# shaohua-pan/RobustCap

Measured on AMD Instinct MI355X. Metric: body-frames/sec (sig_mp fwd + FK) at batch 256, higher is better.
Workload: dtype f32; 1 GPU; synthetic 60 fps, 6 IMU + 33 keypoints, batch 256 x 1448 frames per GPU (256 bodies in total, weak scaling), confidence schedule 'mixed', seeded random weights (63.4 M params); batch_per_gpu=256, bodies_total=256, frames=1448, conf=mixed, parallelism=dp1 (sequence sharding)

## Files before the change

### include/robustcap_hip.h

```cpp
#ifndef ROBUSTCAP_HIP_H
#define ROBUSTCAP_HIP_H

#include <stdint.h>

#ifdef __cplusplus
extern "C" {
#endif

typedef struct rc_ctx rc_ctx;

typedef enum {
    RC_OK = 0,
    RC_ERR_INVALID = -1,
    RC_ERR_HIP = -2,
    RC_ERR_STATE = -3,
    RC_ERR_UNKNOWN_KEY = -4
} rc_status;

typedef struct {
    double conf_lo, conf_hi;
    float contact_threshold;
    float distance_threshold;
    float height_threshold;
    double tran_filter_num;
    int32_t use_flat_floor;
    int32_t use_vision_updater;
    int32_t use_imu_updater;
    int32_t live;
    int32_t update_vision_freq;
    int32_t use_reproj_opt;
    float smooth;
    int32_t reserved;
} rc_params;

#define RC_FLAG_FIRST_FRAME 1u

int rc_create(int32_t batch, int32_t live_at_construction, rc_ctx** out);
int rc_destroy(rc_ctx* ctx);
const char* rc_last_error(const rc_ctx* ctx);
int rc_default_params(int32_t live_at_construction, rc_params* out);
int rc_get_params(const rc_ctx* ctx, rc_params* out);
int rc_set_params(rc_ctx* ctx, const rc_params* p);

int rc_load_weight(rc_ctx* ctx, const char* key, const float* host, int64_t numel);
int rc_finalize_weights(rc_ctx* ctx);

int rc_set_body(rc_ctx* ctx, const int32_t* parent, const float* J, const float* w33, const float* v33);

int rc_set_gravity(rc_ctx* ctx, const float* gravity_host);

int rc_reset(rc_ctx* ctx, const uint8_t* row_mask, void* stream);

int rc_step(rc_ctx* ctx, const float* j2dc, const float* accc, const float* oric, const float* first_tran,
            uint32_t flags, float* pose_out, float* tran_out, void* stream);

int rc_sequence(rc_ctx* ctx, int32_t T, const float* j2dc, int64_t rs_j2d, const float* accc, int64_t rs_acc,
                const float* oric, int64_t rs_ori, const float* first_tran, uint32_t flags, float* pose_out,
                int64_t rs_pose, float* tran_out, int64_t rs_tran, void* stream);

int rc_sequence_rows(rc_ctx* ctx, int32_t T, const int32_t* len_host, const float* j2dc, int64_t rs_j2d, const float* accc,
                     int64_t rs_acc, const float* oric, int64_t rs_ori, const float* first_tran, uint32_t flags, float* pose_out,
                     int64_t rs_pose, float* tran_out, int64_t rs_tran, void* stream);
int rc_get_sequence_row_frames(rc_ctx* ctx, int64_t* body_frames);

int rc_set_gemm_mode(rc_ctx* ctx, int32_t mode);
int rc_get_gemm_mode(const rc_ctx* ctx);
int rc_default_gemm_mode(int32_t total_rows);

int rc_set_sequence_mode(rc_ctx* ctx, int32_t mode, int32_t min_frames);
int rc_get_sequence_stats(rc_ctx* ctx, int64_t* wave_frames, int64_t* stepped_frames, int64_t* ticks);
int rc_get_launch_stats(rc_ctx* ctx, int64_t* lds_launches, int64_t* other_wide_launches);
int rc_get_launch_stats_w32(rc_ctx* ctx, int64_t* w32_launches);
int rc_set_resident(rc_ctx* ctx, int32_t enable, int32_t workgroups);
int rc_get_resident_stats(rc_ctx* ctx, int64_t* segments, int64_t* aborts);
int rc_plan_sequence(const int8_t* codes, int32_t B, int32_t T, const int32_t* pend, uint32_t flags, int32_t use_vision_updater,
                     uint8_t* mode_out);
int rc_plan_wave(const int8_t* codes, int32_t B, int32_t T, int32_t t0, const int32_t* first_reach, const int32_t* pend,
                 int32_t use_imu_updater, int32_t use_vision_updater, int32_t* frame_at, int64_t frame_at_cap,
                 int32_t* n_ticks, int32_t* n_prep, int32_t* counts, double* est_us);
int rc_plan_wave_rows(const int8_t* codes, int32_t B, int32_t T, int32_t t0, const int32_t* len, const int32_t* first_reach,
                      const int32_t* pend, int32_t use_imu_updater, int32_t use_vision_updater, int32_t* frame_at, int64_t frame_at_cap,
                      int32_t* n_ticks, int32_t* n_prep, int32_t* counts, double* est_us);

int rc_live_begin(rc_ctx* ctx);
int rc_live_step(rc_ctx* ctx, const float* j2dc_host, const float* accc_host, const float* oric_host,
                 const float* first_tran_host, uint32_t flags, float* pose_host, float* tran_host);
int rc_live_end(rc_ctx* ctx);
int rc_get_live_stats(rc_ctx* ctx, int64_t* lean_frames, int64_t* full_frames);
int rc_get_live_prestep(rc_ctx* ctx, int64_t* presteps, int32_t* available);
int rc_get_live_replayed(rc_ctx* ctx, int64_t* frames);
int rc_get_live_spin(rc_ctx* ctx, int64_t* taken, int64_t* lost);
int rc_get_live_profile(rc_ctx* ctx, double* avg_us4);
int rc_get_live_last_profile(rc_ctx* ctx, double* us6);
int rc_get_live_backend(rc_ctx* ctx, int32_t* lean_captured, int32_t* aql, char* note, int32_t note_len);

int rc_r6d_to_rotmat(const float* r6d, float* R, int64_t n, void* stream);
int rc_axis_angle_to_rotmat(const float* aa, float* R, int64_t n, void* stream);
int rc_rotmat_to_axis_angle(const float* R, float* aa, int64_t n, void* stream);
int rc_rotmat_to_r6d(const float* R, float* r6d, int64_t n, void* stream);
int rc_angle_between(const float* R1, const float* R2, float* out, int64_t n, void* stream);
int rc_lerp(const float* a, const float* b, double t, float* out, int64_t n, void* stream);
int rc_normalize_rows(const float* x, float* out, float* norm, int64_t rows, int32_t width, void* stream);
int rc_bbox_normalise(const float* kp, float* out, int64_t n, void* stream);
int rc_conf_mean(const float* j2dc, int64_t n, double lo, double hi, float* mean, int8_t* code, void* stream);
int rc_shape_body(rc_ctx* ctx, const float* v_template, const float* shapedirs, const float* J_regressor, const float* beta,
                  int32_t V, float* verts_out, float* joints_out);
int rc_fk_r(rc_ctx* ctx, const float* Rlocal, float* Rglobal, int64_t n, void* stream);
int rc_bone_to_joint(rc_ctx* ctx, const float* bone, float* joint, int64_t n, void* stream);
int rc_joint_to_bone(rc_ctx* ctx, const float* joint, float* bone, int64_t n, void* stream);
int rc_zero_pose(rc_ctx* ctx, float* joint, float* vert, void* stream);
int rc_ik_r(rc_ctx* ctx, const float* Rglobal, float* Rlocal, int64_t n, void* stream);
int rc_fk_bone(rc_ctx* ctx, const float* Rglobal, float* joints, int64_t n, void* stream);
int rc_body_fk(rc_ctx* ctx, const float* pose, const float* tran, float* grot, float* joint, float* j33,
               int64_t n, void* stream);
int rc_lstm_step(rc_ctx* ctx, const char* net, const float* x, const uint8_t* row_mask, float* y, void* stream);
#define RC_SUBNET_SCRATCH_BYTES (256ll << 20)
int rc_subnet_forward(rc_ctx* ctx, const char* net, int32_t n, const int32_t* lengths_host, const float* x, float* y,
                      const float* init_h, const float* init_c, float* final_h, float* final_c, void* stream);
int rc_init_net_forward(rc_ctx* ctx, int32_t n, const float* v, float* out, void* stream);
int rc_get_subnet_stats(rc_ctx* ctx, int64_t* calls, int64_t* frames, int64_t* chunks, int64_t* scratch_bytes);
int rc_set_mesh(rc_ctx* ctx, const float* v_template_host, const float* weights_host, int32_t V);
int rc_body_mesh(rc_ctx* ctx, const float* pose, const float* tran, float* vert, int64_t n, void* stream);
int rc_set_regressor(rc_ctx* ctx, const float* j_regressor_host, int32_t n_rows, int32_t n_used);
int rc_mesh_metrics(rc_ctx* ctx, const float* pose, const float* gt_pose, int64_t n, float* per_frame, double* mean_host,
                    void* stream);
int rc_synth_imu(rc_ctx* ctx, const float* pose, const float* tran, const int32_t* vertex_ids_host,
                 const int32_t* joint_ids_host, int64_t T, int32_t smooth_n, float* imu_ori, float* imu_acc, float* joint3d,
                 float* vert6, void* stream);
int rc_syn_acc(const float* v, int64_t T, int64_t width, int32_t smooth_n, float* acc, void* stream);
int rc_procrustes_error(const float* S1, const float* S2, int64_t n, int32_t n_points, float* err, void* stream);
int rc_position_error(const float* p, const float* t, int64_t n, float* dist, double* mean_host, void* stream);
int rc_set_ignored_landmarks(rc_ctx* ctx, const int32_t* ids_host, int32_t n);
int rc_reproj_residual(rc_ctx* ctx, const float* pose, const float* tran, const float* kp, const float* K,
                       float sigma, float* loss, int64_t T, void* stream);


int rc_smplify_set_prior(rc_ctx* ctx, const float* means_host, const float* precisions_host, const float* nll_weights_host);

int rc_smplify_loss_grad(rc_ctx* ctx, const float* x, const float* kp, const float* ref3d, const float* imu_aa,
                         const float* K_host, int64_t T, double* loss_host, float* grad, void* stream);

int rc_smplify_set_ref3d(rc_ctx* ctx, const float* ref3d);

typedef struct rc_smplify_info {
    int32_t status;
    int32_t n_iter, n_eval;
    int32_t reserved;
    double first_loss, final_loss;
    double host_ms, device_ms;
} rc_smplify_info;

int rc_smplify_run(rc_ctx* ctx, const float* pose, const float* tran, const float* kp, const float* imu_ori,
                   const float* K_host, int64_t T, float lr, int32_t max_iter, float loss_threshold, float* pose_out,
                   float* tran_out, uint8_t* update_host, rc_smplify_info* info, void* stream);

int rc_smplify_run_batch(rc_ctx* ctx, int32_t n_rows, const int64_t* T_rows, const float* const* pose, const float* const* tran,
                         const float* const* kp, const float* const* imu_ori, const float* K_host, float lr, int32_t max_iter,
                         float loss_threshold, float* const* pose_out, float* const* tran_out, uint8_t* const* update_host,
                         rc_smplify_info* infos, void* stream);

typedef double (*rc_objective_fn)(void* user, const double* x, double* grad, int64_t n);
int rc_lbfgs_minimize(rc_objective_fn objective, void* user, int64_t n, double* x, double lr, int32_t max_iter,
                      int32_t max_eval, int32_t history_size, double tolerance_grad, double tolerance_change,
                      int32_t* n_iter_out, int32_t* n_eval_out, double* losses_out, int64_t cap);

int rc_camera_inputs(const float* kp_pix, const float* imu_acc_w, const float* imu_ori_w, const float* K_host,
                     const float* Tcw_host, float* j2dc, float* accc, float* oric, float* gravity_out_host, int64_t n,
                     void* stream);

int rc_camera_inputs_rows(const float* kp_norm, const float* imu_acc_w, const float* imu_ori_w, const int32_t* seq_of_row,
                          const int32_t* len, const float* K_host, const float* Tcw_host, float image_w, float image_h,
                          int32_t n_rows, int32_t Tmax, float* j2dc, float* accc, float* oric, float* gravity_out_host,
                          void* cam_scratch, void* stream);

int rc_get_state(rc_ctx* ctx, const char* net, float* h_host, float* c_host, void* stream);
int rc_get_fusion_state(rc_ctx* ctx, int32_t* out_host, void* stream);

int rc_get_trace(rc_ctx* ctx, int32_t* trace_host, void* stream);

int rc_gemm_timing(rc_ctx* ctx, int32_t enable);
int rc_gemm_timing_read(rc_ctx* ctx, double* total_ms, int64_t* launches);
int rc_gemm_timing_busy(rc_ctx* ctx, double* busy_ms);

#ifdef __cplusplus
}
#endif
#endif
```

### robustcap_amd/_lib.py

```python
import ctypes as C
import os

_HERE = os.path.dirname(os.path.abspath(__file__))
LIB_PATH = os.environ.get("RC_LIB_PATH") or os.path.join(_HERE, "csrc", "librobustcap_hip.so")
HEADER_PATH = os.path.join(os.path.dirname(_HERE), "include", "robustcap_hip.h")

RC_FLAG_FIRST_FRAME = 1


class RcParams(C.Structure):
    _fields_ = [("conf_lo", C.c_double), ("conf_hi", C.c_double),
                ("contact_threshold", C.c_float), ("distance_threshold", C.c_float),
                ("height_threshold", C.c_float), ("tran_filter_num", C.c_double),
                ("use_flat_floor", C.c_int32), ("use_vision_updater", C.c_int32),
                ("use_imu_updater", C.c_int32), ("live", C.c_int32),
                ("update_vision_freq", C.c_int32), ("use_reproj_opt", C.c_int32), ("smooth", C.c_float),
                ("reserved", C.c_int32)]


class RcSmplifyInfo(C.Structure):
    _fields_ = [("status", C.c_int32), ("n_iter", C.c_int32), ("n_eval", C.c_int32), ("reserved", C.c_int32),
                ("first_loss", C.c_double), ("final_loss", C.c_double), ("host_ms", C.c_double), ("device_ms", C.c_double)]


OBJECTIVE_FN = C.CFUNCTYPE(C.c_double, C.c_void_p, C.POINTER(C.c_double), C.POINTER(C.c_double), C.c_int64)


class RobustcapLibraryError(RuntimeError):
    pass


_P, _I32, _I64, _U32, _F = C.c_void_p, C.c_int32, C.c_int64, C.c_uint32, C.c_float
SIGNATURES = {
    "rc_create": (_I32, [_I32, _I32, C.POINTER(_P)]),
    "rc_destroy": (_I32, [_P]),
    "rc_last_error": (C.c_char_p, [_P]),
    "rc_default_params": (_I32, [_I32, C.POINTER(RcParams)]),
    "rc_get_params": (_I32, [_P, C.POINTER(RcParams)]),
    "rc_set_params": (_I32, [_P, C.POINTER(RcParams)]),
    "rc_load_weight": (_I32, [_P, C.c_char_p, _P, _I64]),
    "rc_finalize_weights": (_I32, [_P]),
    "rc_set_body": (_I32, [_P, _P, _P, _P, _P]),
    "rc_set_gravity": (_I32, [_P, _P]),
    "rc_reset": (_I32, [_P, _P, _P]),
    "rc_step": (_I32, [_P, _P, _P, _P, _P, _U32, _P, _P, _P]),
    "rc_sequence": (_I32, [_P, _I32, _P, _I64, _P, _I64, _P, _I64, _P, _U32, _P, _I64, _P, _I64, _P]),
    "rc_sequence_rows": (_I32, [_P, _I32, _P, _P, _I64, _P, _I64, _P, _I64, _P, _U32, _P, _I64, _P, _I64, _P]),
    "rc_get_sequence_row_frames": (_I32, [_P, C.POINTER(_I64)]),
    "rc_set_gemm_mode": (_I32, [_P, _I32]),
    "rc_get_gemm_mode": (_I32, [_P]),
    "rc_default_gemm_mode": (_I32, [_I32]),
    "rc_set_sequence_mode": (_I32, [_P, _I32, _I32]),
    "rc_get_sequence_stats": (_I32, [_P, C.POINTER(_I64), C.POINTER(_I64), C.POINTER(_I64)]),
    "rc_get_launch_stats": (_I32, [_P, C.POINTER(_I64), C.POINTER(_I64)]),
    "rc_get_launch_stats_w32": (_I32, [_P, C.POINTER(_I64)]),
    "rc_set_resident": (_I32, [_P, _I32, _I32]),
    "rc_get_resident_stats": (_I32, [_P, C.POINTER(_I64), C.POINTER(_I64)]),
    "rc_plan_sequence": (_I32, [_P, _I32, _I32, _P, _U32, _I32, _P]),
    "rc_plan_wave": (_I32, [_P, _I32, _I32, _I32, _P, _P, _I32, _I32, _P, _I64, C.POINTER(_I32), C.POINTER(_I32), _P, _P]),
    "rc_plan_wave_rows": (_I32, [_P, _I32, _I32, _I32, _P, _P, _P, _I32, _I32, _P, _I64, C.POINTER(_I32), C.POINTER(_I32), _P, _P]),
    "rc_live_begin": (_I32, [_P]),
    "rc_live_step": (_I32, [_P, _P, _P, _P, _P, _U32, _P, _P]),
    "rc_live_end": (_I32, [_P]),
    "rc_get_live_stats": (_I32, [_P, _P, _P]),
    "rc_get_live_prestep": (_I32, [_P, _P, _P]),
    "rc_get_live_replayed": (_I32, [_P, _P]),
    "rc_get_live_spin": (_I32, [_P, _P, _P]),
    "rc_get_live_profile": (_I32, [_P, _P]),
    "rc_get_live_last_profile": (_I32, [_P, _P]),
    "rc_get_live_backend": (_I32, [_P, _P, _P, _P, _I32]),
    "rc_get_fusion_state": (_I32, [_P, _P, _P]),
    "rc_r6d_to_rotmat": (_I32, [_P, _P, _I64, _P]),
    "rc_axis_angle_to_rotmat": (_I32, [_P, _P, _I64, _P]),
    "rc_rotmat_to_axis_angle": (_I32, [_P, _P, _I64, _P]),
    "rc_rotmat_to_r6d": (_I32, [_P, _P, _I64, _P]),
    "rc_angle_between": (_I32, [_P, _P, _P, _I64, _P]),
    "rc_lerp": (_I32, [_P, _P, C.c_double, _P, _I64, _P]),
    "rc_normalize_rows": (_I32, [_P, _P, _P, _I64, _I32, _P]),
    "rc_bbox_normalise": (_I32, [_P, _P, _I64, _P]),
    "rc_conf_mean": (_I32, [_P, _I64, C.c_double, C.c_double, _P, _P, _P]),
    "rc_shape_body": (_I32, [_P, _P, _P, _P, _P, _I32, _P, _P]),
    "rc_fk_r": (_I32, [_P, _P, _P, _I64, _P]),
    "rc_bone_to_joint": (_I32, [_P, _P, _P, _I64, _P]),
    "rc_joint_to_bone": (_I32, [_P, _P, _P, _I64, _P]),
    "rc_zero_pose": (_I32, [_P, _P, _P, _P]),
    "rc_ik_r": (_I32, [_P, _P, _P, _I64, _P]),
    "rc_fk_bone": (_I32, [_P, _P, _P, _I64, _P]),
    "rc_body_fk": (_I32, [_P, _P, _P, _P, _P, _P, _I64, _P]),
    "rc_set_mesh": (_I32, [_P, _P, _P, _I32]),
    "rc_body_mesh": (_I32, [_P, _P, _P, _P, _I64, _P]),
    "rc_set_regressor": (_I32, [_P, _P, _I32, _I32]),
    "rc_mesh_metrics": (_I32, [_P, _P, _P, _I64, _P, C.POINTER(C.c_double), _P]),
    "rc_synth_imu": (_I32, [_P, _P, _P, _P, _P, _I64, _I32, _P, _P, _P, _P, _P]),
    "rc_syn_acc": (_I32, [_P, _I64, _I64, _I32, _P, _P]),
    "rc_procrustes_error": (_I32, [_P, _P, _I64, _I32, _P, _P]),
    "rc_position_error": (_I32, [_P, _P, _I64, _P, C.POINTER(C.c_double), _P]),
    "rc_lstm_step": (_I32, [_P, C.c_char_p, _P, _P, _P, _P]),
    "rc_subnet_forward": (_I32, [_P, C.c_char_p, _I32, _P, _P, _P, _P, _P, _P, _P, _P]),
    "rc_init_net_forward": (_I32, [_P, _I32, _P, _P, _P]),
    "rc_get_subnet_stats": (_I32, [_P, C.POINTER(_I64), C.POINTER(_I64), C.POINTER(_I64), C.POINTER(_I64)]),
    "rc_set_ignored_landmarks": (_I32, [_P, _P, _I32]),
    "rc_reproj_residual": (_I32, [_P, _P, _P, _P, _P, _F, _P, _I64, _P]),
    "rc_smplify_set_prior": (_I32, [_P, _P, _P, _P]),
    "rc_smplify_set_ref3d": (_I32, [_P, _P]),
    "rc_smplify_loss_grad": (_I32, [_P, _P, _P, _P, _P, _P, _I64, C.POINTER(C.c_double), _P, _P]),
    "rc_smplify_run": (_I32, [_P, _P, _P, _P, _P, _P, _I64, _F, _I32, _F, _P, _P, _P, C.POINTER(RcSmplifyInfo), _P]),
    "rc_smplify_run_batch": (_I32, [_P, _I32, _P, _P, _P, _P, _P, _P, _F, _I32, _F, _P, _P, _P, _P, _P]),
    "rc_lbfgs_minimize": (_I32, [OBJECTIVE_FN, _P, _I64, C.POINTER(C.c_double), C.c_double, _I32, _I32, _I32, C.c_double,
                                 C.c_double, C.POINTER(_I32), C.POINTER(_I32), C.POINTER(C.c_double), _I64]),
    "rc_camera_inputs": (_I32, [_P, _P, _P, _P, _P, _P, _P, _P, _P, _I64, _P]),
    "rc_camera_inputs_rows": (_I32, [_P, _P, _P, _P, _P, _P, _P, _F, _F, _I32, _I32, _P, _P, _P, _P, _P, _P]),
    "rc_get_state": (_I32, [_P, C.c_char_p, _P, _P, _P]),
    "rc_get_trace": (_I32, [_P, _P, _P]),
    "rc_gemm_timing": (_I32, [_P, _I32]),
    "rc_gemm_timing_read": (_I32, [_P, C.POINTER(C.c_double), C.POINTER(_I64)]),
    "rc_gemm_timing_busy": (_I32, [_P, C.POINTER(C.c_double)]),
}

_lib = None


OPTIONAL_IN_AB_BUILDS = frozenset({"rc_get_launch_stats_w32", "rc_set_resident", "rc_get_resident_stats", "rc_get_launch_stats", "rc_get_live_spin", "rc_get_live_replayed", "rc_get_live_profile", "rc_get_live_last_profile",
                                   "rc_get_live_prestep"})


def load():
    global _lib
    if _lib is not None:
        return _lib
    if not os.path.exists(LIB_PATH):
        raise RobustcapLibraryError(
            f"{LIB_PATH} not found: the HIP extension is not built. Run "
            "`python -c \"import __graft_entry__ as g; g.build()\"` at the repo root. There is no CPU fallback.")
    try:
        lib = C.CDLL(LIB_PATH)
    except OSError as e:
        raise RobustcapLibraryError(f"cannot load {LIB_PATH}: {e}") from e
    ab_build = bool(os.environ.get("RC_LIB_PATH"))
    skipped = []
    for name, (res, args) in SIGNATURES.items():
        if ab_build and name in OPTIONAL_IN_AB_BUILDS and not hasattr(lib, name):
            skipped.append(name)
            continue
        try:
            fn = getattr(lib, name)
        except AttributeError as e:
            raise RobustcapLibraryError(f"{LIB_PATH} does not export {name}: the library does not match include/robustcap_hip.h") from e
        fn.restype, fn.argtypes = res, args
    if skipped:
        import warnings
        warnings.warn(f"RC_LIB_PATH={LIB_PATH}: entry points missing in this build (calls to them will fail): {', '.join(skipped)}")
    _lib = lib
    return lib


def check(ctx, rc, what):
    if rc != 0:
        msg = load().rc_last_error(ctx)
        raise RobustcapLibraryError(f"{what} failed ({rc}): {msg.decode() if msg else ''}")


def ptr(t):
    return None if t is None else C.c_void_p(t.data_ptr())


def stream_ptr():
    import torch
    return C.c_void_p(torch.cuda.current_stream().cuda_stream)
```

### robustcap_amd/csrc/rc_api.cpp

```cpp
#include "../../include/robustcap_hip.h"
#include "rc_internal.h"

#include <algorithm>
#if defined(__x86_64__) || defined(_M_X64)
#include <immintrin.h>
#define RC_STORE_FENCE() _mm_sfence()
#else
#define RC_STORE_FENCE() __atomic_thread_fence(__ATOMIC_SEQ_CST)
#endif

#include <chrono>
#include <cmath>
#include <cstdio>
#include <cstdlib>
#include <cstring>
#include <map>
#include <string>
#include <thread>
#include <vector>

#define RC_SPLIT_MAIN_MIN_BATCH 48
#define RC_SPLIT_MIN_BATCH 48
#define RC_TILE64_MIN_BATCH 192

// ... 8 lines not shown
struct NetSpec { const char* name; int in, H, out; };
const NetSpec kNets[6] = {{"rnn2", 72, 512, 69},  {"rnn3", 141, 512, 3},   {"rnn4", 171, 1280, 69},
                          {"rnn6", 240, 1024, 3}, {"rnn7", 141, 512, 144}, {"rnn8", 141, 512, 2}};
enum { N2 = 0, N3 = 1, N4 = 2, N6 = 3, N7 = 4, N8 = 5 };
const int kInit[3][2] = {{69, 512}, {512, 1024}, {1024, 2048}};

inline int round_up(int x, int m) { return (x + m - 1) / m * m; }

struct Dense {
    float* W = nullptr; float* b = nullptr;
    void* Ws = nullptr;
    float* Wrm = nullptr;
    int K = 0, N = 0, Kp = 0, Np = 0;
    int mr = 2, nc = 4;
};
struct NetDev {
    Dense lin1, lin2;
    float* Wl[2] = {nullptr, nullptr};
    void* Wls[2] = {nullptr, nullptr};
    float* bl[2] = {nullptr, nullptr};
    float* h = nullptr;
    float* c = nullptr;
    int* steps = nullptr;
    float* x1 = nullptr;
    float* part = nullptr;
    int in = 0, H = 0, out = 0;
    int nc = 4;
    int mr = 2;
};

}

struct rc_ctx {
    int B = 0;
    int Bp = 0;
    int dev = 0;
    rc_params prm{};
    NetDev net[6];
    Dense init[3];
    float *hid1 = nullptr, *hid2 = nullptr, *xtmp = nullptr;
    FrameBuffers fb{};
    BodyConst* body = nullptr;
    float *mesh_vt = nullptr, *mesh_w = nullptr;
    int mesh_V = 0;
    float* mesh_kM = nullptr;
    int mesh_nk = 0;
    std::vector<float> mesh_vt_h, mesh_w_h, mesh_Jr_h;
    float jroot_h[3] = {0.f, 0.f, 0.f};
    bool fold_dirty = false;
    DevBuf<float> sweep_scratch;
    size_t sweep_scratch_cap = 0;
    unsigned long long ign_mask = RC_IGN_DEFAULT;
    bool have_body = false, have_weights = false;
    std::map<std::string, std::vector<float>> staged;
    std::vector<DevBuf<char>> allocs;
    std::vector<std::pair<void*, size_t>> alloc_bytes;
    std::vector<DevBuf<char>> weight_allocs;
    bool alloc_weights = false;
    HipEvent eager_ev;
    bool eager_dirty = false;
    std::string err;
    HipStream live_stream;
    HipGraph live_graph;
    HipGraphExec live_exec;
    PinBuf<float> live_in_h, live_out_h;
    DevBuf<float> live_in_d, live_out_d, live_ft_d;
    float *live_in_io = nullptr, *live_out_io = nullptr;
    bool live_zero_copy = false;
    bool live_eager = false;
    HipGraph live_graph_notr;
    HipGraphExec live_exec_notr;
    std::vector<unsigned char> live_maybe_pend;
    bool live_prev_known = false;
    int live_lean = 1;
    int live_lean_nc = 1;
    HipGraph live_graph_lean;
    HipGraphExec live_exec_lean;
    LiveFrame live_frame{};
    int live_aql_on = 1;
    AqlChain* live_aql = nullptr;
    std::string live_aql_note;
    int live_prestep = 1;
    bool live_spin = false, live_spin_always = false;
    volatile unsigned* spin_mb = nullptr;
    float* spin_in = nullptr;
    PinBuf<unsigned> spin_state_h;
    int aql_prog_spin[2] = {-1, -1}, aql_prog_spin_pre[2] = {-1, -1};
    int spin_pending = -1;
    int spin_pending_par = 0, spin_next_par = 0;
    unsigned long long spin_pending_seq = 0;
    bool live_spin_b2b = true;
    bool spin_valid = false;
    long long stat_live_spin = 0, stat_live_spin_lost = 0;
    bool live_arm = true;
    double live_prestep_idle_us = 500.0;
    DevBuf<float> live_pre_buf;
    int aql_prog_lean = -1, aql_prog_lean_pre = -1, aql_prog_pre = -1;
    bool live_pre_valid = false;
    bool live_have_return = false;
    std::chrono::steady_clock::time_point live_last_return{};
    long long stat_live_pre = 0;
    PinBuf<int> live_status_h;
    std::vector<unsigned char> live_may_reach;
    long long stat_live_lean = 0, stat_live_full = 0;
    long long stat_live_replayed = 0;
    DevBuf<int> live_abort_d;
    bool live_blind = false;
    double live_prof_us[4] = {0.0, 0.0, 0.0, 0.0};
    long long live_prof_n = 0;
    double live_prof_last[6] = {0, 0, 0, 0, 0, 0};
    bool timing = false;
    int timing_mode = 1;
    std::vector<std::pair<HipEvent, HipEvent>> ev_pool;
    size_t ev_used = 0;
    double timed_ms = 0.0;
    double timed_busy_ms = 0.0;
    long long timed_launches = 0;
    bool gemm_split = false;
    bool live_launch = false;
    unsigned live_nt_mask = 63u;
    int seq_mode = 1;
    int seq_min_frames = 8;
    float* x1_alt[6] = {nullptr, nullptr, nullptr, nullptr, nullptr, nullptr};
    int tile6[2] = {0, 0}, tile378[2] = {0, 0}, tile2[2] = {0, 0}, tile4[2] = {0, 0};
    bool ring2_failed = false;
    HipStream aux_stream;
    HipStream wide2_stream;
    HipEvent ev_main[8], ev_aux[8], ev_wide2[4];
    HipStream wide3_stream;
    HipEvent ev_head[4], ev_wide3[4];
    float* x1_alt2[6] = {nullptr, nullptr, nullptr, nullptr, nullptr, nullptr};
    DevBuf<signed char> scan_codes_d;
    PinBuf<signed char> scan_codes_h;
    PinBuf<int> scan_state_h;
    size_t scan_cap = 0;
    long long stat_wave_frames = 0, stat_stepped_frames = 0, stat_ticks = 0;
    long long stat_row_frames = 0;
    DevBuf<int> row_len_d;
    PinBuf<int> row_len_h;
    size_t row_len_cap = 0;
    HipEvent row_len_ev[2];
    unsigned row_len_turn = 0;
    bool ring2_ready = false;
    FrameBuffers ring2[16];
    std::vector<GemmProblem> wave2_prob;
    bool wave2_valid = false;
    DevBuf<int> frame_at_d;
    PinBuf<int> frame_at_h;
    size_t frame_at_cap = 0;
    double cost_tick_us = 1.0, cost_tick_small_us = 13.0, cost_frame_us = 285.0, cost_tr_us = 55.0;
    SmplifyOwner smplify;
    SubnetOwner subnet;
    int trace_next = 0;
    long long stat_wide_launches = 0;
    int lds_min_rows = 64;
    int lds_min_batch = 65;
    int lds_ksplit[3] = {1, 2, 2};
    DevBuf<float> lds_slab;
    DevBuf<int> lds_tickets;
    size_t lds_region_tiles = 0;
    unsigned lds_rot = 0;
    DevBuf<ResidentTick> res_ticks_d;
    PinBuf<ResidentTick> res_ticks_h;
    DevBuf<int> res_ints_d;
    PinBuf<int> res_base_h;
    PinBuf<int> res_abort_h;
    size_t res_cap = 0;
    long long stat_resident_segments = 0, stat_resident_aborts = 0;
    bool live_selfcheck_ran = false;
    bool resident_on = false;
    int resident_wgs = 224;
    long long stat_lds_launches = 0;
    long long stat_w32_launches = 0;
};

namespace {

int fail(rc_ctx* ctx, int code, const std::string& msg) {
    if (ctx) ctx->err = msg; else g_create_error = msg;
    return code;
}

template <typename T>
int dev_alloc(rc_ctx* ctx, T** p, size_t count, bool zero = true) {
    DevBuf<char> q;
    HIP_TRY(ctx, rc_alloc(q, count * sizeof(T)));
    if (zero) HIP_TRY(ctx, hipMemset(q.get(), 0, count * sizeof(T)));
    *p = reinterpret_cast<T*>(q.get());
    if (!ctx->alloc_weights) ctx->alloc_bytes.emplace_back(q.get(), count * sizeof(T));
    (ctx->alloc_weights ? ctx->weight_allocs : ctx->allocs).push_back(std::move(q));
    return RC_OK;
}

int dismiss_queued_frame(rc_ctx* ctx) {
    if (ctx->spin_pending < 0 || !ctx->live_aql || !ctx->spin_mb) return RC_OK;
    const int par = ctx->spin_pending_par;
    ctx->spin_mb[32 * par] = 2u;
    RC_STORE_FENCE();
    const int arc = rc_aql_wait_frame(ctx->live_aql);
    ctx->spin_state_h[4 * par] = 0;
    ctx->stat_live_spin_lost += 1;
    ctx->spin_pending = -1;
    return arc == 0 ? RC_OK : fail(ctx, RC_ERR_HIP, "the live frame queued ahead did not leave");
}

int mark_eager(rc_ctx* ctx, hipStream_t st) {
    ctx->live_pre_valid = false;
    ctx->spin_valid = false;
    if (int rc = dismiss_queued_frame(ctx)) return rc;
    if (!ctx->eager_ev) return RC_OK;
    HIP_TRY(ctx, hipEventRecord(ctx->eager_ev.get(), st));
    ctx->eager_dirty = true;
    return RC_OK;
}

template <typename Body>
void for_column_blocks(int n_cb, Body body) {
    const int nt = std::max(1, std::min({8, n_cb / 8, (int)std::thread::hardware_concurrency()}));
    if (nt <= 1) { for (int cb = 0; cb < n_cb; ++cb) body(cb); return; }
    std::vector<std::thread> th;
    for (int t = 0; t < nt; ++t)
        th.emplace_back([=] { for (int cb = t; cb < n_cb; cb += nt) body(cb); });
    for (std::thread& x : th) x.join();
}

template <typename F>
std::vector<float> pack_weights(int Np, int Kp, F getW) {
    std::vector<float> out((size_t)Np * Kp);
    const int Q = Kp / RC_KC;
    for_column_blocks(Np / 16, [&](int cb) {
        for (int q = 0; q < Q; ++q)
            for (int l = 0; l < 64; ++l) {
                const int kq = l >> 4, j = l & 15;
                float* d = &out[(((size_t)cb * Q + q) * 64 + l) * 4];
                for (int s = 0; s < 4; ++s) d[s] = getW(cb * 16 + j, RC_KC * q + 4 * kq + s);
            }
    });
    return out;
}

template <typename F>
std::vector<uint16_t> pack_weights_split(int Np, int Kp, F getW) {
    std::vector<uint16_t> out((size_t)Np * Kp * 3);
    const int Qs = Kp / 32;
    for_column_blocks(Np / 16, [&](int cb) {
        for (int kb = 0; kb < Qs; ++kb)
            for (int l = 0; l < 64; ++l) {
                const int kq = l >> 4, j = l & 15;
                for (int e = 0; e < 8; ++e) {
                    const int k = 32 * kb + (e < 4 ? 4 * kq + e : 16 + 4 * kq + (e - 4));
                    const float w = getW(cb * 16 + j, k);
                    uint32_t u;
                    std::memcpy(&u, &w, 4);
                    const uint32_t uh = u & 0xffff0000u;
                    float fh;
                    std::memcpy(&fh, &uh, 4);
                    const float r1 = w - fh;
                    uint32_t u1;
                    std::memcpy(&u1, &r1, 4);
                    const uint32_t um = u1 & 0xffff0000u;
                    float fm;
                    std::memcpy(&fm, &um, 4);
                    const float r2 = r1 - fm;
                    uint32_t u2;
                    std::memcpy(&u2, &r2, 4);
                    const size_t base = (((size_t)cb * Qs + kb) * 3) * 512 + (size_t)l * 8 + e;
                    out[base] = (uint16_t)(uh >> 16);
                    out[base + 512] = (uint16_t)(um >> 16);
                    out[base + 1024] = (uint16_t)(u2 >> 16);
                }
            }
    });
    return out;
}

int upload16(rc_ctx* ctx, void** dst, const std::vector<uint16_t>& v) {
    uint16_t* q = nullptr;
    if (int rc = dev_alloc(ctx, &q, v.size(), false)) return rc;
    HIP_TRY(ctx, hipMemcpy(q, v.data(), v.size() * sizeof(uint16_t), hipMemcpyHostToDevice));
    *dst = q;
    return RC_OK;
}

int upload(rc_ctx* ctx, float** dst, const std::vector<float>& v) {
    if (int rc = dev_alloc(ctx, dst, v.size(), false)) return rc;
    HIP_TRY(ctx, hipMemcpy(*dst, v.data(), v.size() * sizeof(float), hipMemcpyHostToDevice));
    return RC_OK;
}

int make_dense(rc_ctx* ctx, Dense& d, const std::vector<float>& W, const std::vector<float>& b, int N, int K) {
    d.mr = N <= 160 ? 1 : 2; d.nc = N <= 160 ? 2 : 4;
    d.N = N; d.K = K; d.Kp = round_up(K, RC_KALIGN); d.Np = round_up(N, 16 * d.nc);
    auto get = [&](int n, int k) -> float { return (n < N && k < K) ? W[(size_t)n * K + k] : 0.0f; };
    std::vector<float> bp(d.Np, 0.0f);
    for (int n = 0; n < N; ++n) bp[n] = b[n];
    if (int rc = upload(ctx, &d.W, pack_weights(d.Np, d.Kp, get))) return rc;
    if (int rc = upload16(ctx, &d.Ws, pack_weights_split(d.Np, d.Kp, get))) return rc;
    if (N <= 160) if (int rc = upload(ctx, &d.Wrm, W)) return rc;
    return upload(ctx, &d.b, bp);
}

const std::vector<float>* staged(rc_ctx* ctx, const std::string& key, size_t numel) {
    auto it = ctx->staged.find(key);
    if (it == ctx->staged.end() || it->second.size() != numel) return nullptr;
    return &it->second;
}
// ... 604 lines not shown
        if (i < 4) HIP_TRY(ctx, hipEventCreateWithFlags(rc_out(ctx->ev_wide3[i]), evf));
    }
    ctx->ring2_ready = true;
    ctx->wave2_valid = false;
    return RC_OK;
}

int ensure_wave2_buffers(rc_ctx* ctx) {
    if (ctx->ring2_ready) return RC_OK;
    if (ctx->ring2_failed) return fail(ctx, RC_ERR_STATE, "wavefront engine: its buffers could not be allocated earlier (out of memory?)");
    const int rc = ensure_wave2_buffers_once(ctx);
    if (rc != RC_OK) ctx->ring2_failed = true;
    return rc;
}

int build_wave2_problems(rc_ctx* ctx) {
    ctx->wave2_prob.assign((size_t)kRing * W2_PROB, GemmProblem{});
    const int B = ctx->B;
    for (int sl = 0; sl < kRing; ++sl) {
        const FrameBuffers& fb = ctx->ring2[sl];
        for (int q = 0; q < RC_TICK_PROB; ++q) {
            const TickStage& ts = kTick[q];
            const NetDev& n = ctx->net[ts.net];
            float* x1 = (sl & 1) ? ctx->x1_alt[ts.net] : n.x1;
            Stage st{ts.net, (int)RC_ROW2_VALID, nullptr, 256, Out{nullptr, 0, 0, false}, fb.flags2};
            switch (ts.net) {
                case N4: st.x = fb.x4; st.y = Out{fb.x6, 256, 171, true}; st.flag_bit = (int)RC_ROW2_M4; st.x_alt = fb.x4l;
                         st.sel_bit = (int)RC_ROW_VIS; st.out_bit = (int)RC_ROW_VIS; break;
                case N2: st.x = fb.x2; st.ldx = 128; st.y = Out{fb.x3, 256, 72, true}; break;
                case N6: st.x = fb.x6; st.y = Out{fb.pc, 4, 0, false}; st.flag_bit = (int)RC_ROW2_M6; st.x_alt = fb.x6l;
                         st.sel_bit = (int)RC_ROW_PC; st.out_bit = (int)RC_ROW_PC; break;
                case N3: st.x = fb.x3; st.y = Out{fb.vr, 4, 0, false}; break;
                case N7: st.x = fb.x78; st.y = Out{fb.r6d, 144, 0, false}; break;
                default: st.x = fb.x78; st.y = Out{fb.contact, 2, 0, false}; break;
            }
            GemmProblem p = ts.kind == 0 ? lin1_problem(ctx, st) : (ts.kind == 3 ? lin2_problem(ctx, st) : lstm_problem(ctx, st, ts.kind - 1));
            if (ts.kind == 0) { p.out = x1; p.sel_flags = fb.flags; }
            if (ts.kind == 1) p.seg[0].base = x1;
            if (ts.kind == 3) p.out_flags = fb.flags;
            p.steps = fb.wsteps + (size_t)ts.net * B;
            p.open_step = 0; p.step_off = 0;
            ctx->wave2_prob[(size_t)sl * W2_PROB + q] = p;
        }
        ctx->wave2_prob[(size_t)sl * W2_PROB + W2_INIT0] = dense_problem(ctx, ctx->init[0], seg(fb.xi, 128, 0), Out{ctx->hid1, 512, 0, true}, true, RC_ROW_REACH, fb.flags, nullptr, false);
        ctx->wave2_prob[(size_t)sl * W2_PROB + W2_INIT1] = dense_problem(ctx, ctx->init[1], seg(ctx->hid1, 512, 0), Out{ctx->hid2, 1024, 0, true}, true, RC_ROW_REACH, fb.flags, nullptr, false);
        ctx->wave2_prob[(size_t)sl * W2_PROB + W2_INIT2] = dense_problem(ctx, ctx->init[2], seg(ctx->hid2, 1024, 0), Out{ctx->fb.init_out, 2048, 0, false}, false, RC_ROW_REACH, fb.flags, nullptr, false);
    }
    ctx->wave2_valid = true;
    return RC_OK;
}

inline int w2_stage(int q) { return q < RC_TICK_PROB ? kTick[q].stage : kInitStage + (q - W2_INIT0); }

enum WaveEngine { ENG_PLAIN, ENG_SPLIT, ENG_TRI };
WaveEngine pick_wave_engine(const rc_ctx* c) {
    if (c->B < RC_SPLIT_MAIN_MIN_BATCH) return ENG_PLAIN;
    return lds_context(c) ? ENG_TRI : ENG_SPLIT;
}
bool resident_segment(const rc_ctx* c, WaveEngine eng, const WavePlan& P) {
    return eng == ENG_TRI && c->resident_on && c->B <= 256 && P.n_ticks > 0 && !(c->timing && c->timing_mode != 3);
}
inline int w2_group(int q, bool tri) {
    if (q >= RC_TICK_PROB) return tri ? G_REST : G_BIG;
    return (tri && kTick[q].net == N6 && kTick[q].group == G_BIG) ? G_REST : kTick[q].group;
}

struct WaveTiles { int t4[2], t6[2], t5[2]; };
WaveTiles wave_tiles(WaveEngine eng) {
    WaveTiles t{{4, eng == ENG_PLAIN ? 5 : 8}, {4, 8}, {4, 8}};
    tile_env("RC_SEQ_RNN4", &t.t4[0], &t.t4[1]);
    tile_env("RC_SEQ_RNN6", &t.t6[0], &t.t6[1]);
    tile_env("RC_SEQ_H512", &t.t5[0], &t.t5[1]);
    return t;
}

int reserve_frame_at(rc_ctx* ctx, size_t need, size_t want) {
    HIP_TRY(ctx, rc_grow(ctx->frame_at_cap, need, want, ctx->frame_at_d, want, ctx->frame_at_h, want));
    return RC_OK;
}

std::vector<GemmProblem> collect(const rc_ctx* ctx, const WavePlan& P, WaveEngine eng, const WaveTiles& tiles, int k, int g) {
    static const int tile64_rows = tune_env("RC_SEQ_TILE64_ROWS", 33);
    static const bool rows_as_padded = tune_env("RC_SEQ_ROWS_AS_PADDED", 1) != 0;
    const int B = ctx->B;
    std::vector<GemmProblem> ps;
    for (int qi = 0; qi < W2_PROB; ++qi) {
        const int q = qi < 4 ? (qi ^ 2) : qi;
        if (w2_group(q, eng == ENG_TRI) != g) continue;
        const int e = k - w2_stage(q);
        if (e < 0 || e >= P.n_prep) continue;
        const int net = q < RC_TICK_PROB ? kTick[q].net : -1;
        const int kind = q < RC_TICK_PROB ? kTick[q].kind : 4;
        const int riders = P.n_rider[e];
        const int rows = kind == 4 ? P.n_reach[e] : ((net == N4 || net == N6) ? P.n_vis[e] + riders : P.n_valid[e]);
        if (rows <= 0) continue;
        const int rows_k = kind == 4 ? rows : rows + (rows_as_padded ? P.done(e) : 0);
        GemmProblem p = ctx->wave2_prob[(size_t)(e % kRing) * W2_PROB + q];
        if (kind == 0 || kind == 1) {
            float* x1 = e % 3 == 0 ? ctx->net[net].x1 : (e % 3 == 1 ? ctx->x1_alt[net] : ctx->x1_alt2[net]);
            if (kind == 0) p.out = x1; else p.seg[0].base = x1;
        }
        if (kind == 1 || kind == 2) {
            const NetDev& n = ctx->net[net];
            int mr, nc;
            if (lds_problem(ctx, rows_k)) {
                mr = 16; nc = 8;
            } else if (ctx->gemm_split && rows_k >= tile64_rows) {
                const int* t = n.H == 512 ? tiles.t5 : (n.H == 1024 ? tiles.t6 : tiles.t4);
                mr = t[0]; nc = t[1];
            } else {
                pick_tile(n.H, rows_k, &mr, &nc);
            }
            p.mr = mr; p.nc = nc; p.n_tiles = n.H / (4 * nc);
        } else if (kind == 0 || kind == 4) {
            if (rows_k <= 16) { p.mr = 1; p.nc = 1; p.n_tiles = (p.N + 15) / 16; }
            else if (kind == 0 && ctx->gemm_split && rows_k >= tile64_rows) {
                const int np = round_up(p.N, 64);
                if (np % 128 == 0) { p.mr = 4; p.nc = 8; p.n_tiles = np / 128; }
            }
        }
        p.m_tiles = (rows + 16 * p.mr - 1) / (16 * p.mr);
        if (rows == B && kind != 4) {
            p.flags = nullptr; p.flag_bit = 0;
            if (riders == 0 && (net == N4 || net == N6) && P.n_vis[e] == B) {
                p.alt_base = nullptr; p.sel_flags = nullptr; p.sel_bit = 0; p.out_flags = nullptr; p.out_bit = 0;
            }
        }
        ps.push_back(p);
    }
    if (g != G_LIN2) {
        int total = 0;
        for (const GemmProblem& p : ps) total += p.n_tiles * p.m_tiles;
        if (total > 0 && total <= 128)
            for (GemmProblem& p : ps)
                if (p.epi == RC_EPI_LSTM && p.mr == 4 && p.nc == 8) { p.nc = 4; p.n_tiles *= 2; }
    }
    return ps;
}

struct WaveSeg {
    rc_ctx* ctx; const WavePlan& P; const FrameIO& io0; hipStream_t st, aux;
    WaveEngine eng; WaveTiles tiles; rc_params_dev prm; WavePrep wp; WaveTail wt;
    int rows(const std::vector<int>& v, int tick) const { return tick >= 0 && tick < P.n_prep ? v[tick] : 0; }
    std::vector<GemmProblem> group(int k, int g) const { return collect(ctx, P, eng, tiles, k, g); }
};

void wave_prep(WaveSeg& S, int k) {
    if (k >= S.P.n_prep) return;
    S.wp.frame_at = S.ctx->frame_at_d.get() + (size_t)k * S.ctx->B;
    S.wp.first_tick = k == 0 ? 1 : 0;
    rc_launch_prep_wave(S.ctx->ring2[k % kRing], S.io0, S.prm, S.ctx->B, S.wp, S.aux);
}

int wave_lin2_fuse_tail(WaveSeg& S, int k, bool merge, hipEvent_t signal) {
    rc_ctx* ctx = S.ctx;
    const int B = ctx->B;
    if (int rc = launch_problems(ctx, S.group(k, G_LIN2), nullptr, S.aux, true)) return rc;
    const bool fuse = S.rows(S.P.n_valid, k - kFuseStage) > 0, tail = S.rows(S.P.n_valid, k - kTailStage) > 0;
    bool merged = false, carried = false;
    if (tail) {
        const FrameBuffers& tgt = ctx->ring2[k % kRing];
        S.wt.x4l = tgt.x4l; S.wt.x6l = tgt.x6l; S.wt.flags2 = tgt.flags2; S.wt.wsteps = tgt.wsteps;
    }
    if (merge && fuse && tail)
        merged = carried = rc_launch_fuse_tail(ctx->ring2[(k - kTailStage) % kRing], ctx->ring2[(k - kFuseStage) % kRing], S.io0, S.prm, ctx->body, B, S.wt, S.aux, signal);
    if (!merged && fuse) rc_launch_fuse(ctx->ring2[(k - kFuseStage) % kRing], S.io0, S.prm, B, S.aux);
    if (!merged && tail) {
        rc_launch_tail(ctx->ring2[(k - kTailStage) % kRing], S.io0, S.prm, ctx->body, B, 0, S.aux, nullptr, &S.wt, signal);
        carried = true;
    }
    if (signal && !carried) HIP_TRY(ctx, hipEventRecord(signal, S.aux));
    return RC_OK;
}

inline int wave_wait(rc_ctx* ctx, int k, hipStream_t s, std::initializer_list<hipEvent_t> waits) {
    if (k > 0) for (hipEvent_t w : waits) if (w) HIP_TRY(ctx, hipStreamWaitEvent(s, w, 0));
    return RC_OK;
}

int wave_issue(rc_ctx* ctx, int k, hipStream_t s, std::initializer_list<hipEvent_t> waits, const std::vector<GemmProblem>& ps, hipEvent_t signal) {
    if (int rc = wave_wait(ctx, k, s, waits)) return rc;
    bool carried = false;
    if (int rc = launch_problems(ctx, ps, nullptr, s, false, signal, &carried)) return rc;
    if (signal && !carried) HIP_TRY(ctx, hipEventRecord(signal, s));
    return RC_OK;
}

int stream_tick(WaveSeg& S, int k) {
    rc_ctx* ctx = S.ctx;
    const int e = k & 3, ep = (k + 3) & 3;
    hipStream_t st = S.st, aux = S.aux, w2 = ctx->wide2_stream.get(), w3 = ctx->wide3_stream.get();
    hipEvent_t main_p = ctx->ev_main[ep].get(), aux_p = ctx->ev_aux[ep].get(), w2_p = ctx->ev_wide2[ep].get(), w3_p = ctx->ev_wide3[ep].get(),
               head_p = ctx->ev_head[ep].get();
    hipEvent_t main_e = ctx->ev_main[e].get(), aux_e = ctx->ev_aux[e].get(), w2_e = ctx->ev_wide2[e].get(), w3_e = ctx->ev_wide3[e].get(),
               head_e = ctx->ev_head[e].get();
    bool init_now = false;
    for (int q = W2_INIT0; q < W2_PROB; ++q) init_now = init_now || S.rows(S.P.n_reach, k - w2_stage(q)) > 0;
    if (S.eng == ENG_TRI) {
        std::vector<GemmProblem> l1, rnn6, h512;
        for (const GemmProblem& p : S.group(k, G_REST)) (p.epi != RC_EPI_LSTM ? l1 : (p.H == 1024 ? rnn6 : h512)).push_back(p);
        if (int rc = wave_issue(ctx, k, aux, {}, l1, head_e)) return rc;
        wave_prep(S, k);
        if (int rc = wave_wait(ctx, k, aux, {w3_p, main_p, w2_p})) return rc;
        if (int rc = wave_lin2_fuse_tail(S, k, true, aux_e)) return rc;
        if (int rc = wave_issue(ctx, k, w2, {head_p}, rnn6, w2_e)) return rc;
        static const int h5_early = tune_env("RC_SEQ_H5_EARLY", 0);
        const bool early = h5_early && S.rows(S.P.n_reach, k - 1 - kTailStage) == 0;
        if (int rc = wave_issue(ctx, k, w3, {early ? head_p : aux_p}, h512, w3_e)) return rc;
        if (int rc = wave_issue(ctx, k, st, {head_p}, S.group(k, G_BIG), main_e)) return rc;
    } else if (S.eng == ENG_SPLIT) {
        if (int rc = wave_wait(ctx, k, aux, {main_p, w2_p})) return rc;
        wave_prep(S, k);
        if (int rc = wave_lin2_fuse_tail(S, k, false, aux_e)) return rc;
        if (int rc = wave_issue(ctx, k, w2, {aux_p}, S.group(k, G_REST), w2_e)) return rc;
        if (int rc = wave_issue(ctx, k, st, {w2_p, init_now ? aux_p : nullptr}, S.group(k, G_BIG), main_e)) return rc;
    } else {
        if (int rc = wave_wait(ctx, k, aux, {main_p})) return rc;
        wave_prep(S, k);
        if (int rc = wave_lin2_fuse_tail(S, k, false, aux_e)) return rc;
        if (int rc = wave_issue(ctx, k, st, {init_now ? aux_p : nullptr}, S.group(k, G_BIG), nullptr)) return rc;
        if (int rc = wave_issue(ctx, k, st, {init_now ? nullptr : aux_p}, S.group(k, G_REST), main_e)) return rc;
    }
    ctx->stat_ticks += 1;
    return RC_OK;
}

struct ResidentWords { int *item_base, *done, *tick_done, *words; };

int build_resident_ticks(WaveSeg& S, std::vector<std::vector<GemmProblem>>& init_l) {
    rc_ctx* ctx = S.ctx;
    int run = 0;
    for (int k = 0; k < S.P.n_ticks; ++k) {
        std::vector<GemmProblem> ls;
        for (int g : {G_BIG, G_REST})
            for (GemmProblem& p : S.group(k, g)) {
                if (p.epi == RC_EPI_LSTM) { p.mr = 16; p.nc = 8; }
                else if (p.epi == RC_EPI_RELU && p.out_packed && p.N % 128 == 0 && p.Kp % 128 == 0 && p.out_bit == 0 && p.out_col0 == 0 && p.seg[0].par_mode == 0 &&
                         p.out != ctx->hid1 && p.out != ctx->hid2) { }
                else { init_l[k].push_back(p); continue; }
                p.m_tiles = 1;
                ls.push_back(p);
            }
        ResidentTick& T = ctx->res_ticks_h[k];
        const size_t region = (size_t)(k & 3);
        size_t tiles = 0;
        T.B = ctx->B;
        T.n = build_lds_problems(ctx, ls, nullptr, ctx->lds_slab.get() + region * ctx->lds_region_tiles * RC_LDS_SLAB_FLOATS,
                                 ctx->lds_tickets.get() + region * ctx->lds_region_tiles, T.p, RC_RES_MAXP, &T.n_items, &tiles, true);
        if (T.n != (int)ls.size()) return fail(ctx, RC_ERR_INVALID, "resident engine: more problems in a tick than its table holds");
        if (tiles > ctx->lds_region_tiles) return fail(ctx, RC_ERR_INVALID, "resident engine: more tiles in a tick than a slab region holds");
        const bool tail_wrote = S.rows(S.P.n_reach, k - 1 - kTailStage) > 0;
        for (int i = 0; i < RC_RES_MAXP; ++i) {
            T.dep[i][0] = T.dep[i][1] = -1; T.dep_items[i][0] = T.dep_items[i][1] = 0;
            T.need_tail[i] = 0;
            if (i >= T.n) continue;
            const bool lstm = T.p[i].epi == RC_EPI_LSTM;
            T.need_tail[i] = lstm ? ((tail_wrote && T.p[i].H == 512) ? 1 : 0) : 1;
            if (k == 0 || !lstm) continue;
            const ResidentTick& Tp = ctx->res_ticks_h[k - 1];
            for (int j = 0; j < Tp.n; ++j) {
                const int items_j = (j + 1 < Tp.n ? Tp.p[j + 1].wg_base : Tp.n_items) - Tp.p[j].wg_base;
                const bool lstm_j = Tp.p[j].epi == RC_EPI_LSTM;
                if (lstm_j && Tp.p[j].hstate == T.p[i].hstate) { T.dep[i][0] = j; T.dep_items[i][0] = items_j; }
                if ((const float*)(lstm_j ? Tp.p[j].hstate : Tp.p[j].out) == T.p[i].seg[0].base) { T.dep[i][1] = j; T.dep_items[i][1] = items_j; }
            }
        }
        ctx->res_base_h[k] = run;
        run += T.n_items;
    }
    ctx->res_base_h[S.P.n_ticks] = run;
    return RC_OK;
}

int run_resident_segment(WaveSeg& S) {
    rc_ctx* ctx = S.ctx;
    hipStream_t st = S.st, aux = S.aux;
    const int res_wgs = std::min(240, std::max(8, ctx->resident_wgs));
    if (int rc = ensure_lds_pool(ctx)) return rc;
    if (!ctx->res_abort_h) {
        HIP_TRY(ctx, rc_alloc(ctx->res_abort_h, 1));
        ctx->res_abort_h[0] = 0;
    }
    const size_t nt = (size_t)S.P.n_ticks;
    if (nt > ctx->res_cap) {
        HIP_TRY(ctx, hipDeviceSynchronize());
        const size_t cap = nt + nt / 4 + 64;
        HIP_TRY(ctx, rc_grow(ctx->res_cap, nt, cap, ctx->res_ticks_d, cap, ctx->res_ticks_h, cap,
                             ctx->res_ints_d, cap * (RC_RES_MAXP + 2) + 1 + 4 + 16, ctx->res_base_h, cap + 1));
    }
    const size_t cap = ctx->res_cap;
    ResidentWords W{};
    W.item_base = ctx->res_ints_d.get(); W.done = W.item_base + cap + 1; W.tick_done = W.done + cap * RC_RES_MAXP; W.words = W.tick_done + cap;
    std::vector<std::vector<GemmProblem>> init_l(nt);
    if (int rc = build_resident_ticks(S, init_l)) return rc;
    HIP_TRY(ctx, hipMemcpyAsync(ctx->res_ticks_d.get(), ctx->res_ticks_h.get(), nt * sizeof(ResidentTick), hipMemcpyHostToDevice, st));
    HIP_TRY(ctx, hipMemcpyAsync(W.item_base, ctx->res_base_h.get(), (nt + 1) * sizeof(int), hipMemcpyHostToDevice, st));
    HIP_TRY(ctx, hipMemsetAsync(W.done, 0, (cap * (RC_RES_MAXP + 1) + 4 + 16) * sizeof(int), st));
    HIP_TRY(ctx, hipEventRecord(ctx->ev_main[6].get(), st));
    HIP_TRY(ctx, hipStreamWaitEvent(aux, ctx->ev_main[6].get(), 0));
    ResidentArgs R{};
    R.ticks = ctx->res_ticks_d.get(); R.item_base = W.item_base; R.n_ticks = S.P.n_ticks;
    R.head = W.words; R.done = W.done; R.tick_done = W.tick_done;
    R.flag_tail = W.words + 2; R.abort = W.words + 3;
    R.spin_bound = (unsigned long long)std::max(1, tune_env("RC_SEQ_RESIDENT_BOUND_MS", 2000)) * 100000ull;
    {
        hipEvent_t ta = nullptr, tb = nullptr;
        if (ctx->timing && !timing_pair(ctx, &ta, &tb)) return fail(ctx, RC_ERR_HIP, "hipEventCreate");
        if (ta) HIP_TRY(ctx, hipEventRecord(ta, st));
        rc_launch_gemm_resident(R, res_wgs, st);
        if (tb) HIP_TRY(ctx, hipEventRecord(tb, st));
    }
    ctx->stat_lds_launches += 1;
    for (int k = 0; k < S.P.n_ticks; ++k) {
        if (int rc = launch_problems(ctx, init_l[k], nullptr, aux, false)) return rc;
        wave_prep(S, k);
        if (k > 0) rc_launch_flag_wait(W.tick_done + (k - 1), ctx->res_ticks_h[k - 1].n_items, W.words + 3, R.spin_bound, aux);
// ... 556 lines not shown
        {
            std::vector<int> fr(ctx->scan_state_h.get(), ctx->scan_state_h.get() + B), pd(ctx->scan_state_h.get() + B, ctx->scan_state_h.get() + 2 * B);
            if (w0) {
                for (int b = 0; b < B; ++b) {
                    if (L && L[b] < 1) continue;
                    const int c = ctx->scan_codes_h[b];
                    if (fr[b] && c == 2 && imu) fr[b] = 0;
                    pd[b] = (c == 0 && vup) ? 1 : 0;
                }
            }
            const double cost[4] = {ctx->cost_tick_us, ctx->cost_tick_small_us, ctx->cost_frame_us, ctx->cost_tr_us};
            plan_wave(ctx->scan_codes_h.get(), B, T, w0, fr.data(), pd.data(), imu, vup, cost, wplan, L);
            if (ctx->seq_mode == 2 || wplan.est_wave_us < wplan.est_stepped_us) wave2_from = w0;
            static const bool dbg = tune_env("RC_SEQ_DEBUG", 0) != 0;
            if (dbg) std::fprintf(stderr, "rc_sequence plan: T=%d ticks=%d lag_max=%d est_wave=%.0f us est_stepped=%.0f us -> %s\n", T, wplan.n_ticks,
                                  wplan.lag_max, wplan.est_wave_us, wplan.est_stepped_us, wave2_from >= 0 ? "wavefront" : "frame-stepped");
        }
        plan_sequence(ctx->scan_codes_h.get(), B, T, ctx->scan_state_h.get() + B, ff, vup, mode.data(), L);
    }
    bool prep_done = false;
    for (int t = 0; t < T;) {
        if (t == wave2_from) {
            FrameIO io0 = io_at(0);
            io0.first_tran = nullptr;
            if (int rc = run_wave2_segment(ctx, wplan, io0, t, T - 1, st)) return rc;
            t = T;
        } else {
            const bool chain = t + 1 < T && t + 1 != wave2_from;
            const FrameIO next = chain ? io_at(t + 1) : FrameIO{};
            if (int rc = step_impl(ctx, io_at(t), t == 0 ? flags : 0u, st, mode[t] == SEQ_STEPPED_TR, prep_done, chain ? &next : nullptr,
                                   L ? n_live[t] : -1)) return rc;
            prep_done = chain;
            ctx->stat_stepped_frames += 1;
            ++t;
        }
    }
    return mark_eager(ctx, st);
}

int rc_sequence(rc_ctx* ctx, int32_t T, const float* j2dc, int64_t rs_j2d, const float* accc, int64_t rs_acc, const float* oric,
                int64_t rs_ori, const float* first_tran, uint32_t flags, float* pose_out, int64_t rs_pose, float* tran_out,
                int64_t rs_tran, void* stream) {
    if (int rc = check_ready(ctx)) return rc;
    if (T == 0) return RC_OK;
    ctx->live_prev_known = false;
    if (T < 0 || !j2dc || !accc || !oric || !pose_out || !tran_out) return fail(ctx, RC_ERR_INVALID, "rc_sequence: bad argument");
    return sequence_impl(ctx, T, nullptr, 0, j2dc, rs_j2d, accc, rs_acc, oric, rs_ori, first_tran, flags, pose_out, rs_pose, tran_out, rs_tran, stream);
}

int rc_sequence_rows(rc_ctx* ctx, int32_t T, const int32_t* len_host, const float* j2dc, int64_t rs_j2d, const float* accc, int64_t rs_acc,
                     const float* oric, int64_t rs_ori, const float* first_tran, uint32_t flags, float* pose_out, int64_t rs_pose,
                     float* tran_out, int64_t rs_tran, void* stream) {
    if (int rc = check_ready(ctx)) return rc;
    if (T < 0 || !len_host || !j2dc || !accc || !oric || !pose_out || !tran_out) return fail(ctx, RC_ERR_INVALID, "rc_sequence_rows: bad argument");
    const size_t B = (size_t)ctx->B;
    for (size_t b = 0; b < B; ++b)
        if (len_host[b] < 0 || len_host[b] > T) return fail(ctx, RC_ERR_INVALID, "rc_sequence_rows: a row's length is outside 0 .. T");
    if (T == 0) return RC_OK;
    ctx->live_prev_known = false;
    hipStream_t st = (hipStream_t)stream;
    for (HipEvent& ev : ctx->row_len_ev)
        if (!ev) HIP_TRY(ctx, hipEventCreateWithFlags(rc_out(ev), hipEventDisableTiming));
    const unsigned turn = ctx->row_len_turn++ & 1u;
    if (B > ctx->row_len_cap) HIP_TRY(ctx, rc_grow(ctx->row_len_cap, B, B, ctx->row_len_d, B, ctx->row_len_h, 2 * B));
    else HIP_TRY(ctx, hipEventSynchronize(ctx->row_len_ev[turn].get()));
    int* len_h = ctx->row_len_h.get() + turn * B;
    std::memcpy(len_h, len_host, B * sizeof(int));
    HIP_TRY(ctx, hipMemcpyAsync(ctx->row_len_d.get(), len_h, B * sizeof(int), hipMemcpyHostToDevice, st));
    HIP_TRY(ctx, hipEventRecord(ctx->row_len_ev[turn].get(), st));
    return sequence_impl(ctx, T, len_h, 0, j2dc, rs_j2d, accc, rs_acc, oric, rs_ori, first_tran, flags, pose_out, rs_pose, tran_out, rs_tran, stream);
}

int rc_get_sequence_row_frames(rc_ctx* ctx, int64_t* body_frames) {
    if (!ctx || !body_frames) return RC_ERR_INVALID;
    *body_frames = ctx->stat_row_frames;
    return RC_OK;
}

int rc_set_gemm_mode(rc_ctx* ctx, int32_t mode) {
    if (!ctx || mode < 0 || mode > 1) return ctx ? fail(ctx, RC_ERR_INVALID, "rc_set_gemm_mode: 0 (fp32 MFMA) or 1 (split-bf16 products)") : RC_ERR_INVALID;
    if ((mode != 0) != ctx->gemm_split) rc_live_end(ctx);
    ctx->gemm_split = mode != 0;
    return RC_OK;
}
int rc_get_gemm_mode(const rc_ctx* ctx) { return ctx ? (ctx->gemm_split ? 1 : 0) : RC_ERR_INVALID; }
int rc_default_gemm_mode(int32_t total_rows) { return tune_env("RC_GEMM_SPLIT", total_rows >= RC_SPLIT_MIN_BATCH ? 1 : 0) != 0 ? 1 : 0; }

int rc_set_sequence_mode(rc_ctx* ctx, int32_t mode, int32_t min_frames) {
    if (!ctx || mode < 0 || mode > 2 || min_frames < 1) return ctx ? fail(ctx, RC_ERR_INVALID, "rc_set_sequence_mode: mode 0|1|2, min_frames >= 1") : RC_ERR_INVALID;
    ctx->seq_mode = mode;
    ctx->seq_min_frames = min_frames;
    return RC_OK;
}

int rc_get_sequence_stats(rc_ctx* ctx, int64_t* wave_frames, int64_t* stepped_frames, int64_t* ticks) {
    if (!ctx) return RC_ERR_INVALID;
    if (wave_frames) *wave_frames = ctx->stat_wave_frames;
    if (stepped_frames) *stepped_frames = ctx->stat_stepped_frames;
    if (ticks) *ticks = ctx->stat_ticks;
    return RC_OK;
}

int rc_set_resident(rc_ctx* ctx, int32_t enable, int32_t workgroups) {
    if (!ctx) return RC_ERR_INVALID;
    ctx->resident_on = enable != 0;
    if (workgroups > 0) ctx->resident_wgs = workgroups;
    return RC_OK;
}

int rc_get_resident_stats(rc_ctx* ctx, int64_t* segments, int64_t* aborts) {
    if (!ctx) return RC_ERR_INVALID;
    if (segments) *segments = ctx->stat_resident_segments;
    if (aborts) *aborts = ctx->stat_resident_aborts;
    return RC_OK;
}

int rc_get_launch_stats_w32(rc_ctx* ctx, int64_t* w32_launches) {
    if (!ctx || !w32_launches) return RC_ERR_INVALID;
    *w32_launches = ctx->stat_w32_launches;
    return RC_OK;
}

int rc_get_launch_stats(rc_ctx* ctx, int64_t* tick_launches, int64_t* other_wide_launches) {
    if (!ctx) return RC_ERR_INVALID;
    if (tick_launches) *tick_launches = ctx->stat_lds_launches;
    if (other_wide_launches) *other_wide_launches = ctx->stat_wide_launches;
    return RC_OK;
}

int rc_plan_sequence(const int8_t* codes, int32_t B, int32_t T, const int32_t* pend, uint32_t flags, int32_t use_vision_updater,
                     uint8_t* mode_out) {
    if (!codes || !pend || !mode_out || B < 1 || T < 0) return RC_ERR_INVALID;
    plan_sequence(reinterpret_cast<const signed char*>(codes), B, T, pend, (flags & RC_FLAG_FIRST_FRAME) != 0, use_vision_updater != 0, mode_out);
    return RC_OK;
}

static int plan_wave_abi(const int8_t* codes, int32_t B, int32_t T, int32_t t0, const int32_t* len, const int32_t* first_reach,
                         const int32_t* pend, int32_t use_imu_updater, int32_t use_vision_updater, int32_t* frame_at, int64_t frame_at_cap,
                         int32_t* n_ticks, int32_t* n_prep, int32_t* counts, double* est_us) {
    if (!codes || !first_reach || !pend || !n_ticks || !n_prep || B < 1 || T < 1 || t0 < 0 || t0 >= T) return RC_ERR_INVALID;
    WavePlan P;
    const double cost[4] = {1.0, 13.0, 285.0, 55.0};
    plan_wave(reinterpret_cast<const signed char*>(codes), B, T, t0, first_reach, pend, use_imu_updater != 0, use_vision_updater != 0, cost, P, len);
    *n_ticks = P.n_ticks;
    *n_prep = P.n_prep;
    if (est_us) { est_us[0] = P.est_wave_us; est_us[1] = P.est_stepped_us; }
    if (!frame_at || (int64_t)P.frame_at.size() > frame_at_cap) return RC_ERR_INVALID;
    std::memcpy(frame_at, P.frame_at.data(), P.frame_at.size() * sizeof(int));
    if (counts)
        for (int k = 0; k < P.n_prep; ++k) {
            counts[k] = P.n_valid[k]; counts[P.n_prep + k] = P.n_vis[k];
            counts[2 * P.n_prep + k] = P.n_rider[k]; counts[3 * P.n_prep + k] = P.n_reach[k];
        }
    return RC_OK;
}

int rc_plan_wave(const int8_t* codes, int32_t B, int32_t T, int32_t t0, const int32_t* first_reach, const int32_t* pend,
                 int32_t use_imu_updater, int32_t use_vision_updater, int32_t* frame_at, int64_t frame_at_cap, int32_t* n_ticks,
                 int32_t* n_prep, int32_t* counts, double* est_us) {
    return plan_wave_abi(codes, B, T, t0, nullptr, first_reach, pend, use_imu_updater, use_vision_updater, frame_at, frame_at_cap, n_ticks, n_prep,
                         counts, est_us);
}

int rc_plan_wave_rows(const int8_t* codes, int32_t B, int32_t T, int32_t t0, const int32_t* len, const int32_t* first_reach,
                      const int32_t* pend, int32_t use_imu_updater, int32_t use_vision_updater, int32_t* frame_at, int64_t frame_at_cap,
                      int32_t* n_ticks, int32_t* n_prep, int32_t* counts, double* est_us) {
    if (!len || B < 1) return RC_ERR_INVALID;
    for (int b = 0; b < B; ++b) if (len[b] < 0 || len[b] > T) return RC_ERR_INVALID;
    return plan_wave_abi(codes, B, T, t0, len, first_reach, pend, use_imu_updater, use_vision_updater, frame_at, frame_at_cap, n_ticks, n_prep,
                         counts, est_us);
}

int rc_live_end(rc_ctx* ctx) {
    if (!ctx) return RC_ERR_INVALID;
    ctx->live_exec.reset(); ctx->live_graph.reset(); ctx->live_exec_notr.reset();
    if (ctx->live_aql) { rc_aql_destroy(ctx->live_aql); ctx->live_aql = nullptr; }
    ctx->spin_mb = nullptr; ctx->spin_in = nullptr; ctx->spin_pending = -1; ctx->spin_valid = false;
    for (int q = 0; q < 2; ++q) ctx->aql_prog_spin[q] = ctx->aql_prog_spin_pre[q] = -1;
    ctx->spin_state_h.reset(); ctx->live_pre_buf.reset();
    ctx->aql_prog_lean = ctx->aql_prog_lean_pre = ctx->aql_prog_pre = -1;
    ctx->live_pre_valid = false; ctx->live_have_return = false;
    ctx->live_exec_lean.reset(); ctx->live_graph_lean.reset(); ctx->live_status_h.reset(); ctx->live_abort_d.reset();
    ctx->live_graph_notr.reset(); ctx->live_stream.reset();
    ctx->live_in_h.reset(); ctx->live_out_h.reset(); ctx->live_in_d.reset(); ctx->live_out_d.reset(); ctx->live_ft_d.reset();
    return RC_OK;
}

int rc_live_begin(rc_ctx* ctx) {
    if (int rc = check_ready(ctx)) return rc;
    rc_live_end(ctx);
    const size_t B = ctx->B;
    HIP_TRY(ctx, hipStreamCreateWithFlags(rc_out(ctx->live_stream), hipStreamNonBlocking));
    HIP_TRY(ctx, rc_alloc(ctx->live_in_h, B * 171, hipHostMallocMapped));
    HIP_TRY(ctx, rc_alloc(ctx->live_out_h, B * 219, hipHostMallocMapped));
    HIP_TRY(ctx, rc_alloc_all(ctx->live_in_d, B * 171, ctx->live_out_d, B * 219, ctx->live_ft_d, B * 3));
    ctx->live_zero_copy = B <= 16;
    ctx->live_in_io = ctx->live_in_d.get();
    ctx->live_out_io = ctx->live_out_d.get();
    if (ctx->live_zero_copy) {
        HIP_TRY(ctx, hipHostGetDevicePointer((void**)&ctx->live_in_io, ctx->live_in_h.get(), 0));
        HIP_TRY(ctx, hipHostGetDevicePointer((void**)&ctx->live_out_io, ctx->live_out_h.get(), 0));
    }
    hipStream_t st = ctx->live_stream.get();
    const bool timing = ctx->timing;
    struct TimingGuard { rc_ctx* c; bool v; ~TimingGuard() { c->timing = v; } } timing_guard{ctx, timing};
    ctx->timing = false;
    FrameIO io{ctx->live_in_io, ctx->live_in_io + B * 99, ctx->live_in_io + B * 117, nullptr,
               ctx->live_out_io, ctx->live_out_io + B * 216, 99, 18, 54, 216, 3};
    int rc = RC_OK;
    for (int v = 0; v < 2 && !rc; ++v) {
        HIP_TRY(ctx, hipStreamBeginCapture(st, hipStreamCaptureModeThreadLocal));
        if (!ctx->live_zero_copy) (void)hipMemcpyAsync(ctx->live_in_d.get(), ctx->live_in_h.get(), B * 171 * sizeof(float), hipMemcpyHostToDevice, st);
        ctx->live_launch = true;
        rc = step_impl(ctx, io, 0u, st, v == 0);
        ctx->live_launch = false;
        if (!ctx->live_zero_copy) (void)hipMemcpyAsync(ctx->live_out_h.get(), ctx->live_out_d.get(), B * 219 * sizeof(float), hipMemcpyDeviceToHost, st);
        HipGraph& g = v == 0 ? ctx->live_graph : ctx->live_graph_notr;
        const hipError_t e = hipStreamEndCapture(st, rc_out(g));
        if (!rc && e != hipSuccess) rc = fail(ctx, RC_ERR_HIP, std::string("hipStreamEndCapture: ") + hipGetErrorString(e));
        if (!rc && hipGraphInstantiate(rc_out(v == 0 ? ctx->live_exec : ctx->live_exec_notr), g.get(), nullptr, nullptr, 0) != hipSuccess)
            rc = fail(ctx, RC_ERR_HIP, "hipGraphInstantiate");
    }
    if (!rc && ctx->live_lean && B <= RC_LIVE_MAXB && !ctx->gemm_split) {
        ctx->live_aql_note.clear();
        auto lean_setup = [&]() -> std::string {
            if (rc_alloc(ctx->live_status_h, 1, hipHostMallocMapped) != hipSuccess) return "lean frame: status word allocation failed";
            ctx->live_status_h[0] = 0;
            if (rc_alloc(ctx->live_abort_d, 16) != hipSuccess || hipMemset(ctx->live_abort_d.get(), 0, 64) != hipSuccess) return "lean frame: abort word allocation failed";
            LiveFrame& F = ctx->live_frame;
            F = LiveFrame{};
            for (int i = 0; i < 6; ++i) {
                const NetDev& n = ctx->net[i];
                LiveNet& l = F.net[i];
                l.W1 = n.lin1.W; l.b1 = n.lin1.b;
                for (int q = 0; q < 2; ++q) { l.Wl[q] = n.Wl[q]; l.bl[q] = n.bl[q]; }
                l.W2 = n.lin2.Wrm; l.b2 = n.lin2.b;
                l.x1 = n.x1; l.h = n.h; l.c = n.c; l.part = n.part; l.steps = n.steps;
                l.H = n.H; l.out = n.out; l.outp = round_up(n.out, 4); l.Kp1 = n.lin1.Kp;
                l.BpH = (long long)ctx->Bp * n.H;
            }
            F.fb = ctx->fb; F.io = io; F.prm = dev_params(ctx->prm); F.body = ctx->body; F.B = (int)B; F.nc = ctx->live_lean_nc;
            if (hipHostGetDevicePointer((void**)&F.status, ctx->live_status_h.get(), 0) != hipSuccess) return "lean frame: status word not mapped";
            F.abort = ctx->live_abort_d.get();
            std::vector<LiveKernel> plan(RC_LIVE_KERNELS);
            const int nk = rc_live_plan(F, plan.data());
            if (nk != RC_LIVE_KERNELS) return "lean frame: sub-net sizes these kernels are not compiled for";
            if (hipStreamBeginCapture(st, hipStreamCaptureModeThreadLocal) != hipSuccess) return "lean frame: hipStreamBeginCapture failed";
            if (!ctx->live_zero_copy) (void)hipMemcpyAsync(ctx->live_in_d.get(), ctx->live_in_h.get(), B * 171 * sizeof(float), hipMemcpyHostToDevice, st);
            rc_launch_live_frame(F, st);
            if (!ctx->live_zero_copy) (void)hipMemcpyAsync(ctx->live_out_h.get(), ctx->live_out_d.get(), B * 219 * sizeof(float), hipMemcpyDeviceToHost, st);
            const hipError_t e = hipStreamEndCapture(st, rc_out(ctx->live_graph_lean));
            if (e != hipSuccess) return std::string("lean frame: hipStreamEndCapture: ") + hipGetErrorString(e);
            if (hipGraphInstantiate(rc_out(ctx->live_exec_lean), ctx->live_graph_lean.get(), nullptr, nullptr, 0) != hipSuccess) return "lean frame: hipGraphInstantiate failed";
            const char* preload = std::getenv("LD_PRELOAD");
            bool tool = std::getenv("ROCP_TOOL_LIBRARIES") || std::getenv("HSA_TOOLS_LIB") || std::getenv("ROCPROFILER_REGISTER_FORCE_LOAD") ||
                        std::getenv("ROCR_DEBUG_AGENT") || std::getenv("HSA_ENABLE_DEBUG");
            for (const char* sub : {"rocprof", "roctracer", "rocm-debug", "rocgdb", "omnitrace", "rocprofiler"}) tool = tool || (preload && std::strstr(preload, sub));
            if (tool && ctx->live_aql_on == 1) ctx->live_aql_note = "a profiling / debugging tool intercepts the HSA queues";
            else if (ctx->live_aql_on && ctx->live_zero_copy && !ctx->live_eager) {
                char msg[256] = {0};
                if (rc_aql_create(ctx->dev, &ctx->live_aql, msg, (int)sizeof(msg)) != 0) { ctx->live_aql = nullptr; ctx->live_aql_note = msg; }
                else if ((ctx->aql_prog_lean = rc_aql_add(ctx->live_aql, plan.data(), nk, 1, msg, (int)sizeof(msg))) < 0) {
                    rc_aql_destroy(ctx->live_aql); ctx->live_aql = nullptr; ctx->live_aql_note = msg;
                } else if (ctx->live_prestep && F.nc == 1) {
                    const size_t nf = (size_t)rc_live_pre_floats(F);
                    if (rc_alloc(ctx->live_pre_buf, nf) == hipSuccess && hipMemset(ctx->live_pre_buf.get(), 0, nf * sizeof(float)) == hipSuccess) {
                        std::vector<LiveKernel> plan2(RC_LIVE_KERNELS), plan3(2);
                        const int n3 = rc_live_pre_plan(F, ctx->live_pre_buf.get(), plan3.data());
                        if (rc_live_plan(F, plan2.data(), ctx->live_pre_buf.get()) == RC_LIVE_KERNELS && n3 >= 1) {
                            ctx->aql_prog_lean_pre = rc_aql_add(ctx->live_aql, plan2.data(), RC_LIVE_KERNELS, 1, msg, (int)sizeof(msg));
                            if (ctx->aql_prog_lean_pre >= 0) ctx->aql_prog_pre = rc_aql_add(ctx->live_aql, plan3.data(), n3, 0, msg, (int)sizeof(msg));
                        }
                    } else { ctx->live_pre_buf.reset(); (void)hipGetLastError(); }
                    if (ctx->aql_prog_pre < 0) ctx->aql_prog_lean_pre = -1;
                }
                if (ctx->live_aql && (ctx->live_spin || ctx->live_spin_b2b) && ctx->aql_prog_lean >= 0 && RC_LIVE_KERNELS * 6 + 8 <= 64) {
                    void* shared = nullptr;
                    unsigned* state_d = nullptr;
                    if (rc_aql_alloc_shared(ctx->live_aql, 4096 + B * 171 * sizeof(float), &shared) == 0 &&
                        rc_alloc(ctx->spin_state_h, 16, hipHostMallocMapped) == hipSuccess &&
                        hipHostGetDevicePointer((void**)&state_d, ctx->spin_state_h.get(), 0) == hipSuccess) {
                        for (int q = 0; q < 16; ++q) ctx->spin_state_h[q] = 0;
                        ctx->spin_mb = (volatile unsigned*)shared;
                        ctx->spin_in = (float*)((char*)shared + 4096);
                        for (int q = 0; q < 64; ++q) ctx->spin_mb[q] = 0u;
                        LiveFrame Fs = F;
                        Fs.io.j2d = ctx->spin_in; Fs.io.acc = ctx->spin_in + B * 99; Fs.io.ori = ctx->spin_in + B * 117;
                        std::vector<LiveKernel> ps(RC_LIVE_KERNELS);
                        bool ok = true;
                        for (int par = 0; par < 2 && ok; ++par) {
                            Fs.spin_mb = (unsigned*)shared + 32 * par; Fs.spin_state = state_d + 4 * par;
                            if (rc_live_plan(Fs, ps.data()) == RC_LIVE_KERNELS) ctx->aql_prog_spin[par] = rc_aql_add(ctx->live_aql, ps.data(), RC_LIVE_KERNELS, 1, msg, (int)sizeof(msg));
                            ok = ctx->aql_prog_spin[par] >= 0;
                            if (ok && ctx->aql_prog_lean_pre >= 0 && rc_live_plan(Fs, ps.data(), ctx->live_pre_buf.get()) == RC_LIVE_KERNELS)
                                ctx->aql_prog_spin_pre[par] = rc_aql_add(ctx->live_aql, ps.data(), RC_LIVE_KERNELS, 1, msg, (int)sizeof(msg));
                        }
                        if (!ok) ctx->aql_prog_spin[0] = ctx->aql_prog_spin[1] = -1;
                        if (ctx->aql_prog_spin_pre[0] < 0 || ctx->aql_prog_spin_pre[1] < 0) ctx->aql_prog_spin_pre[0] = ctx->aql_prog_spin_pre[1] = -1;
                        if (ok) rc_aql_set_mailbox(ctx->live_aql, ctx->spin_mb);
                    }
                    if (ctx->aql_prog_spin[0] < 0) { ctx->spin_mb = nullptr; ctx->spin_in = nullptr; (void)hipGetLastError(); }
                }
            } else ctx->live_aql_note = "switched off";
            return std::string();
        };
        const std::string why = lean_setup();
// ... 640 lines not shown
```

### robustcap_amd/csrc/rc_frame.hip

```cpp
#include "rc_internal.h"
#include <hip/hip_ext.h>
#include <cstdlib>

#include "rc_device.h"
#include "rc_frame_dev.h"

__global__ __launch_bounds__(64) void rc_prep_kernel(FrameBuffers fb, FrameIO io, rc_params_dev prm, int B, int first_frame) {
    const int row = blockIdx.x;
    if (!rc_row_live(io, row, io.t)) {
        if (threadIdx.x == 0) { fb.flags[row] = 0; fb.flags2[row] = 0; }
        return;
    }
    prep_body(fb, io, prm, row, threadIdx.x, first_frame, fb.pend[row], fb.uv_count[row], io.len ? RC_ROW2_VALID : 0u);
}

template <int RPB>
__global__ __launch_bounds__(64 * RPB) void rc_prep_wave_kernel(FrameBuffers fb, FrameIO io, rc_params_dev prm, int B, WavePrep w) {
    const int row = blockIdx.x * RPB + (threadIdx.x >> 6), lane = threadIdx.x & 63;
    if (row >= B) return;
    const int f = w.frame_at[row];
    const bool rider = w.first_tick && prm.use_vision_updater && fb.pend[row] != 0 && rc_row_live(io, row, io.t + w.t0);
    unsigned fl = 0;
    if (f >= 0) {
        FrameIO iof = io;
        iof.j2d += (long long)f * 99; iof.acc += (long long)f * 18; iof.ori += (long long)f * 54;
        fl = prep_body(fb, iof, prm, row, lane, 0, 0, 0, RC_ROW2_VALID);
    }
    if (lane == 0) {
        fb.frame[row] = f;
        unsigned f2 = f >= 0 ? (RC_ROW2_VALID | ((fl & RC_ROW_VIS) ? RC_ROW2_M4 : 0u) | ((fl & RC_ROW_PC) ? RC_ROW2_M6 : 0u)) : 0u;
        if (f < 0) fb.flags[row] = 0;
        else {
            const int always[4] = {0, 1, 4, 5};
#pragma unroll
            for (int q = 0; q < 4; ++q) { const int n = always[q]; fb.wsteps[n * B + row] = ++w.steps[n][row]; }
            if (fl & RC_ROW_VIS) fb.wsteps[2 * B + row] = ++w.steps[2][row];
            if (fl & RC_ROW_PC) fb.wsteps[3 * B + row] = ++w.steps[3][row];
        }
        if (rider) {
            fb.wsteps[2 * B + row] = ++w.steps[2][row];
            fb.wsteps[3 * B + row] = ++w.steps[3][row];
            f2 |= RC_ROW2_M4 | RC_ROW2_M6;
            fb.pend[row] = 0;
        }
        fb.flags2[row] = (unsigned char)f2;
    }
    if (rider) {
        for (int k = lane; k < 256; k += 64) {
            fb.x4l[rc_pk(row, k, LD_X4)] = w.cx4l[rc_pk(row, k, LD_X4)];
            fb.x6l[rc_pk(row, k, LD_X6)] = w.cx6l[rc_pk(row, k, LD_X6)];
        }
    }
}

__device__ __forceinline__ void fuse_body(const FrameBuffers& fb, const FrameIO& io, const rc_params_dev& prm, const int B, const int idx) {
    const int row = idx / 24, j = idx % 24;
    if (row >= B) return;
    int frame = 0;
    if (fb.frame) { frame = fb.frame[row]; if (frame < 0) return; }
    else if (!rc_row_live(io, row, io.t)) return;
    const int regime = fb.regime[row];
    if (j == 23) {
        if (regime == 2 && prm.use_imu_updater && fb.first_reach[row]) {
            fb.first_reach[row] = 0;
            fb.flags[row] |= RC_ROW_REACH;
            fb.trace[row * 8 + 4] = 1;
        }
        return;
    }
    const float* R = io.ori + row * io.s_ori + (long long)frame * 54 + 45;
    float vc[3], vi[3];
#pragma unroll
    for (int c = 0; c < 3; ++c) {
        vc[c] = fb.x6[rc_pk(row, 171 + 3 * j + c, LD_X6)];
        vi[c] = fb.x3[rc_pk(row, 72 + 3 * j + c, LD_X3)];
    }
    float out[3];
    if (regime == 0) {
        out[0] = vi[0]; out[1] = vi[1]; out[2] = vi[2];
    } else {
        float v[3];
#pragma unroll
        for (int c = 0; c < 3; ++c) v[c] = (vc[0] * R[c] + vc[1] * R[3 + c]) + vc[2] * R[6 + c];
        if (regime == 2) {
            out[0] = v[0]; out[1] = v[1]; out[2] = v[2];
        } else {
            const double k = fb.kconf[row];
            const float w1 = (float)(1.0 - k), w2 = (float)k;
#pragma unroll
            for (int c = 0; c < 3; ++c) out[c] = vi[c] * w1 + v[c] * w2;
        }
    }
#pragma unroll
    for (int c = 0; c < 3; ++c) {
        fb.x78[rc_pk(row, 72 + 3 * j + c, LD_X78)] = out[c];
        fb.xi[rc_pk(row, 3 * j + c, LD_XI)] = out[c];
    }
}

__global__ __launch_bounds__(256) void rc_fuse_kernel(FrameBuffers fb, FrameIO io, rc_params_dev prm, int B) {
    fuse_body(fb, io, prm, B, blockIdx.x * 256 + threadIdx.x);
}

__global__ __launch_bounds__(256) void rc_fuse_tail_kernel(FrameBuffers fb_tail, FrameBuffers fb_fuse, FrameIO io, rc_params_dev prm,
                                                           const BodyConst* __restrict__ body_g, int B, WaveTail wt, int n_tail_blocks) {
    __shared__ WaveScratch s_all[4];
    __shared__ __attribute__((aligned(16))) BodyConst s_body;
    if ((int)blockIdx.x >= n_tail_blocks) {
        fuse_body(fb_fuse, io, prm, B, ((int)blockIdx.x - n_tail_blocks) * 256 + (int)threadIdx.x);
        return;
    }
    tail_impl<4, false>(fb_tail, io, prm, body_g, B, 0, io, 0, wt, s_all, s_body, nullptr);
}

struct ResetArgs {
    float* h[6];
    float* c[6];
    long long h_elems[6];
    long long c_elems[6];
    int H[6];
};
__global__ __launch_bounds__(256) void rc_reset_kernel(FrameBuffers fb, ResetArgs a, const unsigned char* mask, int B) {
    const int row = blockIdx.x;
    if (mask && !mask[row]) return;
    for (int n = 0; n < 6; ++n) {
        const int H = a.H[n];
        for (int e = threadIdx.x; e < H; e += 256) {
#pragma unroll
            for (int q = 0; q < 2 * RC_HBUF; ++q) a.h[n][q * a.h_elems[n] + rc_pk(row, e, H)] = 0.0f;
            a.c[n][(long long)row * H + e] = 0.0f;
            a.c[n][a.c_elems[n] + (long long)row * H + e] = 0.0f;
        }
    }
    if (threadIdx.x == 0) {
        fb.has_last[row] = 0;
        fb.n_floor[row] = 0;
        fb.first_reach[row] = 1;
        fb.pend[row] = 0;
    }
}

__global__ void rc_r6d_kernel(const float* r6d, float* R, long long n) {
    const long long i = (long long)blockIdx.x * blockDim.x + threadIdx.x;
    if (i >= n) return;
    float v[6], M[9];
#pragma unroll
    for (int k = 0; k < 6; ++k) v[k] = r6d[6 * i + k];
    r6d_to_R(v, M);
#pragma unroll
    for (int k = 0; k < 9; ++k) R[9 * i + k] = M[k];
}

__global__ void rc_ik_kernel(const BodyConst* __restrict__ body, const float* Rg, float* Rl, long long n) {
    const long long idx = (long long)blockIdx.x * blockDim.x + threadIdx.x;
    const long long b = idx / 24;
    const int j = (int)(idx % 24);
    if (b >= n) return;
    const float* g = Rg + (b * 24 + j) * 9;
    float M[9];
    if (j == 0) {
#pragma unroll
        for (int k = 0; k < 9; ++k) M[k] = g[k];
    } else {
        mat3T_mul(Rg + (b * 24 + body->parent[j]) * 9, g, M);
    }
#pragma unroll
    for (int k = 0; k < 9; ++k) Rl[(b * 24 + j) * 9 + k] = M[k];
}

__global__ __launch_bounds__(64) void rc_fk_bone_kernel(const BodyConst* __restrict__ body, const float* Rg, float* joints, long long n) {
    __shared__ float sR[24][9];
    const long long b = blockIdx.x;
    const int lane = threadIdx.x;
    for (int e = lane; e < 216; e += 64) sR[e / 9][e % 9] = Rg[b * 216 + e];
    __syncthreads();
    if (lane < 24) {
        float o[3];
        bone_chain(body, sR, lane, o);
#pragma unroll
        for (int c = 0; c < 3; ++c) joints[(b * 24 + lane) * 3 + c] = o[c];
    }
}

__global__ __launch_bounds__(64) void rc_body_fk_kernel(const BodyConst* __restrict__ body, const float* pose, const float* tran,
                                                        float* grot, float* joint, float* j33) {
    __shared__ WaveScratch s;
    const long long b = blockIdx.x;
    const int lane = threadIdx.x;
    for (int e = lane; e < 216; e += 64) s.Rl[e / 9][e % 9] = pose[b * 216 + e];
    const float t[3] = {tran[b * 3], tran[b * 3 + 1], tran[b * 3 + 2]};
    __syncthreads();
    wave_body_fk(body, s, t, lane);
    if (grot) for (int e = lane; e < 216; e += 64) grot[b * 216 + e] = s.G[e / 9][e % 9];
    if (lane < 24) {
#pragma unroll
        for (int c = 0; c < 3; ++c) joint[(b * 24 + lane) * 3 + c] = s.P[lane][c] + t[c];
    }
    if (lane < 33) {
#pragma unroll
        for (int c = 0; c < 3; ++c) j33[(b * 33 + lane) * 3 + c] = s.J33[lane][c];
    }
}

__global__ void rc_aa2R_kernel(const float* aa, float* R, long long n) {
    const long long i = (long long)blockIdx.x * blockDim.x + threadIdx.x;
    if (i >= n) return;
    const float a[3] = {aa[3 * i], aa[3 * i + 1], aa[3 * i + 2]};
    const float th = norm3(a);
    float k[3] = {a[0] / th, a[1] / th, a[2] / th};
#pragma unroll
    for (int q = 0; q < 3; ++q) if (!(fabsf(k[q]) <= 3.0e38f)) k[q] = 0.0f;
    const float c = cosf(th), sn = sinf(th), t = 1.0f - c;
    const float K[9] = {0.f, -k[2], k[1], k[2], 0.f, -k[0], -k[1], k[0], 0.f};
#pragma unroll
    for (int r = 0; r < 3; ++r)
#pragma unroll
        for (int q = 0; q < 3; ++q)
            R[9 * i + 3 * r + q] = ((r == q ? c : 0.0f) + t * (k[r] * k[q])) + sn * K[3 * r + q];
}

__global__ void rc_R2aa_kernel(const float* Rm, float* aa, long long n) {
    const long long i = (long long)blockIdx.x * blockDim.x + threadIdx.x;
    if (i >= n) return;
    rotmat_to_aa(Rm + 9 * i, aa + 3 * i);
}

__global__ void rc_camera_inputs_kernel(const float* kp, const float* acc, const float* ori, CamConst cam, float* j2dc,
                                        float* accc, float* oric, long long n) {
    const long long f = blockIdx.x;
    const int t = threadIdx.x;
    if (t < 33) {
        const float u = kp[(f * 33 + t) * 3], v = kp[(f * 33 + t) * 3 + 1], cf = kp[(f * 33 + t) * 3 + 2];
        float* o = j2dc + (f * 33 + t) * 3;
        o[0] = (cam.Kinv[0] * u + cam.Kinv[1] * v) + cam.Kinv[2];
        o[1] = (cam.Kinv[3] * u + cam.Kinv[4] * v) + cam.Kinv[5];
        o[2] = cf;
    } else if (t < 33 + 18) {
        const int e = t - 33, i = e / 3, r = e % 3;
        const float* a = acc + (f * 6 + i) * 3;
        accc[f * 18 + e] = (cam.R[3 * r] * a[0] + cam.R[3 * r + 1] * a[1]) + cam.R[3 * r + 2] * a[2];
    } else if (t < 33 + 18 + 54) {
        const int e = t - 51, i = e / 9, r = (e % 9) / 3, c = e % 3;
        const float* o = ori + (f * 6 + i) * 9;
        oric[f * 54 + e] = (cam.R[3 * r] * o[c] + cam.R[3 * r + 1] * o[3 + c]) + cam.R[3 * r + 2] * o[6 + c];
    }
}

__global__ __launch_bounds__(128) void rc_camera_inputs_rows_kernel(const float* kp, const float* acc, const float* ori,
                                                                    const int* seq_of_row, const int* len, const CamConst* cams,
                                                                    float sx, float sy, int Tmax, float* j2dc, float* accc, float* oric) {
    const long long r = blockIdx.y, f = blockIdx.x;
    const int t = threadIdx.x;
    const long long o = r * Tmax + f, in = (long long)seq_of_row[r] * Tmax + f;
    const bool pad = f >= len[r];
    const CamConst& cam = cams[r];
    if (t < 33) {
        const float* k = kp + (o * 33 + t) * 3;
        float* d = j2dc + (o * 33 + t) * 3;
        const float u = pad ? 0.f : k[0] * sx, v = pad ? 0.f : k[1] * sy;
        d[0] = pad ? 0.f : (cam.Kinv[0] * u + cam.Kinv[1] * v) + cam.Kinv[2];
        d[1] = pad ? 0.f : (cam.Kinv[3] * u + cam.Kinv[4] * v) + cam.Kinv[5];
        d[2] = pad ? 0.f : k[2];
    } else if (t < 33 + 18) {
        const int e = t - 33, i = e / 3, q = e % 3;
        const float* a = acc + (in * 6 + i) * 3;
        accc[o * 18 + e] = pad ? 0.f : (cam.R[3 * q] * a[0] + cam.R[3 * q + 1] * a[1]) + cam.R[3 * q + 2] * a[2];
    } else if (t < 33 + 18 + 54) {
        const int e = t - 51, i = e / 9, q = (e % 9) / 3, c = e % 3;
        const float* m = ori + (in * 6 + i) * 9;
        oric[o * 54 + e] = pad ? (q == c ? 1.f : 0.f) : (cam.R[3 * q] * m[c] + cam.R[3 * q + 1] * m[3 + c]) + cam.R[3 * q + 2] * m[6 + c];
    }
}

__global__ __launch_bounds__(64) void rc_residual_kernel(const BodyConst* __restrict__ body, const float* pose, const float* tran,
                                                         const float* kp, const float* K, float sigma, unsigned long long ign_mask,
                                                         float* loss) {
    __shared__ WaveScratch s;
    const long long b = blockIdx.x;
    const int lane = threadIdx.x;
    for (int e = lane; e < 216; e += 64) s.Rl[e / 9][e % 9] = pose[b * 216 + e];
    const float t[3] = {tran[b * 3], tran[b * 3 + 1], tran[b * 3 + 2]};
    __syncthreads();
    wave_body_fk(body, s, t, lane);
    if (lane < 33) {
        const float z = s.J33[lane][2];
        const float q[3] = {s.J33[lane][0] / z, s.J33[lane][1] / z, z / z};
        const float u = (K[0] * q[0] + K[1] * q[1]) + K[2] * q[2];
        const float v = (K[3] * q[0] + K[4] * q[1]) + K[5] * q[2];
        const float* k3 = kp + (b * 33 + lane) * 3;
        const bool ign = (ign_mask >> lane) & 1ull;
        const float cf = ign ? 0.0f : k3[2];
        const float s2 = sigma * sigma;
        const float dx = u - k3[0], dy = v - k3[1];
        const float ex = (s2 * (dx * dx)) / (s2 + dx * dx), ey = (s2 * (dy * dy)) / (s2 + dy * dy);
        loss[b * 33 + lane] = (cf * cf) * (ex + ey);
    }
}

__global__ void rc_pack_rows_kernel(const float* src, int src_ld, int cols, float* dst, int ld, int B) {
    const long long idx = (long long)blockIdx.x * blockDim.x + threadIdx.x;
    const long long row = idx / cols;
    const int k = (int)(idx % cols);
    if (row >= B) return;
    dst[rc_pk(row, k, ld)] = src[row * src_ld + k];
}

__global__ void rc_flush_flags_kernel(FrameBuffers fb, int B) {
    const int row = blockIdx.x * blockDim.x + threadIdx.x;
    if (row >= B) return;
    fb.flags2[row] = fb.pend[row] ? RC_ROW2_FLUSH : 0;
    fb.pend[row] = 0;
}

__global__ __launch_bounds__(256) void rc_scan_conf_kernel(const float* j2d, long long row_stride, int B, int T, double conf_lo,
                                                          double conf_hi, signed char* codes, float* means, const int* len, int len_t0) {
    const long long item = (long long)blockIdx.x * 4 + (threadIdx.x >> 6);
    const int lane = threadIdx.x & 63;
    if (item >= (long long)B * T) return;
    const int t = (int)(item / B), row = (int)(item % B);
    if (len && len_t0 + t >= len[row]) {
        if (lane == 0 && codes) codes[item] = -1;
        return;
    }
    const float* kp = j2d + row * row_stride + (long long)t * 99;
    const float cf = lane < 33 ? kp[3 * lane + 2] : 0.f;
    const float c = rc_conf_mean33(cf);
    const double c64 = (double)c;
    if (lane == 0 && codes) codes[item] = c64 >= conf_hi ? 2 : (c64 > conf_lo ? 1 : 0);
    if (lane == 0 && means) means[item] = c;
}

struct StepPtrs { int* p[6]; };
__global__ void rc_advance_steps_kernel(StepPtrs sp, int n_frames, int B) {
    const int i = blockIdx.x * blockDim.x + threadIdx.x;
    if (i >= 6 * B) return;
    sp.p[i / B][i % B] += n_frames;
}

static int rc_wave_rows_per_wg() {
    static const int v = [] { const char* e = std::getenv("RC_SEQ_ROWS_PER_WG"); return (e && std::atoi(e) == 1) ? 1 : 4; }();
    return v;
}

void rc_launch_scan_conf(const float* j2d, long long row_stride, int B, int T, double conf_lo, double conf_hi, signed char* codes,
                         hipStream_t st, float* means, const int* len, int len_t0) {
    const long long items = (long long)B * T;
    if (items <= 0) return;
    hipLaunchKernelGGL(rc_scan_conf_kernel, dim3((unsigned)((items + 3) / 4)), dim3(256), 0, st, j2d, row_stride, B, T, conf_lo, conf_hi, codes,
                       means, len, len_t0);
}
void rc_launch_advance_steps(int* const* steps6, int n_frames, int B, hipStream_t st) {
    StepPtrs sp;
    for (int i = 0; i < 6; ++i) sp.p[i] = steps6[i];
    hipLaunchKernelGGL(rc_advance_steps_kernel, dim3((6 * B + 255) / 256), dim3(256), 0, st, sp, n_frames, B);
}
void rc_launch_flush_flags(const FrameBuffers& fb, int B, hipStream_t st) {
    hipLaunchKernelGGL(rc_flush_flags_kernel, dim3((B + 255) / 256), dim3(256), 0, st, fb, B);
}
void rc_launch_pack_rows(const float* src, int src_ld, int cols, float* dst, int ld, int B, hipStream_t st) {
    const long long n = (long long)B * cols;
    hipLaunchKernelGGL(rc_pack_rows_kernel, dim3((unsigned)((n + 255) / 256)), dim3(256), 0, st, src, src_ld, cols, dst, ld, B);
}
void rc_launch_prep(const FrameBuffers& fb, const FrameIO& io, const rc_params_dev& prm, int B, int first_frame, hipStream_t st) {
    hipLaunchKernelGGL(rc_prep_kernel, dim3(B), dim3(64), 0, st, fb, io, prm, B, first_frame);
}
void rc_launch_fuse(const FrameBuffers& fb, const FrameIO& io, const rc_params_dev& prm, int B, hipStream_t st) {
    hipLaunchKernelGGL(rc_fuse_kernel, dim3((B * 24 + 255) / 256), dim3(256), 0, st, fb, io, prm, B);
}
void rc_launch_tail(const FrameBuffers& fb, const FrameIO& io, const rc_params_dev& prm, const BodyConst* body, int B,
                    int first_frame, hipStream_t st, const FrameIO* io_next, const WaveTail* wt, hipEvent_t stop) {
    const WaveTail w = wt ? *wt : WaveTail{};
    const FrameIO nx = io_next ? *io_next : io;
    const int has_next = io_next ? 1 : 0;
    if (w.on && rc_wave_rows_per_wg() == 4) {
        const dim3 g((B + 3) / 4), b(256);
        if (stop) hipExtLaunchKernelGGL(rc_tail_kernel<4>, g, b, 0, st, nullptr, stop, 0, fb, io, prm, body, B, first_frame, nx, has_next, w);
        else hipLaunchKernelGGL(rc_tail_kernel<4>, g, b, 0, st, fb, io, prm, body, B, first_frame, nx, has_next, w);
    } else {
        if (stop) hipExtLaunchKernelGGL(rc_tail_kernel<1>, dim3(B), dim3(64), 0, st, nullptr, stop, 0, fb, io, prm, body, B, first_frame, nx, has_next, w);
        else hipLaunchKernelGGL(rc_tail_kernel<1>, dim3(B), dim3(64), 0, st, fb, io, prm, body, B, first_frame, nx, has_next, w);
    }
}
bool rc_launch_fuse_tail(const FrameBuffers& fb_tail, const FrameBuffers& fb_fuse, const FrameIO& io, const rc_params_dev& prm, const BodyConst* body, int B,
                         const WaveTail& wt, hipStream_t st, hipEvent_t stop) {
    if (rc_wave_rows_per_wg() != 4) return false;
    const int n_tail = (B + 3) / 4, n_fuse = (B * 24 + 255) / 256;
    const dim3 g(n_tail + n_fuse), b(256);
    if (stop) hipExtLaunchKernelGGL(rc_fuse_tail_kernel, g, b, 0, st, nullptr, stop, 0, fb_tail, fb_fuse, io, prm, body, B, wt, n_tail);
    else hipLaunchKernelGGL(rc_fuse_tail_kernel, g, b, 0, st, fb_tail, fb_fuse, io, prm, body, B, wt, n_tail);
    return true;
}
void rc_launch_prep_wave(const FrameBuffers& slot, const FrameIO& io0, const rc_params_dev& prm, int B, const WavePrep& w, hipStream_t st) {
    if (rc_wave_rows_per_wg() == 4) hipLaunchKernelGGL(rc_prep_wave_kernel<4>, dim3((B + 3) / 4), dim3(256), 0, st, slot, io0, prm, B, w);
    else hipLaunchKernelGGL(rc_prep_wave_kernel<1>, dim3(B), dim3(64), 0, st, slot, io0, prm, B, w);
}
void rc_launch_reset(const FrameBuffers& fb, float* const* h, float* const* c, const int* hidden, const unsigned char* mask,
                     int B, hipStream_t st) {
    ResetArgs a;
    const long long Bp = (B + 31) / 32 * 32;
    for (int n = 0; n < 6; ++n) {
        a.h[n] = h[n]; a.c[n] = c[n]; a.H[n] = hidden[n];
        a.h_elems[n] = Bp * hidden[n]; a.c_elems[n] = (long long)B * hidden[n];
    }
    hipLaunchKernelGGL(rc_reset_kernel, dim3(B), dim3(256), 0, st, fb, a, mask, B);
}
void rc_launch_r6d(const float* r6d, float* R, long long n, hipStream_t st) {
    if (n <= 0) return;
    hipLaunchKernelGGL(rc_r6d_kernel, dim3((unsigned)((n + 255) / 256)), dim3(256), 0, st, r6d, R, n);
}
void rc_launch_camera_inputs(const float* kp, const float* acc, const float* ori, const CamConst& cam, float* j2dc, float* accc,
                             float* oric, long long n, hipStream_t st) {
    hipLaunchKernelGGL(rc_camera_inputs_kernel, dim3((unsigned)n), dim3(128), 0, st, kp, acc, ori, cam, j2dc, accc, oric, n);
}
void rc_launch_camera_inputs_rows(const float* kp, const float* acc, const float* ori, const int* seq_of_row, const int* len,
                                  const CamConst* cams, float sx, float sy, int n_rows, int Tmax, float* j2dc, float* accc,
                                  float* oric, hipStream_t st) {
    if (n_rows <= 0 || Tmax <= 0) return;
    hipLaunchKernelGGL(rc_camera_inputs_rows_kernel, dim3((unsigned)Tmax, (unsigned)n_rows), dim3(128), 0, st, kp, acc, ori, seq_of_row,
                       len, cams, sx, sy, Tmax, j2dc, accc, oric);
}
void rc_launch_aa2R(const float* aa, float* R, long long n, hipStream_t st) {
    hipLaunchKernelGGL(rc_aa2R_kernel, dim3((unsigned)((n + 255) / 256)), dim3(256), 0, st, aa, R, n);
}
void rc_launch_R2aa(const float* R, float* aa, long long n, hipStream_t st) {
    hipLaunchKernelGGL(rc_R2aa_kernel, dim3((unsigned)((n + 255) / 256)), dim3(256), 0, st, R, aa, n);
}
void rc_launch_ik(const BodyConst* body, const float* Rg, float* Rl, long long n, hipStream_t st) {
    if (n <= 0) return;
    hipLaunchKernelGGL(rc_ik_kernel, dim3((unsigned)((n * 24 + 255) / 256)), dim3(256), 0, st, body, Rg, Rl, n);
}
void rc_launch_fk_bone(const BodyConst* body, const float* Rg, float* joints, long long n, hipStream_t st) {
    if (n <= 0) return;
    hipLaunchKernelGGL(rc_fk_bone_kernel, dim3((unsigned)n), dim3(64), 0, st, body, Rg, joints, n);
}
void rc_launch_body_fk(const BodyConst* body, const float* pose, const float* tran, float* grot, float* joint, float* j33,
                       long long n, hipStream_t st) {
    if (n <= 0) return;
    hipLaunchKernelGGL(rc_body_fk_kernel, dim3((unsigned)n), dim3(64), 0, st, body, pose, tran, grot, joint, j33);
}
void rc_launch_residual(const BodyConst* body, const float* pose, const float* tran, const float* kp, const float* K, float sigma,
                        unsigned long long ign_mask, float* loss, long long T, hipStream_t st) {
    if (T <= 0) return;
    hipLaunchKernelGGL(rc_residual_kernel, dim3((unsigned)T), dim3(64), 0, st, body, pose, tran, kp, K, sigma, ign_mask, loss);
}
```

### robustcap_amd/csrc/rc_gemm.hip

```cpp
#include "rc_internal.h"
#include <hip/hip_ext.h>
#include <cstdlib>


#ifdef RC_TRACE_TILES
__device__ unsigned long long* g_trace_buf = nullptr;
__device__ unsigned long long g_trace_cap = 0;
extern "C" int rc_trace_tiles_set(unsigned long long* buf, unsigned long long cap_records) {
    if (hipMemcpyToSymbol(HIP_SYMBOL(g_trace_buf), &buf, sizeof(buf)) != hipSuccess) return -1;
    return hipMemcpyToSymbol(HIP_SYMBOL(g_trace_cap), &cap_records, sizeof(cap_records)) == hipSuccess ? 0 : -1;
}
#define TRACE_T(i) do { if (threadIdx.x == 0) trace_t[i] = wall_clock64(); } while (0)
#else
#define TRACE_T(i) do { } while (0)
#endif

#ifndef LDS_PAD
#define LDS_PAD 16
#endif
#define RC_LDS_HEAD 192

#include "rc_gates.h"
#include "rc_mma.h"
__device__ __forceinline__ float sigmoidf_(float x) { return rc_gate_sigmoid(x); }
__device__ __forceinline__ float tanhf_(float x) { return rc_gate_tanh(x); }


template <int MR, int NC, int D, bool PIPE, bool SPLIT = false, bool DEEPOK = true, bool NTW = false, bool W32 = (RC_SPLIT_W32 != 0)>
__device__ __forceinline__ void gemm_tile(const GemmProblem& P, const int B, const int m_tile0, const int n_tile, float* s_mem) {
    constexpr int MT = 16 * MR, NT = 16 * NC, UT = 4 * NC, LD = NT + (MR >= 8 ? 4 : LDS_PAD);
#ifdef RC_TRACE_TILES
    unsigned long long trace_t[4] = {0, 0, 0, 0};
    bool traced = false;
#endif
  for (int m_tile = m_tile0;; m_tile += P.m_tiles) {
    int* s_rows = reinterpret_cast<int*>(s_mem);
    int* s_cnt = s_rows + 128;
    float* s_part = s_mem + RC_LDS_HEAD;
    const int tid = threadIdx.x, lane = tid & 63, wave = tid >> 6;

    TRACE_T(0);
    const int lo = m_tile * MT;
    int nrows;
    if (P.flag_bit == 0) {
        nrows = min(MT, B - lo);
        if (nrows <= 0) return;
        __syncthreads();
        if (tid < MT) s_rows[tid] = lo + min(tid, nrows - 1);
        __syncthreads();
    } else {
        int total = 0;
        __syncthreads();
        for (int base = 0; base < B && total < lo + MT; base += RC_NW * 64) {
            const int r = base + tid;
            const bool f = r < B && (P.flags[r] & P.flag_bit);
            const unsigned long long bal = __ballot(f);
            if (lane == 0) s_cnt[wave] = __popcll(bal);
            __syncthreads();
            int woff = 0, sum = 0;
#pragma unroll
            for (int w = 0; w < RC_NW; ++w) {
                const int cw = s_cnt[w];
                woff += (w < wave) ? cw : 0;
                sum += cw;
            }
            const int idx = total + woff + __popcll(bal & ((1ull << lane) - 1ull));
            if (f && idx >= lo && idx < lo + MT) s_rows[idx - lo] = r;
            total += sum;
            __syncthreads();
        }
        nrows = min(MT, total - lo);
        if (nrows <= 0) return;
        if (tid < MT && tid >= nrows) s_rows[tid] = s_rows[0];
        __syncthreads();
    }
    if (P.open_step && n_tile == 0 && tid < nrows) P.steps[s_rows[tid]] += 1;

    const int i = lane & 15, kq = lane >> 4;
    const float* pa0[MR];
    const float* pa1[MR];
    int row_r[MR], st_r[MR];
#pragma unroll
    for (int r = 0; r < MR; ++r) {
        row_r[r] = s_rows[16 * r + i];
        st_r[r] = (P.seg[0].par_mode | P.seg[1].par_mode) ? P.steps[row_r[r]] : 0;
    }
    FragS<MR, NC, W32> fa = {}, fb = {};
    const int Qs = P.Kp / 32, Qws = Qs / RC_NW;
    constexpr int WPL = W32 ? 2 : 3;
    constexpr int KBU = WPL * 64;
    const long long bs = (long long)Qs * KBU;
    const u32x4* pbs = reinterpret_cast<const u32x4*>(W32 ? (const void*)P.W : P.Ws) + ((long long)(n_tile * NC) * Qs + (long long)wave * Qws) * KBU + lane;
    constexpr bool DEEP = SPLIT && DEEPOK && MR >= 2 && (MR * 8 + NC * 4 * WPL) * 3 + (W32 ? NC * 12 : 0) + MR * NC * 4 <= 380;
    if constexpr (SPLIT) {
        load_kblock_b(fa, pbs, bs);
        if constexpr (DEEP) load_kblock_b(fb, pbs + (long long)min(1, Qws - 1) * KBU, bs);
    }
#pragma unroll
    for (int r = 0; r < MR; ++r) {
        const int row = row_r[r];
        const int st = st_r[r] + ((P.seg[0].par_mode | P.seg[1].par_mode) ? P.step_off : 0);
        const float* pp[2];
#pragma unroll
        for (int sgi = 0; sgi < 2; ++sgi) {
            const GemmSeg& sg = P.seg[sgi];
            const int par = sg.par_mode == RC_PAR_SRC ? ((st - 1) % RC_HBUF) : (sg.par_mode == RC_PAR_DST ? (st % RC_HBUF) : 0);
            const float* base = sg.base;
            if (sgi == 0 && P.sel_bit && !(P.sel_flags[row] & P.sel_bit)) base = P.alt_base;
            pp[sgi] = base + (long long)par * sg.par_stride + rc_pk(row, 4 * kq, sg.ld);
        }
        pa0[r] = pp[0];
        pa1[r] = pp[1];
    }
    const int Q = P.Kp / RC_KC, Qw = Q / RC_NW;
    const int K0 = P.seg[0].K;
    const long long bstride = (long long)Q * 256;
    const float* pb = P.W + ((long long)(n_tile * NC) * Q + (long long)wave * Qw) * 256 + lane * 4;
    const int kbase = wave * Qw * RC_KC;

    TRACE_T(1);
    f32x4 acc[MR][NC];
#pragma unroll
    for (int r = 0; r < MR; ++r)
#pragma unroll
        for (int j = 0; j < NC; ++j) acc[r][j] = f32x4{0.f, 0.f, 0.f, 0.f};
#define LOADC(F, QI)                                                                                      \
    do {                                                                                                  \
        const int k_ = kbase + (QI) * RC_KC;                                                              \
        if (k_ < K0) load_chunk<MR, NC, NTW>(F, pa0, (long long)k_ * 16, pb + (long long)(QI) * 256, bstride);  \
        else load_chunk<MR, NC, NTW>(F, pa1, (long long)(k_ - K0) * 16, pb + (long long)(QI) * 256, bstride);   \
    } while (0)
#define SB() do { if (PIPE) __builtin_amdgcn_sched_barrier(0); } while (0)
    if constexpr (SPLIT) {
        const int kb0 = wave * Qws * 32;
#define LOADS_A(F, QI)                                                                                              \
    do {                                                                                                            \
        const int k_ = kb0 + (QI) * 32;                                                                             \
        if (k_ < K0) load_kblock_a(F, pa0, (long long)k_ * 16);                                        \
        else load_kblock_a(F, pa1, (long long)(k_ - K0) * 16);                                              \
    } while (0)
#define LOADS(F, QI)                                                                                                \
    do {                                                                                                            \
        const int k_ = kb0 + (QI) * 32;                                                                             \
        if (k_ < K0) load_kblock(F, pa0, (long long)k_ * 16, pbs + (long long)(QI) * KBU, bs);              \
        else load_kblock(F, pa1, (long long)(k_ - K0) * 16, pbs + (long long)(QI) * KBU, bs);               \
    } while (0)
        int q = 0;
#define STEP(FL, QL, FM) do { LOADS(FL, QL); SB(); mma_kblock(FM, acc); SB(); } while (0)
        if constexpr (DEEP) {
            FragS<MR, NC, W32> fc = {};
            LOADS_A(fa, 0);
            LOADS_A(fb, min(1, Qws - 1));
            for (; q + 3 <= Qws; q += 3) {
                STEP(fc, min(q + 2, Qws - 1), fa);
                STEP(fa, min(q + 3, Qws - 1), fb);
                STEP(fb, min(q + 4, Qws - 1), fc);
            }
            if (q < Qws) mma_kblock(fa, acc);
            if (q + 1 < Qws) mma_kblock(fb, acc);
        } else {
            LOADS_A(fa, 0);
            for (; q + 2 <= Qws; q += 2) {
                STEP(fb, min(q + 1, Qws - 1), fa);
                STEP(fa, min(q + 2, Qws - 1), fb);
            }
            if (q < Qws) mma_kblock(fa, acc);
        }
#undef STEP
#undef LOADS_A
#undef LOADS
    } else if constexpr (D == 2) {
        Frag<MR, NC> fa = {}, fb = {};
        int q = 0;
        LOADC(fa, 0);
        for (; q + 2 < Qw; q += 2) {
            LOADC(fb, q + 1);
            SB();
            mma_chunk<MR, NC>(fa, acc);
            SB();
            LOADC(fa, q + 2);
            SB();
            mma_chunk<MR, NC>(fb, acc);
            SB();
        }
        LOADC(fb, q + 1);
        SB();
        mma_chunk<MR, NC>(fa, acc);
        SB();
        mma_chunk<MR, NC>(fb, acc);
    } else {
        Frag<MR, NC> f[D];
    #pragma unroll
        for (int d = 0; d < D; ++d) f[d] = Frag<MR, NC>{};
    #pragma unroll
        for (int d = 0; d < D - 1; ++d) LOADC(f[d], min(d, Qw - 1));
        int q = 0;
        for (; q + D <= Qw; q += D) {
    #pragma unroll
            for (int d = 0; d < D; ++d) {
                LOADC(f[(d + D - 1) % D], min(q + d + D - 1, Qw - 1));
                SB();
                mma_chunk<MR, NC>(f[d], acc);
                SB();
            }
        }
        const int rem = Qw - q;
    #pragma unroll
        for (int d = 0; d < D - 1; ++d)
            if (d < rem) mma_chunk<MR, NC>(f[d], acc);
    }
#undef LOADC
#undef SB

    TRACE_T(2);
    constexpr int EPI_ITEMS = (MT * UT + RC_NW * 64 - 1) / (RC_NW * 64);
    float c_prev[EPI_ITEMS];
    int st_row[EPI_ITEMS];
    constexpr bool BIAS_ONE = (RC_NW * 64) % UT == 0;
    f32x4 bias4 = f32x4{0.f, 0.f, 0.f, 0.f};
    if (P.epi == RC_EPI_LSTM) {
#pragma unroll
        for (int k = 0; k < EPI_ITEMS; ++k) {
            const int item = tid + k * RC_NW * 64;
            const int rr = item / UT, u = item - rr * UT;
            const bool ok = item < MT * UT && rr < nrows;
            const int r2 = s_rows[ok ? rr : 0];
            c_prev[k] = ok ? P.cstate[(long long)r2 * P.H + n_tile * UT + u] : 0.f;
            st_row[k] = ok ? P.steps[r2] : 0;
        }
    }
#pragma unroll
    for (int r = 0; r < MR; ++r)
#pragma unroll
        for (int j = 0; j < NC; ++j)
#pragma unroll
            for (int e = 0; e < 4; ++e)
                s_part[(wave * MT + 16 * r + 4 * kq + e) * LD + 16 * j + i] = acc[r][j][e];
    if (P.epi == RC_EPI_LSTM) {
        if constexpr (BIAS_ONE) bias4 = *reinterpret_cast<const f32x4*>(&P.bias[n_tile * NT + 4 * (tid % UT)]);
    }
    __syncthreads();

    if (P.epi == RC_EPI_LSTM) {
#pragma unroll
        for (int k = 0; k < EPI_ITEMS; ++k) {
            const int item = tid + k * RC_NW * 64;
            const int rr = item / UT, u = item - rr * UT;
            if (item >= MT * UT || rr >= nrows) continue;
            const int unit = n_tile * UT + u;
            static_assert(RC_NW == 4, "the reduction order below names the four K quarters");
            f32x4 g4 = (*reinterpret_cast<const f32x4*>(&s_part[rr * LD + 4 * u]) + *reinterpret_cast<const f32x4*>(&s_part[(MT + rr) * LD + 4 * u])) +
                       (*reinterpret_cast<const f32x4*>(&s_part[(2 * MT + rr) * LD + 4 * u]) + *reinterpret_cast<const f32x4*>(&s_part[(3 * MT + rr) * LD + 4 * u]));
            if constexpr (BIAS_ONE) g4 += bias4; else g4 += *reinterpret_cast<const f32x4*>(&P.bias[n_tile * NT + 4 * u]);
            const int r2 = s_rows[rr];
            const int dst = (st_row[k] + P.step_off) % RC_HBUF;
            const long long ci = (long long)r2 * P.H + unit;
            float cn, hn;
            rc_lstm_cell(g4[0], g4[1], g4[2], g4[3], c_prev[k], cn, hn);
            P.cstate[ci] = cn;
            P.hstate[(long long)dst * P.h_par_stride + rc_pk(r2, unit, P.H)] = hn;
        }
    } else {
        const bool vec4 = P.out_packed && P.out_bit == 0 && ((P.out_col0 | P.N) & 3) == 0;
        if (vec4) {
            constexpr int V4_ITEMS = (MT * (NT / 4) + RC_NW * 64 - 1) / (RC_NW * 64);
            constexpr bool B4_ONE = (RC_NW * 64) % (NT / 4) == 0;
            f32x4 b4 = f32x4{0.f, 0.f, 0.f, 0.f};
            if constexpr (B4_ONE) b4 = *reinterpret_cast<const f32x4*>(&P.bias[n_tile * NT + (tid % (NT / 4)) * 4]);
#pragma unroll
            for (int k = 0; k < V4_ITEMS; ++k) {
                const int item = tid + k * RC_NW * 64;
                const int rr = item / (NT / 4), c4 = (item - rr * (NT / 4)) * 4;
                const int n = n_tile * NT + c4;
                if (item >= MT * (NT / 4) || rr >= nrows || n >= P.N) continue;
                f32x4 v = *reinterpret_cast<const f32x4*>(&s_part[rr * LD + c4]);
#pragma unroll
                for (int w = 1; w < RC_NW; ++w) v += *reinterpret_cast<const f32x4*>(&s_part[(w * MT + rr) * LD + c4]);
                if constexpr (B4_ONE) v += b4; else v += *reinterpret_cast<const f32x4*>(&P.bias[n]);
                if (P.epi == RC_EPI_RELU) { v[0] = fmaxf(v[0], 0.0f); v[1] = fmaxf(v[1], 0.0f); v[2] = fmaxf(v[2], 0.0f); v[3] = fmaxf(v[3], 0.0f); }
                *reinterpret_cast<f32x4*>(&P.out[rc_pk(s_rows[rr], P.out_col0 + n, P.ldo)]) = v;
            }
        } else
        for (int item = tid; item < MT * NT; item += RC_NW * 64) {
            const int rr = item / NT, col = item - rr * NT;
            if (rr >= nrows) continue;
            const int n = n_tile * NT + col;
            float v = s_part[rr * LD + col];
#pragma unroll
            for (int w = 1; w < RC_NW; ++w) v += s_part[(w * MT + rr) * LD + col];
            v += P.bias[n];
            if (P.epi == RC_EPI_RELU) v = fmaxf(v, 0.0f);
            const int r2 = s_rows[rr];
            if (n < P.N && (P.out_bit == 0 || (P.out_flags[r2] & P.out_bit))) {
                P.out[P.out_packed ? rc_pk(r2, P.out_col0 + n, P.ldo) : (long long)r2 * P.ldo + P.out_col0 + n] = v;
            }
        }
    }
#ifdef RC_TRACE_TILES
    if (threadIdx.x == 0 && !traced && g_trace_buf) {
        traced = true;
        const unsigned long long idx = (unsigned long long)P.trace_base + blockIdx.x;
        if (idx < g_trace_cap) {
            unsigned long long* r = g_trace_buf + idx * 8;
            r[0] = (unsigned long long)blockIdx.x + 1; r[1] = (unsigned long long)(MR * 16 + NC) | ((unsigned long long)nrows << 16);
            r[2] = __smid(); r[3] = (unsigned long long)n_tile | ((unsigned long long)m_tile << 32);
            r[4] = trace_t[0]; r[5] = trace_t[1]; r[6] = trace_t[2]; r[7] = wall_clock64();
        }
    }
#endif
  }
}

#ifndef RC_LDS_FLOATS
#define RC_LDS_FLOATS (RC_LDS_HEAD + RC_NW * 64 * (16 * 8 + LDS_PAD))
#endif

#ifndef RC_WPS
#define RC_WPS 1
#endif
__device__ __forceinline__ bool locate_tile(const GemmLaunch& L, int& pi, int& m_tile, int& n_tile) {
    pi = 0;
#pragma unroll
    for (int q = 1; q < RC_MAX_PROB; ++q)
        if (q < L.n && (int)blockIdx.x >= L.p[q].wg_base) pi = q;
    const GemmProblem& P = L.p[pi];
    const int local = blockIdx.x - P.wg_base;
    if ((P.n_tiles & 7) == 0) {
        const int xcd = local & 7, s = local >> 3;
        m_tile = s % P.m_tiles;
        n_tile = (s / P.m_tiles) * 8 + xcd;
    } else {
        m_tile = local % P.m_tiles;
        n_tile = local / P.m_tiles;
    }
    return n_tile < P.n_tiles;
}

template <bool SPLIT>
__device__ __forceinline__ void wide_tiles(const GemmLaunch& L, float* s_mem) {
    int pi, m_tile, n_tile;
    if (!locate_tile(L, pi, m_tile, n_tile)) return;
    const GemmProblem& P = L.p[pi];
    switch (P.mr * 16 + P.nc) {
        case 8 * 16 + 4: gemm_tile<8, 4, 2, true, SPLIT>(P, L.B, m_tile, n_tile, s_mem); break;
        case 4 * 16 + 8: gemm_tile<4, 8, 2, true, SPLIT>(P, L.B, m_tile, n_tile, s_mem); break;
        case 4 * 16 + 5: gemm_tile<4, 5, 2, true, SPLIT>(P, L.B, m_tile, n_tile, s_mem); break;
        case 4 * 16 + 4: gemm_tile<4, 4, 2, true, SPLIT>(P, L.B, m_tile, n_tile, s_mem); break;
        case 2 * 16 + 10: gemm_tile<2, 10, 2, true, SPLIT>(P, L.B, m_tile, n_tile, s_mem); break;
        case 2 * 16 + 8: gemm_tile<2, 8, 2, true, SPLIT>(P, L.B, m_tile, n_tile, s_mem); break;
        case 1 * 16 + 2: gemm_tile<1, 2, 8, true, SPLIT>(P, L.B, m_tile, n_tile, s_mem); break;
        case 1 * 16 + 1: gemm_tile<1, 1, 8, true, SPLIT>(P, L.B, m_tile, n_tile, s_mem); break;
        default: gemm_tile<2, 4, 2, true, SPLIT>(P, L.B, m_tile, n_tile, s_mem); break;
    }
}

__global__ __launch_bounds__(RC_NW * 64, RC_WPS) void rc_gemm_kernel(const GemmLaunch L) {
    __shared__ __attribute__((aligned(16))) float s_mem[RC_LDS_FLOATS];
    wide_tiles<false>(L, s_mem);
}
__global__ __launch_bounds__(RC_NW * 64, RC_WPS) void rc_gemm_split_kernel(const GemmLaunch L) {
    __shared__ __attribute__((aligned(16))) float s_mem[RC_LDS_FLOATS];
    wide_tiles<true>(L, s_mem);
}

__global__ __launch_bounds__(RC_NW * 64, RC_WPS) void rc_gemm_split48_w32_kernel(const GemmLaunch L) {
    __shared__ __attribute__((aligned(16))) float s_mem[RC_LDS_FLOATS];
    int pi, m_tile, n_tile;
    if (!locate_tile(L, pi, m_tile, n_tile)) return;
    gemm_tile<4, 8, 2, true, true, true, false, true>(L.p[pi], L.B, m_tile, n_tile, s_mem);
}

#define RC_MID_LDS_FLOATS (RC_LDS_HEAD + RC_NW * 32 * (16 * 4 + LDS_PAD))
template <bool SPLIT>
__device__ __forceinline__ void mid_tiles(const GemmLaunch& L, float* s_mem) {
    int pi, m_tile, n_tile;
    if (!locate_tile(L, pi, m_tile, n_tile)) return;
    const GemmProblem& P = L.p[pi];
    switch (P.mr * 16 + P.nc) {
        case 1 * 16 + 2: gemm_tile<1, 2, 8, true, SPLIT>(P, L.B, m_tile, n_tile, s_mem); break;
        case 1 * 16 + 1: gemm_tile<1, 1, 8, true, SPLIT>(P, L.B, m_tile, n_tile, s_mem); break;
        default: gemm_tile<2, 4, 2, true, SPLIT, false>(P, L.B, m_tile, n_tile, s_mem); break;
    }
}
__global__ __launch_bounds__(RC_NW * 64, 2) void rc_gemm_mid_kernel(const GemmLaunch L) {
    __shared__ __attribute__((aligned(16))) float s_mem[RC_MID_LDS_FLOATS];
    mid_tiles<false>(L, s_mem);
}
__global__ __launch_bounds__(RC_NW * 64, 2) void rc_gemm_mid_split_kernel(const GemmLaunch L) {
    __shared__ __attribute__((aligned(16))) float s_mem[RC_MID_LDS_FLOATS];
    mid_tiles<true>(L, s_mem);
}

#define RC_SMALL_LDS_FLOATS (RC_LDS_HEAD + RC_NW * 16 * (16 * 2 + LDS_PAD))
template <bool SPLIT, bool NTW = false>
__device__ __forceinline__ void small_tiles(const GemmLaunch& L, float* s_mem) {
    int pi, m_tile, n_tile;
    if (!locate_tile(L, pi, m_tile, n_tile)) return;
    const GemmProblem& P = L.p[pi];
    if constexpr (NTW) {
        if (P.nc == 2) gemm_tile<1, 2, 4, true, SPLIT, true, true>(P, L.B, m_tile, n_tile, s_mem);
        else if (P.nt) gemm_tile<1, 1, 8, true, SPLIT, true, true>(P, L.B, m_tile, n_tile, s_mem);
        else gemm_tile<1, 1, 8, true, SPLIT, true, false>(P, L.B, m_tile, n_tile, s_mem);
    } else {
        if (P.nc == 2) gemm_tile<1, 2, 4, true, SPLIT, true, false>(P, L.B, m_tile, n_tile, s_mem);
        else gemm_tile<1, 1, 8, true, SPLIT, true, false>(P, L.B, m_tile, n_tile, s_mem);
    }
}
__global__ __launch_bounds__(RC_NW * 64, 4) void rc_gemm_small_kernel(const GemmLaunch L) {
    __shared__ __attribute__((aligned(16))) float s_mem[RC_SMALL_LDS_FLOATS];
    small_tiles<false>(L, s_mem);
}
__global__ __launch_bounds__(RC_NW * 64, 4) void rc_gemm_small_nt_kernel(const GemmLaunch L) {
    __shared__ __attribute__((aligned(16))) float s_mem[RC_SMALL_LDS_FLOATS];
    small_tiles<false, true>(L, s_mem);
}
__global__ __launch_bounds__(RC_NW * 64, 4) void rc_gemm_small_split_kernel(const GemmLaunch L) {
    __shared__ __attribute__((aligned(16))) float s_mem[RC_SMALL_LDS_FLOATS];
    small_tiles<true>(L, s_mem);
}

bool rc_gemm_is_small(const GemmLaunch& L) {
    bool small = true;
    for (int q = 0; q < L.n; ++q) small = small && L.p[q].mr == 1 && L.p[q].nc <= 2;
    return small;
}

bool rc_gemm_is_mid(const GemmLaunch& L) {
    bool mid = true;
    for (int q = 0; q < L.n; ++q) mid = mid && L.p[q].mr <= 2 && L.p[q].nc <= 4 && !(L.p[q].mr == 2 && L.p[q].nc < 4);
    return mid;
}

bool rc_gemm_is_w32(const GemmLaunch& L) {
    if (rc_gemm_is_small(L) || rc_gemm_is_mid(L)) return false;
    bool one_reader = L.split != 0;
    for (int q = 0; q < L.n; ++q) one_reader = one_reader && L.p[q].mr == 4 && L.p[q].nc == 8 && L.p[q].m_tiles == 1;
    static const bool w32 = !std::getenv("RC_GEMM_W32") || std::atoi(std::getenv("RC_GEMM_W32")) != 0;
    return one_reader && w32;
}

void rc_launch_gemm(const GemmLaunch& L, int total_wg, hipStream_t s, hipEvent_t stop) {
    const dim3 g(total_wg), b(RC_NW * 64);
#define RC_GO(K) do { if (stop) hipExtLaunchKernelGGL(K, g, b, 0, s, nullptr, stop, 0, L); else hipLaunchKernelGGL(K, g, b, 0, s, L); } while (0)
    if (rc_gemm_is_small(L)) {
        bool single_reader = L.live != 0;
        for (int q = 0; q < L.n; ++q) single_reader = single_reader && L.p[q].m_tiles == 1;
        if (L.split) RC_GO(rc_gemm_small_split_kernel);
        else if (single_reader) RC_GO(rc_gemm_small_nt_kernel);
        else RC_GO(rc_gemm_small_kernel);
    } else if (rc_gemm_is_mid(L)) {
        if (L.split) RC_GO(rc_gemm_mid_split_kernel);
        else RC_GO(rc_gemm_mid_kernel);
    } else {
        if (rc_gemm_is_w32(L)) RC_GO(rc_gemm_split48_w32_kernel);
        else if (L.split) RC_GO(rc_gemm_split_kernel);
        else RC_GO(rc_gemm_kernel);
    }
#undef RC_GO
}
```

### robustcap_amd/csrc/rc_internal.h

```cpp
#pragma once
#include <hip/hip_runtime.h>
#include <stdint.h>
#include <memory>
#include <string>
#include <type_traits>

#define RC_MT 32
#define RC_NT 64
#ifndef RC_NW
#define RC_NW 4
#endif
#define RC_KC 16
#define RC_KALIGN 128
#define RC_HBUF 3
#define RC_MAX_PROB 14

__host__ __device__ inline long long rc_pk(long long row, int k, int ld) {
    return (row >> 4) * (16ll * ld) + (long long)(k >> 4) * 256 + ((k >> 2) & 3) * 64 + (row & 15) * 4 + (k & 3);
}

enum { RC_EPI_DENSE = 0, RC_EPI_RELU = 1, RC_EPI_LSTM = 2 };
enum { RC_PAR_NONE = 0, RC_PAR_SRC = 1, RC_PAR_DST = 2 };

#define RC_ROW_VIS 1u
// ... 91 lines not shown
struct ResidentArgs {
    const ResidentTick* ticks;
    const int* item_base;
    int n_ticks;
    int* head;
    int* done;
    int* tick_done;
    const int* flag_tail;
    int* abort;
    unsigned long long spin_bound;
};
void rc_launch_gemm_resident(const ResidentArgs& R, int workgroups, hipStream_t s);
void rc_launch_flag_set(int* flag, int value, hipStream_t s);
void rc_launch_flag_wait(const int* counter, int target, int* abort, unsigned long long spin_bound, hipStream_t s);

struct BodyConst {
    int parent[24];
    int level[24];
    float bone[24][3];
    float jrest[24][3];
    float jroot[3];
    float w33[33][24];
    float v33[33][3];
    int override_joint[33];
    int nchild[24];
    int child[24][4];
};

struct FrameBuffers {
    float *x2, *x3, *x4, *x6, *x78, *x4l, *x6l, *xi;
    float *vr, *pc, *r6d, *contact;
    float *init_out;
    unsigned char* flags;
    unsigned char* flags2;
    unsigned char* pend;
    unsigned char* regime;
    double* kconf;
    float* gravity;
    float *last_pfoot, *last_tran, *floor, *j_temp;
    int *has_last, *n_floor, *first_reach, *uv_count;
    int* trace;
    float *h2, *c2;
    int* steps2;
    long long h2_par_stride, h2_layer_stride, c2_layer_stride;
    int* frame;
    int* wsteps;
};

struct WavePrep {
    const int* frame_at;
    int* steps[6];
    const float *cx4l, *cx6l;
    int first_tick;
    int t0;
};
struct WaveTail {
    int on;
    int t_last;
    float *x4l, *x6l;
    unsigned char* flags2;
    int* wsteps;
    int *steps4, *steps6;
    float *cx4l, *cx6l;
};

struct FrameIO {
    const float *j2d, *acc, *ori, *first_tran;
    float *pose_out, *tran_out;
    long long s_j2d, s_acc, s_ori, s_pose, s_tran;
    const int* len;
    int t;
};
__host__ __device__ inline bool rc_row_live(const FrameIO& io, int row, int t) { return !io.len || t < io.len[row]; }

struct rc_params_dev {
    double conf_lo, conf_hi, tran_filter_num;
    float contact_threshold, distance_threshold, height_threshold;
    int use_flat_floor, use_vision_updater, use_imu_updater, live, update_vision_freq, use_reproj_opt;
    float smooth;
};

#define RC_LIVE_MAXB 4
struct LiveGrid { int hot; int st[4][RC_LIVE_MAXB]; int act[4][RC_LIVE_MAXB]; int pre; int pre_base; const float* prebuf; };
struct LiveNet {
    const float *W1, *b1;
    const float *Wl[2], *bl[2];
    const float *W2, *b2;
    float *x1, *h, *c, *part;
    int* steps;
    int H, out, outp, Kp1;
    long long BpH;
};
struct LiveFrame {
    LiveNet net[6];
    FrameBuffers fb;
    FrameIO io;
    rc_params_dev prm;
    const BodyConst* body;
    int* status;
    int* abort;
    unsigned* spin_mb;
    unsigned* spin_state;
    LiveGrid* hot[4];
    unsigned* done_flag;
    unsigned* done_seq;
    int B;
    int nc;
};
#define RC_LIVE_KERNELS 7
struct LiveKernel {
    const void* fn;
    const char* name;
    unsigned grid;
    int has_grid;
    unsigned wg;
    LiveFrame F;
    LiveGrid G;
};
int rc_live_plan(const LiveFrame& F, LiveKernel* out, const float* prebuf = nullptr);
int rc_live_pre_plan(const LiveFrame& F, float* prebuf, LiveKernel* out);
long long rc_live_pre_floats(const LiveFrame& F);
void rc_launch_live_frame(const LiveFrame& F, hipStream_t s, const float* prebuf = nullptr);
void rc_launch_live_pre(const LiveFrame& F, float* prebuf, hipStream_t s);

struct AqlChain;
int rc_aql_create(int hip_device, AqlChain** out, char* err, int err_len);
int rc_aql_add(AqlChain* c, const LiveKernel* k, int n, int frame, char* err, int err_len);
int rc_aql_run(AqlChain* c, int prog);
int rc_aql_submit(AqlChain* c, int prog);
int rc_aql_alloc_shared(AqlChain* c, size_t bytes, void** ptr);
int rc_aql_submit_ahead(AqlChain* c, int prog, int beside);
unsigned long long rc_aql_seq(const AqlChain* c);
int rc_aql_wait_seq(AqlChain* c, unsigned long long seq);
int rc_aql_wait_frame(AqlChain* c);
int rc_aql_fence_background(AqlChain* c);
void rc_aql_set_mailbox(AqlChain* c, volatile unsigned* mb);
int rc_aql_arm(AqlChain* c);
int rc_aql_wait_background(AqlChain* c);
void rc_aql_destroy(AqlChain* c);

void rc_launch_gemm(const GemmLaunch& L, int total_wg, hipStream_t s, hipEvent_t stop = nullptr);
void rc_launch_scan_conf(const float* j2d, long long row_stride, int B, int T, double conf_lo, double conf_hi, signed char* codes, hipStream_t s,
                         float* means = nullptr, const int* len = nullptr, int len_t0 = 0);
void rc_launch_advance_steps(int* const* steps6, int n_frames, int B, hipStream_t s);
bool rc_gemm_is_w32(const GemmLaunch& L);
bool rc_gemm_is_small(const GemmLaunch& L);
void rc_launch_prep(const FrameBuffers& fb, const FrameIO& io, const rc_params_dev& prm, int B, int first_frame, hipStream_t s);
void rc_launch_fuse(const FrameBuffers& fb, const FrameIO& io, const rc_params_dev& prm, int B, hipStream_t s);
void rc_launch_tail(const FrameBuffers& fb, const FrameIO& io, const rc_params_dev& prm, const BodyConst* body, int B,
                    int first_frame, hipStream_t s, const FrameIO* io_next = nullptr,
                    const WaveTail* wt = nullptr, hipEvent_t stop = nullptr);
bool rc_launch_fuse_tail(const FrameBuffers& fb_tail, const FrameBuffers& fb_fuse, const FrameIO& io, const rc_params_dev& prm, const BodyConst* body, int B,
                         const WaveTail& wt, hipStream_t s, hipEvent_t stop);
void rc_launch_prep_wave(const FrameBuffers& slot, const FrameIO& io0, const rc_params_dev& prm, int B, const WavePrep& w, hipStream_t s);
void rc_launch_reset(const FrameBuffers& fb, float* const* h, float* const* c, const int* hidden, const unsigned char* mask,
                     int B, hipStream_t s);

void rc_launch_flush_flags(const FrameBuffers& fb, int B, hipStream_t s);
void rc_launch_pack_rows(const float* src, int src_ld, int cols, float* dst, int ld, int B, hipStream_t s);

void rc_launch_r6d(const float* r6d, float* R, long long n, hipStream_t s);
struct CamConst { float Kinv[9]; float R[9]; };
void rc_launch_camera_inputs(const float* kp, const float* acc, const float* ori, const CamConst& cam, float* j2dc, float* accc,
                             float* oric, long long n, hipStream_t s);
void rc_launch_shape_body(const float* vt, const float* sd, const float* beta, const float* Jr, int V, float* v, float* j, hipStream_t s);
void rc_launch_fk_r(const BodyConst* body, const float* Rl, float* Rg, long long n, hipStream_t s);
void rc_launch_bone_to_joint(const BodyConst* body, const float* bone, float* joint, long long n, hipStream_t s);
void rc_launch_joint_to_bone(const BodyConst* body, const float* joint, float* bone, long long n, hipStream_t s);
void rc_launch_zero_pose(const BodyConst* body, const float* vt, int V, float* joint, float* vert, hipStream_t s);
void rc_launch_rotmat_to_r6d(const float* R, float* r6d, long long n, hipStream_t s);
void rc_launch_lerp(const float* a, const float* b, float w1, float w2, float* out, long long n, hipStream_t s);
void rc_launch_normalize_rows(const float* x, float* out, float* norm, long long rows, int width, hipStream_t s);
void rc_launch_angle_between(const float* R1, const float* R2, float* out, long long n, hipStream_t s);
void rc_launch_bbox_normalise(const float* kp, float* out, long long n, hipStream_t s);
void rc_launch_camera_inputs_rows(const float* kp, const float* acc, const float* ori, const int* seq_of_row, const int* len,
                                  const CamConst* cams, float sx, float sy, int n_rows, int Tmax, float* j2dc, float* accc,
                                  float* oric, hipStream_t s);
void rc_launch_aa2R(const float* aa, float* R, long long n, hipStream_t s);
void rc_launch_R2aa(const float* R, float* aa, long long n, hipStream_t s);
void rc_launch_ik(const BodyConst* body, const float* Rg, float* Rl, long long n, hipStream_t s);
void rc_launch_fk_bone(const BodyConst* body, const float* Rg, float* joints, long long n, hipStream_t s);
void rc_launch_body_fk(const BodyConst* body, const float* pose, const float* tran, float* grot, float* joint,
                       float* j33, long long n, hipStream_t s);
void rc_launch_body_mesh(const BodyConst* body, const float* vt, const float* w, int V, const float* pose, const float* tran,
                         float* vert, long long n, float* scratch, hipStream_t s);
long long rc_body_mesh_scratch_floats(long long n);
void rc_launch_residual(const BodyConst* body, const float* pose, const float* tran, const float* kp, const float* K,
                        float sigma, unsigned long long ign_mask, float* loss, long long T, hipStream_t s);
#define RC_IGN_DEFAULT 0x1800003FEull
void rc_launch_mesh_metrics(const BodyConst* body, const float* vt, const float* w, int V, const float* kM, int nk, const float* pose_p,
                            const float* pose_t, float* out, long long n, float* scratch, hipStream_t s);
long long rc_mesh_metrics_scratch_floats(int V, long long n);
void rc_launch_imu_frames(const BodyConst* body, const float* vt, const float* w, const int* vid, const int* jid, const float* pose,
                          const float* tran, float* ori, float* joint, float* vert6, long long T, hipStream_t s);
void rc_launch_syn_acc(const float* v, float* acc, long long T, long long width, int n, hipStream_t s);
void rc_launch_procrustes(const float* S1, const float* S2, int nk, float* err, long long n, hipStream_t s);
void rc_launch_point_distance(const float* a, const float* b, float* d, long long n, hipStream_t s);

struct SmplifyArgs {
    const float* aa;
    const float* tran;
    const float* kp;
    const float* ref3d;
    const float* imu_aa;
    const float* means;
    const float* prec;
    const float* prec_sym;
    const float* lognll;
    float* mj;
    float* proj;
    float* frame_loss;
    float* imu_loss;
    float* smooth_loss;
    int* argmin;
    float* prior_ll;
    float* prior_g;
    float* fk;
    float* grad_aa;
    float* grad_tran;
    float K[9];
    unsigned long long ign_mask;
    int T;
};
void rc_launch_smplify(const SmplifyArgs& A, const BodyConst* body, hipStream_t s);
#define RC_LBFGS_MAX_PAIRS 100
struct VecComb { const float* v[2 * RC_LBFGS_MAX_PAIRS + 1]; float c[2 * RC_LBFGS_MAX_PAIRS + 1]; int n_vec; };
struct VecJob { const float* a; const float* b; int op; int pad_; };
struct VecOp { const float* a; const float* b; const float* c; float* out; float* out2; float t; int kind; long long n; };
struct VecCombRow { VecComb c; float* out; long long n; };
struct VecJobN { const float* a; const float* b; int op; int pad_; long long n; };
void rc_launch_smplify_rows(const SmplifyArgs* rows_dev, int n_rows, int T_max, const BodyConst* body, hipStream_t s);
void rc_launch_smplify_totals(const SmplifyArgs* rows_dev, int n_rows, double* out_dev, hipStream_t s);
struct SmplifyRowIO {
    const float* pose;
    const float* tran;
    const float* kp;
    const float* imu_ori;
    float* x;
    float* imu_aa;
    float* joint;
    float* ref3d;
    float* res0;
    float* res1;
    float* pose_out;
    float* tran_out;
    float K[9];
    int T;
    int live;
};
void rc_launch_smplify_begin_rows(const SmplifyRowIO* rows_dev, int n_rows, int T_max, const BodyConst* body, float sigma,
                                  unsigned long long ign_mask, hipStream_t s);
void rc_launch_smplify_end_rows(const SmplifyRowIO* rows_dev, int n_rows, int T_max, const BodyConst* body, float sigma,
                                unsigned long long ign_mask, hipStream_t s);
void rc_launch_vec_ops(const VecOp* ops_dev, int n_ops, long long n_max, hipStream_t s);
void rc_launch_vec_comb_rows(const VecCombRow* rows_dev, int n_rows, long long n_max, hipStream_t s);
void rc_launch_vec_dots_rows(const VecJobN* jobs_dev, int n_jobs, int nb_max, double* partial, hipStream_t s);
void rc_launch_vec_axpy(const float* x, const float* d, float t, float* out, long long n, hipStream_t s);
void rc_launch_vec_pair(const float* g_new, const float* g_old, const float* d, float t, float* y, float* sv, long long n, hipStream_t s);
void rc_launch_vec_comb(const VecComb& c, float* out, long long n, hipStream_t s);
void rc_launch_vec_dots(const VecJob* jobs_dev, int n_jobs, long long n, double* partial, hipStream_t s);

template <auto Release> struct RcRelease { template <class P> void operator()(P p) const { (void)Release(p); } };
template <class T> using DevBuf = std::unique_ptr<T[], RcRelease<hipFree>>;
template <class T> using PinBuf = std::unique_ptr<T[], RcRelease<hipHostFree>>;
using HipStream = std::unique_ptr<std::remove_pointer_t<hipStream_t>, RcRelease<hipStreamDestroy>>;
using HipEvent = std::unique_ptr<std::remove_pointer_t<hipEvent_t>, RcRelease<hipEventDestroy>>;
using HipGraph = std::unique_ptr<std::remove_pointer_t<hipGraph_t>, RcRelease<hipGraphDestroy>>;
using HipGraphExec = std::unique_ptr<std::remove_pointer_t<hipGraphExec_t>, RcRelease<hipGraphExecDestroy>>;

template <class Own> struct RcOut {
    Own& own;
    typename Own::pointer raw;
    ~RcOut() { own.reset(raw); }
    operator typename Own::pointer*() { return &raw; }
};
template <class Own> RcOut<Own> rc_out(Own& own) { own.reset(); return {own, nullptr}; }

template <class T> hipError_t rc_alloc(DevBuf<T>& p, size_t n) {
    p.reset();
    void* q = nullptr;
    const hipError_t e = hipMalloc(&q, n * sizeof(T));
    p.reset(static_cast<T*>(q));
    return e;
}
template <class T> hipError_t rc_alloc(PinBuf<T>& p, size_t n, unsigned flags = hipHostMallocDefault) {
    p.reset();
    void* q = nullptr;
    const hipError_t e = hipHostMalloc(&q, n * sizeof(T), flags);
    p.reset(static_cast<T*>(q));
    return e;
}
inline hipError_t rc_alloc_all() { return hipSuccess; }
template <class Buf, class... Rest> hipError_t rc_alloc_all(Buf& p, size_t n, Rest&&... rest) {
    const hipError_t e = rc_alloc(p, n);
    return e != hipSuccess ? e : rc_alloc_all(rest...);
}
template <class Cap, class... BufsAndCounts> hipError_t rc_grow(Cap& cap, size_t need, size_t want, BufsAndCounts&&... bc) {
    if (need <= (size_t)cap) return hipSuccess;
    cap = 0;
    const hipError_t e = rc_alloc_all(bc...);
    if (e == hipSuccess) cap = (Cap)want;
    return e;
}

struct rc_ctx;
struct SmplifyState;
// ... 49 lines not shown
```

Measured before the change: 1.266 million body-frames/s.

## Fold second-linear-layer GEMMs into the fused fuse/tail wave kernel

Adds a kernel that, per wave tick, runs the small lin2 GEMM tiles for a 12-row block of bodies and then runs the tail or fuse stage for the same rows. This replaces the separate lin2 GEMM launch plus fuse/tail launches with a single launch. The gemm_tile device code moves into a shared header so the frame kernel can call it, with three GEMM teams per 768-thread block. The cost is a large block with LDS reuse between the GEMM and tail phases, and lower GEMM parallelism per row block. It falls back to the old path when timing modes are active or the problems do not fit.

```diff
diff --git a/include/robustcap_hip.h b/include/robustcap_hip.h
--- a/include/robustcap_hip.h
+++ b/include/robustcap_hip.h
@@ -81,6 +81,8 @@
 int rc_plan_wave_rows(const int8_t* codes, int32_t B, int32_t T, int32_t t0, const int32_t* len, const int32_t* first_reach,
                       const int32_t* pend, int32_t use_imu_updater, int32_t use_vision_updater, int32_t* frame_at, int64_t frame_at_cap,
                       int32_t* n_ticks, int32_t* n_prep, int32_t* counts, double* est_us);
+int rc_plan_lin2_fold(const int32_t* n_valid, int32_t n_prep, int32_t n_ticks, uint8_t* fold);
+int rc_get_lin2_fold_stats(rc_ctx* ctx, int64_t* folds, int64_t* lin2_launches);
 
 int rc_live_begin(rc_ctx* ctx);
 int rc_live_step(rc_ctx* ctx, const float* j2dc_host, const float* accc_host, const float* oric_host,
diff --git a/robustcap_amd/_lib.py b/robustcap_amd/_lib.py
--- a/robustcap_amd/_lib.py
+++ b/robustcap_amd/_lib.py
@@ -59,6 +59,8 @@
     "rc_plan_sequence": (_I32, [_P, _I32, _I32, _P, _U32, _I32, _P]),
     "rc_plan_wave": (_I32, [_P, _I32, _I32, _I32, _P, _P, _I32, _I32, _P, _I64, C.POINTER(_I32), C.POINTER(_I32), _P, _P]),
     "rc_plan_wave_rows": (_I32, [_P, _I32, _I32, _I32, _P, _P, _P, _I32, _I32, _P, _I64, C.POINTER(_I32), C.POINTER(_I32), _P, _P]),
+    "rc_plan_lin2_fold": (_I32, [_P, _I32, _I32, _P]),
+    "rc_get_lin2_fold_stats": (_I32, [_P, C.POINTER(_I64), C.POINTER(_I64)]),
     "rc_live_begin": (_I32, [_P]),
     "rc_live_step": (_I32, [_P, _P, _P, _P, _P, _U32, _P, _P]),
     "rc_live_end": (_I32, [_P]),
diff --git a/robustcap_amd/csrc/rc_api.cpp b/robustcap_amd/csrc/rc_api.cpp
--- a/robustcap_amd/csrc/rc_api.cpp
+++ b/robustcap_amd/csrc/rc_api.cpp
@@ -184,6 +184,7 @@
     SmplifyOwner smplify;
     SubnetOwner subnet;
     int trace_next = 0;
+    long long stat_lin2_folds = 0, stat_lin2_launches = 0;
     long long stat_wide_launches = 0;
     int lds_min_rows = 64;
     int lds_min_batch = 65;
@@ -1094,16 +1095,40 @@
     rc_launch_prep_wave(S.ctx->ring2[k % kRing], S.io0, S.prm, S.ctx->B, S.wp, S.aux);
 }
 
+inline bool lin2_fold_tick(bool fuse, bool tail) { return fuse || tail; }
+inline bool lin2_launch_timed(const rc_ctx* ctx) { return ctx->timing && ctx->timing_mode != 3 && ctx->timing_mode != 2; }
+
 int wave_lin2_fuse_tail(WaveSeg& S, int k, bool merge, hipEvent_t signal) {
     rc_ctx* ctx = S.ctx;
     const int B = ctx->B;
-    if (int rc = launch_problems(ctx, S.group(k, G_LIN2), nullptr, S.aux, true)) return rc;
     const bool fuse = S.rows(S.P.n_valid, k - kFuseStage) > 0, tail = S.rows(S.P.n_valid, k - kTailStage) > 0;
     bool merged = false, carried = false;
     if (tail) {
         const FrameBuffers& tgt = ctx->ring2[k % kRing];
         S.wt.x4l = tgt.x4l; S.wt.x6l = tgt.x6l; S.wt.flags2 = tgt.flags2; S.wt.wsteps = tgt.wsteps;
     }
+    const std::vector<GemmProblem> lin2 = S.group(k, G_LIN2);
+    if (fuse || tail) {
+        const FrameBuffers& tail_slot = ctx->ring2[(k - kTailStage + kRing) % kRing];
+        GemmProblem ps[RC_TICK_PROB];
+        int n_tail = 0, n_fuse = 0;
+        for (int side = 0; side < 2; ++side)
+            for (const GemmProblem& p : lin2) {
+                const bool of_tail = p.steps >= tail_slot.wsteps && p.steps < tail_slot.wsteps + 6 * (size_t)B;
+                if (of_tail != (side == 0) || !(of_tail ? tail : fuse)) continue;
+                ps[n_tail + n_fuse] = p;
+                ++(of_tail ? n_tail : n_fuse);
+            }
+        if (lin2_fold_tick(fuse, tail) && !lin2_launch_timed(ctx) && (n_tail > 0) == tail && (n_fuse > 0) == fuse &&
+            rc_launch_lin2_fuse_tail(ps, n_tail, n_fuse, tail_slot, ctx->ring2[(k - kFuseStage + kRing) % kRing], S.io0, S.prm, ctx->body, B,
+                                     S.wt, S.aux, signal)) {
+            HIP_TRY(ctx, hipGetLastError());
+            ctx->stat_lin2_folds += 1;
+            return RC_OK;
+        }
+    }
+    if (!lin2.empty()) ctx->stat_lin2_launches += 1;
+    if (int rc = launch_problems(ctx, lin2, nullptr, S.aux, true)) return rc;
     if (merge && fuse && tail)
         merged = carried = rc_launch_fuse_tail(ctx->ring2[(k - kTailStage) % kRing], ctx->ring2[(k - kFuseStage) % kRing], S.io0, S.prm, ctx->body, B, S.wt, S.aux, signal);
     if (!merged && fuse) rc_launch_fuse(ctx->ring2[(k - kFuseStage) % kRing], S.io0, S.prm, B, S.aux);
@@ -1966,6 +1991,20 @@
             counts[k] = P.n_valid[k]; counts[P.n_prep + k] = P.n_vis[k];
             counts[2 * P.n_prep + k] = P.n_rider[k]; counts[3 * P.n_prep + k] = P.n_reach[k];
         }
+    return RC_OK;
+}
+
+int rc_plan_lin2_fold(const int32_t* n_valid, int32_t n_prep, int32_t n_ticks, uint8_t* fold) {
+    if (!n_valid || !fold || n_prep < 0 || n_ticks < 0) return RC_ERR_INVALID;
+    auto rows = [&](int tick) { return tick >= 0 && tick < n_prep ? n_valid[tick] : 0; };
+    for (int k = 0; k < n_ticks; ++k) fold[k] = lin2_fold_tick(rows(k - kFuseStage) > 0, rows(k - kTailStage) > 0) ? 1 : 0;
+    return RC_OK;
+}
+
+int rc_get_lin2_fold_stats(rc_ctx* ctx, int64_t* folds, int64_t* lin2_launches) {
+    if (!ctx) return RC_ERR_INVALID;
+    if (folds) *folds = ctx->stat_lin2_folds;
+    if (lin2_launches) *lin2_launches = ctx->stat_lin2_launches;
     return RC_OK;
 }
 
diff --git a/robustcap_amd/csrc/rc_frame.hip b/robustcap_amd/csrc/rc_frame.hip
--- a/robustcap_amd/csrc/rc_frame.hip
+++ b/robustcap_amd/csrc/rc_frame.hip
@@ -4,6 +4,10 @@
 
 #include "rc_device.h"
 #include "rc_frame_dev.h"
+#ifdef RC_TRACE_TILES
+#undef RC_TRACE_TILES
+#endif
+#include "rc_gemm_tile.h"
 
 __global__ __launch_bounds__(64) void rc_prep_kernel(FrameBuffers fb, FrameIO io, rc_params_dev prm, int B, int first_frame) {
     const int row = blockIdx.x;
@@ -111,6 +115,56 @@
         return;
     }
     tail_impl<4, false>(fb_tail, io, prm, body_g, B, 0, io, 0, wt, s_all, s_body, nullptr);
+}
+
+#define RC_L2F_ROWS 12
+#define RC_L2F_TEAMS 3
+struct Lin2Fold {
+    int n_tail, n_fuse;
+    GemmProblem p[RC_LIN2_FOLD_MAXP];
+};
+constexpr size_t kL2fGemmBytes = sizeof(float) * RC_L2F_TEAMS * RC_TILE16_LDS_FLOATS;
+constexpr size_t kL2fTailBytes = sizeof(WaveScratch) * RC_L2F_ROWS + sizeof(BodyConst);
+static_assert(sizeof(WaveScratch) % 16 == 0 || (sizeof(WaveScratch) * RC_L2F_ROWS) % 16 == 0, "BodyConst behind the scratch rows stays 16-byte aligned");
+__global__ __launch_bounds__(256 * RC_L2F_TEAMS) void rc_lin2_fuse_tail_kernel(FrameBuffers fb_tail, FrameBuffers fb_fuse, FrameIO io, rc_params_dev prm,
+                                                                               const BodyConst* __restrict__ body_g, int B, WaveTail wt, int n_tail_blocks,
+                                                                               const Lin2Fold L) {
+    __shared__ __attribute__((aligned(16))) unsigned char s_raw[kL2fGemmBytes > kL2fTailBytes ? kL2fGemmBytes : kL2fTailBytes];
+    __shared__ int s_live[4], s_list[4 * 16], s_n;
+    const bool tail_side = (int)blockIdx.x < n_tail_blocks;
+    const int blk = tail_side ? (int)blockIdx.x : (int)blockIdx.x - n_tail_blocks;
+    const int p0 = tail_side ? 0 : L.n_tail, np = tail_side ? L.n_tail : L.n_fuse;
+    const int tid = threadIdx.x, wave = tid >> 6, lane = tid & 63;
+    if (wave < np) {
+        const GemmProblem& P = L.p[p0 + wave];
+        const int r = blk * RC_L2F_ROWS + lane;
+        const bool f = lane < RC_L2F_ROWS && r < B && (P.flag_bit == 0 || (P.flags[r] & P.flag_bit));
+        const unsigned long long bal = __ballot(f);
+        if (lane == 0) s_live[wave] = bal != 0ull;
+    }
+    __syncthreads();
+    if (tid == 0) {
+        int n = 0;
+        for (int q = 0; q < np; ++q)
+            if (s_live[q]) for (int t = 0; t < L.p[p0 + q].n_tiles; ++t) s_list[n++] = (q << 8) | t;
+        s_n = n;
+    }
+    __syncthreads();
+    const int n = s_n, team = tid >> 8;
+    float* s_mem = reinterpret_cast<float*>(s_raw) + team * RC_TILE16_LDS_FLOATS;
+    for (int base = 0; base < n; base += RC_L2F_TEAMS) {
+        const bool dead = base + team >= n;
+        const int e = s_list[dead ? 0 : base + team];
+        gemm_tile<1, 1, 8, true, false, true, false, (RC_SPLIT_W32 != 0), RC_L2F_ROWS>(L.p[p0 + (e >> 8)], B, blk, e & 255, s_mem, dead);
+    }
+    __syncthreads();
+    if (tail_side) {
+        WaveScratch* s_all = reinterpret_cast<WaveScratch*>(s_raw);
+        BodyConst& s_body = *reinterpret_cast<BodyConst*>(s_raw + sizeof(WaveScratch) * RC_L2F_ROWS);
+        tail_impl<RC_L2F_ROWS, false>(fb_tail, io, prm, body_g, B, 0, io, 0, wt, s_all, s_body, nullptr);
+    } else if (tid < RC_L2F_ROWS * 24) {
+        fuse_body(fb_fuse, io, prm, B, blk * (RC_L2F_ROWS * 24) + tid);
+    }
 }
 
 struct ResetArgs {
@@ -390,6 +444,19 @@
     else hipLaunchKernelGGL(rc_fuse_tail_kernel, g, b, 0, st, fb_tail, fb_fuse, io, prm, body, B, wt, n_tail);
     return true;
 }
+bool rc_launch_lin2_fuse_tail(const GemmProblem* ps, int n_tail, int n_fuse, const FrameBuffers& fb_tail, const FrameBuffers& fb_fuse, const FrameIO& io,
+                              const rc_params_dev& prm, const BodyConst* body, int B, const WaveTail& wt, hipStream_t st, hipEvent_t stop) {
+    if (!rc_lin2_fold_covers(ps, n_tail, n_fuse) || rc_wave_rows_per_wg() != 4) return false;
+    Lin2Fold L{};
+    L.n_tail = n_tail; L.n_fuse = n_fuse;
+    for (int i = 0; i < n_tail + n_fuse; ++i) L.p[i] = ps[i];
+    const int blocks = (B + RC_L2F_ROWS - 1) / RC_L2F_ROWS;
+    const int n_tail_blocks = n_tail > 0 ? blocks : 0, n_fuse_blocks = n_fuse > 0 ? blocks : 0;
+    const dim3 g(n_tail_blocks + n_fuse_blocks), b(256 * RC_L2F_TEAMS);
+    if (stop) hipExtLaunchKernelGGL(rc_lin2_fuse_tail_kernel, g, b, 0, st, nullptr, stop, 0, fb_tail, fb_fuse, io, prm, body, B, wt, n_tail_blocks, L);
+    else hipLaunchKernelGGL(rc_lin2_fuse_tail_kernel, g, b, 0, st, fb_tail, fb_fuse, io, prm, body, B, wt, n_tail_blocks, L);
+    return true;
+}
 void rc_launch_prep_wave(const FrameBuffers& slot, const FrameIO& io0, const rc_params_dev& prm, int B, const WavePrep& w, hipStream_t st) {
     if (rc_wave_rows_per_wg() == 4) hipLaunchKernelGGL(rc_prep_wave_kernel<4>, dim3((B + 3) / 4), dim3(256), 0, st, slot, io0, prm, B, w);
     else hipLaunchKernelGGL(rc_prep_wave_kernel<1>, dim3(B), dim3(64), 0, st, slot, io0, prm, B, w);
diff --git a/robustcap_amd/csrc/rc_gemm.hip b/robustcap_amd/csrc/rc_gemm.hip
--- a/robustcap_amd/csrc/rc_gemm.hip
+++ b/robustcap_amd/csrc/rc_gemm.hip
@@ -10,306 +10,9 @@
     if (hipMemcpyToSymbol(HIP_SYMBOL(g_trace_buf), &buf, sizeof(buf)) != hipSuccess) return -1;
     return hipMemcpyToSymbol(HIP_SYMBOL(g_trace_cap), &cap_records, sizeof(cap_records)) == hipSuccess ? 0 : -1;
 }
-#define TRACE_T(i) do { if (threadIdx.x == 0) trace_t[i] = wall_clock64(); } while (0)
-#else
-#define TRACE_T(i) do { } while (0)
 #endif
 
-#ifndef LDS_PAD
-#define LDS_PAD 16
-#endif
-#define RC_LDS_HEAD 192
-
-#include "rc_gates.h"
-#include "rc_mma.h"
-__device__ __forceinline__ float sigmoidf_(float x) { return rc_gate_sigmoid(x); }
-__device__ __forceinline__ float tanhf_(float x) { return rc_gate_tanh(x); }
-
-
-template <int MR, int NC, int D, bool PIPE, bool SPLIT = false, bool DEEPOK = true, bool NTW = false, bool W32 = (RC_SPLIT_W32 != 0)>
-__device__ __forceinline__ void gemm_tile(const GemmProblem& P, const int B, const int m_tile0, const int n_tile, float* s_mem) {
-    constexpr int MT = 16 * MR, NT = 16 * NC, UT = 4 * NC, LD = NT + (MR >= 8 ? 4 : LDS_PAD);
-#ifdef RC_TRACE_TILES
-    unsigned long long trace_t[4] = {0, 0, 0, 0};
-    bool traced = false;
-#endif
-  for (int m_tile = m_tile0;; m_tile += P.m_tiles) {
-    int* s_rows = reinterpret_cast<int*>(s_mem);
-    int* s_cnt = s_rows + 128;
-    float* s_part = s_mem + RC_LDS_HEAD;
-    const int tid = threadIdx.x, lane = tid & 63, wave = tid >> 6;
-
-    TRACE_T(0);
-    const int lo = m_tile * MT;
-    int nrows;
-    if (P.flag_bit == 0) {
-        nrows = min(MT, B - lo);
-        if (nrows <= 0) return;
-        __syncthreads();
-        if (tid < MT) s_rows[tid] = lo + min(tid, nrows - 1);
-        __syncthreads();
-    } else {
-        int total = 0;
-        __syncthreads();
-        for (int base = 0; base < B && total < lo + MT; base += RC_NW * 64) {
-            const int r = base + tid;
-            const bool f = r < B && (P.flags[r] & P.flag_bit);
-            const unsigned long long bal = __ballot(f);
-            if (lane == 0) s_cnt[wave] = __popcll(bal);
-            __syncthreads();
-            int woff = 0, sum = 0;
-#pragma unroll
-            for (int w = 0; w < RC_NW; ++w) {
-                const int cw = s_cnt[w];
-                woff += (w < wave) ? cw : 0;
-                sum += cw;
-            }
-            const int idx = total + woff + __popcll(bal & ((1ull << lane) - 1ull));
-            if (f && idx >= lo && idx < lo + MT) s_rows[idx - lo] = r;
-            total += sum;
-            __syncthreads();
-        }
-        nrows = min(MT, total - lo);
-        if (nrows <= 0) return;
-        if (tid < MT && tid >= nrows) s_rows[tid] = s_rows[0];
-        __syncthreads();
-    }
-    if (P.open_step && n_tile == 0 && tid < nrows) P.steps[s_rows[tid]] += 1;
-
-    const int i = lane & 15, kq = lane >> 4;
-    const float* pa0[MR];
-    const float* pa1[MR];
-    int row_r[MR], st_r[MR];
-#pragma unroll
-    for (int r = 0; r < MR; ++r) {
-        row_r[r] = s_rows[16 * r + i];
-        st_r[r] = (P.seg[0].par_mode | P.seg[1].par_mode) ? P.steps[row_r[r]] : 0;
-    }
-    FragS<MR, NC, W32> fa = {}, fb = {};
-    const int Qs = P.Kp / 32, Qws = Qs / RC_NW;
-    constexpr int WPL = W32 ? 2 : 3;
-    constexpr int KBU = WPL * 64;
-    const long long bs = (long long)Qs * KBU;
-    const u32x4* pbs = reinterpret_cast<const u32x4*>(W32 ? (const void*)P.W : P.Ws) + ((long long)(n_tile * NC) * Qs + (long long)wave * Qws) * KBU + lane;
-    constexpr bool DEEP = SPLIT && DEEPOK && MR >= 2 && (MR * 8 + NC * 4 * WPL) * 3 + (W32 ? NC * 12 : 0) + MR * NC * 4 <= 380;
-    if constexpr (SPLIT) {
-        load_kblock_b(fa, pbs, bs);
-        if constexpr (DEEP) load_kblock_b(fb, pbs + (long long)min(1, Qws - 1) * KBU, bs);
-    }
-#pragma unroll
-    for (int r = 0; r < MR; ++r) {
-        const int row = row_r[r];
-        const int st = st_r[r] + ((P.seg[0].par_mode | P.seg[1].par_mode) ? P.step_off : 0);
-        const float* pp[2];
-#pragma unroll
-        for (int sgi = 0; sgi < 2; ++sgi) {
-            const GemmSeg& sg = P.seg[sgi];
-            const int par = sg.par_mode == RC_PAR_SRC ? ((st - 1) % RC_HBUF) : (sg.par_mode == RC_PAR_DST ? (st % RC_HBUF) : 0);
-            const float* base = sg.base;
-            if (sgi == 0 && P.sel_bit && !(P.sel_flags[row] & P.sel_bit)) base = P.alt_base;
-            pp[sgi] = base + (long long)par * sg.par_stride + rc_pk(row, 4 * kq, sg.ld);
-        }
-        pa0[r] = pp[0];
-        pa1[r] = pp[1];
-    }
-    const int Q = P.Kp / RC_KC, Qw = Q / RC_NW;
-    const int K0 = P.seg[0].K;
-    const long long bstride = (long long)Q * 256;
-    const float* pb = P.W + ((long long)(n_tile * NC) * Q + (long long)wave * Qw) * 256 + lane * 4;
-    const int kbase = wave * Qw * RC_KC;
-
-    TRACE_T(1);
-    f32x4 acc[MR][NC];
-#pragma unroll
-    for (int r = 0; r < MR; ++r)
-#pragma unroll
-        for (int j = 0; j < NC; ++j) acc[r][j] = f32x4{0.f, 0.f, 0.f, 0.f};
-#define LOADC(F, QI)                                                                                      \
-    do {                                                                                                  \
-        const int k_ = kbase + (QI) * RC_KC;                                                              \
-        if (k_ < K0) load_chunk<MR, NC, NTW>(F, pa0, (long long)k_ * 16, pb + (long long)(QI) * 256, bstride);  \
-        else load_chunk<MR, NC, NTW>(F, pa1, (long long)(k_ - K0) * 16, pb + (long long)(QI) * 256, bstride);   \
-    } while (0)
-#define SB() do { if (PIPE) __builtin_amdgcn_sched_barrier(0); } while (0)
-    if constexpr (SPLIT) {
-        const int kb0 = wave * Qws * 32;
-#define LOADS_A(F, QI)                                                                                              \
-    do {                                                                                                            \
-        const int k_ = kb0 + (QI) * 32;                                                                             \
-        if (k_ < K0) load_kblock_a(F, pa0, (long long)k_ * 16);                                        \
-        else load_kblock_a(F, pa1, (long long)(k_ - K0) * 16);                                              \
-    } while (0)
-#define LOADS(F, QI)                                                                                                \
-    do {                                                                                                            \
-        const int k_ = kb0 + (QI) * 32;                                                                             \
-        if (k_ < K0) load_kblock(F, pa0, (long long)k_ * 16, pbs + (long long)(QI) * KBU, bs);              \
-        else load_kblock(F, pa1, (long long)(k_ - K0) * 16, pbs + (long long)(QI) * KBU, bs);               \
-    } while (0)
-        int q = 0;
-#define STEP(FL, QL, FM) do { LOADS(FL, QL); SB(); mma_kblock(FM, acc); SB(); } while (0)
-        if constexpr (DEEP) {
-            FragS<MR, NC, W32> fc = {};
-            LOADS_A(fa, 0);
-            LOADS_A(fb, min(1, Qws - 1));
-            for (; q + 3 <= Qws; q += 3) {
-                STEP(fc, min(q + 2, Qws - 1), fa);
-                STEP(fa, min(q + 3, Qws - 1), fb);
-                STEP(fb, min(q + 4, Qws - 1), fc);
-            }
-            if (q < Qws) mma_kblock(fa, acc);
-            if (q + 1 < Qws) mma_kblock(fb, acc);
-        } else {
-            LOADS_A(fa, 0);
-            for (; q + 2 <= Qws; q += 2) {
-                STEP(fb, min(q + 1, Qws - 1), fa);
-                STEP(fa, min(q + 2, Qws - 1), fb);
-            }
-            if (q < Qws) mma_kblock(fa, acc);
-        }
-#undef STEP
-#undef LOADS_A
-#undef LOADS
-    } else if constexpr (D == 2) {
-        Frag<MR, NC> fa = {}, fb = {};
-        int q = 0;
-        LOADC(fa, 0);
-        for (; q + 2 < Qw; q += 2) {
-            LOADC(fb, q + 1);
-            SB();
-            mma_chunk<MR, NC>(fa, acc);
-            SB();
-            LOADC(fa, q + 2);
-            SB();
-            mma_chunk<MR, NC>(fb, acc);
-            SB();
-        }
-        LOADC(fb, q + 1);
-        SB();
-        mma_chunk<MR, NC>(fa, acc);
-        SB();
-        mma_chunk<MR, NC>(fb, acc);
-    } else {
-        Frag<MR, NC> f[D];
-    #pragma unroll
-        for (int d = 0; d < D; ++d) f[d] = Frag<MR, NC>{};
-    #pragma unroll
-        for (int d = 0; d < D - 1; ++d) LOADC(f[d], min(d, Qw - 1));
-        int q = 0;
-        for (; q + D <= Qw; q += D) {
-    #pragma unroll
-            for (int d = 0; d < D; ++d) {
-                LOADC(f[(d + D - 1) % D], min(q + d + D - 1, Qw - 1));
-                SB();
-                mma_chunk<MR, NC>(f[d], acc);
-                SB();
-            }
-        }
-        const int rem = Qw - q;
-    #pragma unroll
-        for (int d = 0; d < D - 1; ++d)
-            if (d < rem) mma_chunk<MR, NC>(f[d], acc);
-    }
-#undef LOADC
-#undef SB
-
-    TRACE_T(2);
-    constexpr int EPI_ITEMS = (MT * UT + RC_NW * 64 - 1) / (RC_NW * 64);
-    float c_prev[EPI_ITEMS];
-    int st_row[EPI_ITEMS];
-    constexpr bool BIAS_ONE = (RC_NW * 64) % UT == 0;
-    f32x4 bias4 = f32x4{0.f, 0.f, 0.f, 0.f};
-    if (P.epi == RC_EPI_LSTM) {
-#pragma unroll
-        for (int k = 0; k < EPI_ITEMS; ++k) {
-            const int item = tid + k * RC_NW * 64;
-            const int rr = item / UT, u = item - rr * UT;
-            const bool ok = item < MT * UT && rr < nrows;
-            const int r2 = s_rows[ok ? rr : 0];
-            c_prev[k] = ok ? P.cstate[(long long)r2 * P.H + n_tile * UT + u] : 0.f;
-            st_row[k] = ok ? P.steps[r2] : 0;
-        }
-    }
-#pragma unroll
-    for (int r = 0; r < MR; ++r)
-#pragma unroll
-        for (int j = 0; j < NC; ++j)
-#pragma unroll
-            for (int e = 0; e < 4; ++e)
-                s_part[(wave * MT + 16 * r + 4 * kq + e) * LD + 16 * j + i] = acc[r][j][e];
-    if (P.epi == RC_EPI_LSTM) {
-        if constexpr (BIAS_ONE) bias4 = *reinterpret_cast<const f32x4*>(&P.bias[n_tile * NT + 4 * (tid % UT)]);
-    }
-    __syncthreads();
-
-    if (P.epi == RC_EPI_LSTM) {
-#pragma unroll
-        for (int k = 0; k < EPI_ITEMS; ++k) {
-            const int item = tid + k * RC_NW * 64;
-            const int rr = item / UT, u = item - rr * UT;
-            if (item >= MT * UT || rr >= nrows) continue;
-            const int unit = n_tile * UT + u;
-            static_assert(RC_NW == 4, "the reduction order below names the four K quarters");
-            f32x4 g4 = (*reinterpret_cast<const f32x4*>(&s_part[rr * LD + 4 * u]) + *reinterpret_cast<const f32x4*>(&s_part[(MT + rr) * LD + 4 * u])) +
-                       (*reinterpret_cast<const f32x4*>(&s_part[(2 * MT + rr) * LD + 4 * u]) + *reinterpret_cast<const f32x4*>(&s_part[(3 * MT + rr) * LD + 4 * u]));
-            if constexpr (BIAS_ONE) g4 += bias4; else g4 += *reinterpret_cast<const f32x4*>(&P.bias[n_tile * NT + 4 * u]);
-            const int r2 = s_rows[rr];
-            const int dst = (st_row[k] + P.step_off) % RC_HBUF;
-            const long long ci = (long long)r2 * P.H + unit;
-            float cn, hn;
-            rc_lstm_cell(g4[0], g4[1], g4[2], g4[3], c_prev[k], cn, hn);
-            P.cstate[ci] = cn;
-            P.hstate[(long long)dst * P.h_par_stride + rc_pk(r2, unit, P.H)] = hn;
-        }
-    } else {
-        const bool vec4 = P.out_packed && P.out_bit == 0 && ((P.out_col0 | P.N) & 3) == 0;
-        if (vec4) {
-            constexpr int V4_ITEMS = (MT * (NT / 4) + RC_NW * 64 - 1) / (RC_NW * 64);
-            constexpr bool B4_ONE = (RC_NW * 64) % (NT / 4) == 0;
-            f32x4 b4 = f32x4{0.f, 0.f, 0.f, 0.f};
-            if constexpr (B4_ONE) b4 = *reinterpret_cast<const f32x4*>(&P.bias[n_tile * NT + (tid % (NT / 4)) * 4]);
-#pragma unroll
-            for (int k = 0; k < V4_ITEMS; ++k) {
-                const int item = tid + k * RC_NW * 64;
-                const int rr = item / (NT / 4), c4 = (item - rr * (NT / 4)) * 4;
-                const int n = n_tile * NT + c4;
-                if (item >= MT * (NT / 4) || rr >= nrows || n >= P.N) continue;
-                f32x4 v = *reinterpret_cast<const f32x4*>(&s_part[rr * LD + c4]);
-#pragma unroll
-                for (int w = 1; w < RC_NW; ++w) v += *reinterpret_cast<const f32x4*>(&s_part[(w * MT + rr) * LD + c4]);
-                if constexpr (B4_ONE) v += b4; else v += *reinterpret_cast<const f32x4*>(&P.bias[n]);
-                if (P.epi == RC_EPI_RELU) { v[0] = fmaxf(v[0], 0.0f); v[1] = fmaxf(v[1], 0.0f); v[2] = fmaxf(v[2], 0.0f); v[3] = fmaxf(v[3], 0.0f); }
-                *reinterpret_cast<f32x4*>(&P.out[rc_pk(s_rows[rr], P.out_col0 + n, P.ldo)]) = v;
-            }
-        } else
-        for (int item = tid; item < MT * NT; item += RC_NW * 64) {
-            const int rr = item / NT, col = item - rr * NT;
-            if (rr >= nrows) continue;
-            const int n = n_tile * NT + col;
-            float v = s_part[rr * LD + col];
-#pragma unroll
-            for (int w = 1; w < RC_NW; ++w) v += s_part[(w * MT + rr) * LD + col];
-            v += P.bias[n];
-            if (P.epi == RC_EPI_RELU) v = fmaxf(v, 0.0f);
-            const int r2 = s_rows[rr];
-            if (n < P.N && (P.out_bit == 0 || (P.out_flags[r2] & P.out_bit))) {
-                P.out[P.out_packed ? rc_pk(r2, P.out_col0 + n, P.ldo) : (long long)r2 * P.ldo + P.out_col0 + n] = v;
-            }
-        }
-    }
-#ifdef RC_TRACE_TILES
-    if (threadIdx.x == 0 && !traced && g_trace_buf) {
-        traced = true;
-        const unsigned long long idx = (unsigned long long)P.trace_base + blockIdx.x;
-        if (idx < g_trace_cap) {
-            unsigned long long* r = g_trace_buf + idx * 8;
-            r[0] = (unsigned long long)blockIdx.x + 1; r[1] = (unsigned long long)(MR * 16 + NC) | ((unsigned long long)nrows << 16);
-            r[2] = __smid(); r[3] = (unsigned long long)n_tile | ((unsigned long long)m_tile << 32);
-            r[4] = trace_t[0]; r[5] = trace_t[1]; r[6] = trace_t[2]; r[7] = wall_clock64();
-        }
-    }
-#endif
-  }
-}
+#include "rc_gemm_tile.h"
 
 #ifndef RC_LDS_FLOATS
 #define RC_LDS_FLOATS (RC_LDS_HEAD + RC_NW * 64 * (16 * 8 + LDS_PAD))
diff --git a/robustcap_amd/csrc/rc_gemm_tile.h b/robustcap_amd/csrc/rc_gemm_tile.h
--- /dev/null
+++ b/robustcap_amd/csrc/rc_gemm_tile.h
@@ -0,0 +1,318 @@
+#pragma once
+#include "rc_internal.h"
+
+#ifdef RC_TRACE_TILES
+#define TRACE_T(i) do { if (threadIdx.x == 0) trace_t[i] = wall_clock64(); } while (0)
+#else
+#define TRACE_T(i) do { } while (0)
+#endif
+
+#ifndef LDS_PAD
+#define LDS_PAD 16
+#endif
+#define RC_LDS_HEAD 192
+#define RC_TILE16_LDS_FLOATS (RC_LDS_HEAD + RC_NW * 16 * (16 + LDS_PAD))
+
+#include "rc_gates.h"
+#include "rc_mma.h"
+
+
+template <int MR, int NC, int D, bool PIPE, bool SPLIT = false, bool DEEPOK = true, bool NTW = false, bool W32 = (RC_SPLIT_W32 != 0), int OWN = 0>
+__device__ __forceinline__ void gemm_tile(const GemmProblem& P, const int B, const int m_tile0, const int n_tile, float* s_mem, const bool dead = false) {
+    static_assert(OWN == 0 || (MR == 1 && OWN <= 16), "own-row tiles are 16-row tiles");
+    constexpr int MT = 16 * MR, NT = 16 * NC, UT = 4 * NC, LD = NT + (MR >= 8 ? 4 : LDS_PAD);
+#ifdef RC_TRACE_TILES
+    unsigned long long trace_t[4] = {0, 0, 0, 0};
+    bool traced = false;
+#endif
+  for (int m_tile = m_tile0;; m_tile += P.m_tiles) {
+    int* s_rows = reinterpret_cast<int*>(s_mem);
+    int* s_cnt = s_rows + 128;
+    float* s_part = s_mem + RC_LDS_HEAD;
+    const int tid = OWN ? (int)(threadIdx.x & (RC_NW * 64 - 1)) : (int)threadIdx.x, lane = tid & 63, wave = tid >> 6;
+
+    TRACE_T(0);
+    const int lo = m_tile * (OWN ? OWN : MT);
+    int nrows;
+    if constexpr (OWN > 0) {
+        __syncthreads();
+        if (wave == 0) {
+            const int r = lo + lane;
+            const bool f = !dead && lane < OWN && r < B && (P.flag_bit == 0 || (P.flags[r] & P.flag_bit));
+            const unsigned long long bal = __ballot(f);
+            if (f) s_rows[__popcll(bal & ((1ull << lane) - 1ull))] = r;
+            if (lane == 0) s_cnt[0] = __popcll(bal);
+        }
+        __syncthreads();
+        nrows = s_cnt[0];
+        if (tid < MT && tid >= nrows) s_rows[tid] = nrows > 0 ? s_rows[0] : lo;
+        __syncthreads();
+    } else if (P.flag_bit == 0) {
+        nrows = min(MT, B - lo);
+        if (nrows <= 0) return;
+        __syncthreads();
+        if (tid < MT) s_rows[tid] = lo + min(tid, nrows - 1);
+        __syncthreads();
+    } else {
+        int total = 0;
+        __syncthreads();
+        for (int base = 0; base < B && total < lo + MT; base += RC_NW * 64) {
+            const int r = base + tid;
+            const bool f = r < B && (P.flags[r] & P.flag_bit);
+            const unsigned long long bal = __ballot(f);
+            if (lane == 0) s_cnt[wave] = __popcll(bal);
+            __syncthreads();
+            int woff = 0, sum = 0;
+#pragma unroll
+            for (int w = 0; w < RC_NW; ++w) {
+                const int cw = s_cnt[w];
+                woff += (w < wave) ? cw : 0;
+                sum += cw;
+            }
+            const int idx = total + woff + __popcll(bal & ((1ull << lane) - 1ull));
+            if (f && idx >= lo && idx < lo + MT) s_rows[idx - lo] = r;
+            total += sum;
+            __syncthreads();
+        }
+        nrows = min(MT, total - lo);
+        if (nrows <= 0) return;
+        if (tid < MT && tid >= nrows) s_rows[tid] = s_rows[0];
+        __syncthreads();
+    }
+    if (P.open_step && n_tile == 0 && tid < nrows) P.steps[s_rows[tid]] += 1;
+
+    const int i = lane & 15, kq = lane >> 4;
+    const float* pa0[MR];
+    const float* pa1[MR];
+    int row_r[MR], st_r[MR];
+#pragma unroll
+    for (int r = 0; r < MR; ++r) {
+        row_r[r] = s_rows[16 * r + i];
+        st_r[r] = (P.seg[0].par_mode | P.seg[1].par_mode) ? P.steps[row_r[r]] : 0;
+    }
+    FragS<MR, NC, W32> fa = {}, fb = {};
+    const int Qs = P.Kp / 32, Qws = Qs / RC_NW;
+    constexpr int WPL = W32 ? 2 : 3;
+    constexpr int KBU = WPL * 64;
+    const long long bs = (long long)Qs * KBU;
+    const u32x4* pbs = reinterpret_cast<const u32x4*>(W32 ? (const void*)P.W : P.Ws) + ((long long)(n_tile * NC) * Qs + (long long)wave * Qws) * KBU + lane;
+    constexpr bool DEEP = SPLIT && DEEPOK && MR >= 2 && (MR * 8 + NC * 4 * WPL) * 3 + (W32 ? NC * 12 : 0) + MR * NC * 4 <= 380;
+    if constexpr (SPLIT) {
+        load_kblock_b(fa, pbs, bs);
+        if constexpr (DEEP) load_kblock_b(fb, pbs + (long long)min(1, Qws - 1) * KBU, bs);
+    }
+#pragma unroll
+    for (int r = 0; r < MR; ++r) {
+        const int row = row_r[r];
+        const int st = st_r[r] + ((P.seg[0].par_mode | P.seg[1].par_mode) ? P.step_off : 0);
+        const float* pp[2];
+#pragma unroll
+        for (int sgi = 0; sgi < 2; ++sgi) {
+            const GemmSeg& sg = P.seg[sgi];
+            const int par = sg.par_mode == RC_PAR_SRC ? ((st - 1) % RC_HBUF) : (sg.par_mode == RC_PAR_DST ? (st % RC_HBUF) : 0);
+            const float* base = sg.base;
+            if (sgi == 0 && P.sel_bit && !(P.sel_flags[row] & P.sel_bit)) base = P.alt_base;
+            pp[sgi] = base + (long long)par * sg.par_stride + rc_pk(row, 4 * kq, sg.ld);
+        }
+        pa0[r] = pp[0];
+        pa1[r] = pp[1];
+    }
+    const int Q = P.Kp / RC_KC, Qw = Q / RC_NW;
+    const int K0 = P.seg[0].K;
+    const long long bstride = (long long)Q * 256;
+    const float* pb = P.W + ((long long)(n_tile * NC) * Q + (long long)wave * Qw) * 256 + lane * 4;
+    const int kbase = wave * Qw * RC_KC;
+
+    TRACE_T(1);
+    f32x4 acc[MR][NC];
+#pragma unroll
+    for (int r = 0; r < MR; ++r)
+#pragma unroll
+        for (int j = 0; j < NC; ++j) acc[r][j] = f32x4{0.f, 0.f, 0.f, 0.f};
+#define LOADC(F, QI)                                                                                      \
+    do {                                                                                                  \
+        const int k_ = kbase + (QI) * RC_KC;                                                              \
+        if (k_ < K0) load_chunk<MR, NC, NTW>(F, pa0, (long long)k_ * 16, pb + (long long)(QI) * 256, bstride);  \
+        else load_chunk<MR, NC, NTW>(F, pa1, (long long)(k_ - K0) * 16, pb + (long long)(QI) * 256, bstride);   \
+    } while (0)
+#define SB() do { if (PIPE) __builtin_amdgcn_sched_barrier(0); } while (0)
+    if constexpr (SPLIT) {
+        const int kb0 = wave * Qws * 32;
+#define LOADS_A(F, QI)                                                                                              \
+    do {                                                                                                            \
+        const int k_ = kb0 + (QI) * 32;                                                                             \
+        if (k_ < K0) load_kblock_a(F, pa0, (long long)k_ * 16);                                        \
+        else load_kblock_a(F, pa1, (long long)(k_ - K0) * 16);                                              \
+    } while (0)
+#define LOADS(F, QI)                                                                                                \
+    do {                                                                                                            \
+        const int k_ = kb0 + (QI) * 32;                                                                             \
+        if (k_ < K0) load_kblock(F, pa0, (long long)k_ * 16, pbs + (long long)(QI) * KBU, bs);              \
+        else load_kblock(F, pa1, (long long)(k_ - K0) * 16, pbs + (long long)(QI) * KBU, bs);               \
+    } while (0)
+        int q = 0;
+#define STEP(FL, QL, FM) do { LOADS(FL, QL); SB(); mma_kblock(FM, acc); SB(); } while (0)
+        if constexpr (DEEP) {
+            FragS<MR, NC, W32> fc = {};
+            LOADS_A(fa, 0);
+            LOADS_A(fb, min(1, Qws - 1));
+            for (; q + 3 <= Qws; q += 3) {
+                STEP(fc, min(q + 2, Qws - 1), fa);
+                STEP(fa, min(q + 3, Qws - 1), fb);
+                STEP(fb, min(q + 4, Qws - 1), fc);
+            }
+            if (q < Qws) mma_kblock(fa, acc);
+            if (q + 1 < Qws) mma_kblock(fb, acc);
+        } else {
+            LOADS_A(fa, 0);
+            for (; q + 2 <= Qws; q += 2) {
+                STEP(fb, min(q + 1, Qws - 1), fa);
+                STEP(fa, min(q + 2, Qws - 1), fb);
+            }
+            if (q < Qws) mma_kblock(fa, acc);
+        }
+#undef STEP
+#undef LOADS_A
+#undef LOADS
+    } else if constexpr (D == 2) {
+        Frag<MR, NC> fa = {}, fb = {};
+        int q = 0;
+        LOADC(fa, 0);
+        for (; q + 2 < Qw; q += 2) {
+            LOADC(fb, q + 1);
+            SB();
+            mma_chunk<MR, NC>(fa, acc);
+            SB();
+            LOADC(fa, q + 2);
+            SB();
+            mma_chunk<MR, NC>(fb, acc);
+            SB();
+        }
+        LOADC(fb, q + 1);
+        SB();
+        mma_chunk<MR, NC>(fa, acc);
+        SB();
+        mma_chunk<MR, NC>(fb, acc);
+    } else {
+        Frag<MR, NC> f[D];
+    #pragma unroll
+        for (int d = 0; d < D; ++d) f[d] = Frag<MR, NC>{};
+    #pragma unroll
+        for (int d = 0; d < D - 1; ++d) LOADC(f[d], min(d, Qw - 1));
+        int q = 0;
+        for (; q + D <= Qw; q += D) {
+    #pragma unroll
+            for (int d = 0; d < D; ++d) {
+                LOADC(f[(d + D - 1) % D], min(q + d + D - 1, Qw - 1));
+                SB();
+                mma_chunk<MR, NC>(f[d], acc);
+                SB();
+            }
+        }
+        const int rem = Qw - q;
+    #pragma unroll
+        for (int d = 0; d < D - 1; ++d)
+            if (d < rem) mma_chunk<MR, NC>(f[d], acc);
+    }
+#undef LOADC
+#undef SB
+
+    TRACE_T(2);
+    constexpr int EPI_ITEMS = (MT * UT + RC_NW * 64 - 1) / (RC_NW * 64);
+    float c_prev[EPI_ITEMS];
+    int st_row[EPI_ITEMS];
+    constexpr bool BIAS_ONE = (RC_NW * 64) % UT == 0;
+    f32x4 bias4 = f32x4{0.f, 0.f, 0.f, 0.f};
+    if (P.epi == RC_EPI_LSTM) {
+#pragma unroll
+        for (int k = 0; k < EPI_ITEMS; ++k) {
+            const int item = tid + k * RC_NW * 64;
+            const int rr = item / UT, u = item - rr * UT;
+            const bool ok = item < MT * UT && rr < nrows;
+            const int r2 = s_rows[ok ? rr : 0];
+            c_prev[k] = ok ? P.cstate[(long long)r2 * P.H + n_tile * UT + u] : 0.f;
+            st_row[k] = ok ? P.steps[r2] : 0;
+        }
+    }
+#pragma unroll
+    for (int r = 0; r < MR; ++r)
+#pragma unroll
+        for (int j = 0; j < NC; ++j)
+#pragma unroll
+            for (int e = 0; e < 4; ++e)
+                s_part[(wave * MT + 16 * r + 4 * kq + e) * LD + 16 * j + i] = acc[r][j][e];
+    if (P.epi == RC_EPI_LSTM) {
+        if constexpr (BIAS_ONE) bias4 = *reinterpret_cast<const f32x4*>(&P.bias[n_tile * NT + 4 * (tid % UT)]);
+    }
+    __syncthreads();
+
+    if (P.epi == RC_EPI_LSTM) {
+#pragma unroll
+        for (int k = 0; k < EPI_ITEMS; ++k) {
+            const int item = tid + k * RC_NW * 64;
+            const int rr = item / UT, u = item - rr * UT;
+            if (item >= MT * UT || rr >= nrows) continue;
+            const int unit = n_tile * UT + u;
+            static_assert(RC_NW == 4, "the reduction order below names the four K quarters");
+            f32x4 g4 = (*reinterpret_cast<const f32x4*>(&s_part[rr * LD + 4 * u]) + *reinterpret_cast<const f32x4*>(&s_part[(MT + rr) * LD + 4 * u])) +
+                       (*reinterpret_cast<const f32x4*>(&s_part[(2 * MT + rr) * LD + 4 * u]) + *reinterpret_cast<const f32x4*>(&s_part[(3 * MT + rr) * LD + 4 * u]));
+            if constexpr (BIAS_ONE) g4 += bias4; else g4 += *reinterpret_cast<const f32x4*>(&P.bias[n_tile * NT + 4 * u]);
+            const int r2 = s_rows[rr];
+            const int dst = (st_row[k] + P.step_off) % RC_HBUF;
+            const long long ci = (long long)r2 * P.H + unit;
+            float cn, hn;
+            rc_lstm_cell(g4[0], g4[1], g4[2], g4[3], c_prev[k], cn, hn);
+            P.cstate[ci] = cn;
+            P.hstate[(long long)dst * P.h_par_stride + rc_pk(r2, unit, P.H)] = hn;
+        }
+    } else {
+        const bool vec4 = P.out_packed && P.out_bit == 0 && ((P.out_col0 | P.N) & 3) == 0;
+        if (vec4) {
+            constexpr int V4_ITEMS = (MT * (NT / 4) + RC_NW * 64 - 1) / (RC_NW * 64);
+            constexpr bool B4_ONE = (RC_NW * 64) % (NT / 4) == 0;
+            f32x4 b4 = f32x4{0.f, 0.f, 0.f, 0.f};
+            if constexpr (B4_ONE) b4 = *reinterpret_cast<const f32x4*>(&P.bias[n_tile * NT + (tid % (NT / 4)) * 4]);
+#pragma unroll
+            for (int k = 0; k < V4_ITEMS; ++k) {
+                const int item = tid + k * RC_NW * 64;
+                const int rr = item / (NT / 4), c4 = (item - rr * (NT / 4)) * 4;
+                const int n = n_tile * NT + c4;
+                if (item >= MT * (NT / 4) || rr >= nrows || n >= P.N) continue;
+                f32x4 v = *reinterpret_cast<const f32x4*>(&s_part[rr * LD + c4]);
+#pragma unroll
+                for (int w = 1; w < RC_NW; ++w) v += *reinterpret_cast<const f32x4*>(&s_part[(w * MT + rr) * LD + c4]);
+                if constexpr (B4_ONE) v += b4; else v += *reinterpret_cast<const f32x4*>(&P.bias[n]);
+                if (P.epi == RC_EPI_RELU) { v[0] = fmaxf(v[0], 0.0f); v[1] = fmaxf(v[1], 0.0f); v[2] = fmaxf(v[2], 0.0f); v[3] = fmaxf(v[3], 0.0f); }
+                *reinterpret_cast<f32x4*>(&P.out[rc_pk(s_rows[rr], P.out_col0 + n, P.ldo)]) = v;
+            }
+        } else
+        for (int item = tid; item < MT * NT; item += RC_NW * 64) {
+            const int rr = item / NT, col = item - rr * NT;
+            if (rr >= nrows) continue;
+            const int n = n_tile * NT + col;
+            float v = s_part[rr * LD + col];
+#pragma unroll
+            for (int w = 1; w < RC_NW; ++w) v += s_part[(w * MT + rr) * LD + col];
+            v += P.bias[n];
+            if (P.epi == RC_EPI_RELU) v = fmaxf(v, 0.0f);
+            const int r2 = s_rows[rr];
+            if (n < P.N && (P.out_bit == 0 || (P.out_flags[r2] & P.out_bit))) {
+                P.out[P.out_packed ? rc_pk(r2, P.out_col0 + n, P.ldo) : (long long)r2 * P.ldo + P.out_col0 + n] = v;
+            }
+        }
+    }
+#ifdef RC_TRACE_TILES
+    if (threadIdx.x == 0 && !traced && g_trace_buf) {
+        traced = true;
+        const unsigned long long idx = (unsigned long long)P.trace_base + blockIdx.x;
+        if (idx < g_trace_cap) {
+            unsigned long long* r = g_trace_buf + idx * 8;
+            r[0] = (unsigned long long)blockIdx.x + 1; r[1] = (unsigned long long)(MR * 16 + NC) | ((unsigned long long)nrows << 16);
+            r[2] = __smid(); r[3] = (unsigned long long)n_tile | ((unsigned long long)m_tile << 32);
+            r[4] = trace_t[0]; r[5] = trace_t[1]; r[6] = trace_t[2]; r[7] = wall_clock64();
+        }
+    }
+#endif
+    if constexpr (OWN > 0) return;
+  }
+}
diff --git a/robustcap_amd/csrc/rc_internal.h b/robustcap_amd/csrc/rc_internal.h
--- a/robustcap_amd/csrc/rc_internal.h
+++ b/robustcap_amd/csrc/rc_internal.h
@@ -267,6 +267,17 @@
                     const WaveTail* wt = nullptr, hipEvent_t stop = nullptr);
 bool rc_launch_fuse_tail(const FrameBuffers& fb_tail, const FrameBuffers& fb_fuse, const FrameIO& io, const rc_params_dev& prm, const BodyConst* body, int B,
                          const WaveTail& wt, hipStream_t s, hipEvent_t stop);
+#define RC_LIN2_FOLD_MAXP 6
+inline bool rc_lin2_fold_covers(const GemmProblem* ps, int n_tail, int n_fuse) {
+    if (n_tail < 0 || n_fuse < 0 || n_tail > 4 || n_fuse > 4 || n_tail + n_fuse > RC_LIN2_FOLD_MAXP || n_tail + n_fuse == 0) return false;
+    for (int i = 0; i < n_tail + n_fuse; ++i) {
+        const GemmProblem& p = ps[i];
+        if (p.mr != 1 || p.nc != 1 || p.epi != RC_EPI_DENSE || p.open_step || p.n_tiles < 1 || p.n_tiles > 10 || p.Kp % RC_KALIGN != 0) return false;
+    }
+    return true;
+}
+bool rc_launch_lin2_fuse_tail(const GemmProblem* ps, int n_tail, int n_fuse, const FrameBuffers& fb_tail, const FrameBuffers& fb_fuse, const FrameIO& io,
+                              const rc_params_dev& prm, const BodyConst* body, int B, const WaveTail& wt, hipStream_t s, hipEvent_t stop);
 void rc_launch_prep_wave(const FrameBuffers& slot, const FrameIO& io0, const rc_params_dev& prm, int B, const WavePrep& w, hipStream_t s);
 void rc_launch_reset(const FrameBuffers& fb, float* const* h, float* const* c, const int* hidden, const unsigned char* mask,
                      int B, hipStream_t s);
```

Result: slower. 1.218 million body-frames/s (-3.8%).
